# pyro-ppl/pyro

Measured on AMD Instinct MI355X. Metric: ELBO-grad steps/sec (SVI), higher is better.
Workload: dtype f32; 1 GPU; BASELINE configs[1]: Bayesian logistic regression, plate=1000000, D=32, Trace_ELBO num_particles=64 per GPU (vectorised), AutoNormal, Adam; full SVI.step of SVI(model, guide, optim, loss), one hipGraph replay per step; parallelism=particles sharded x1, flat RCCL grad all-reduce

## Files before the change

### include/pyro_amd.h

```cpp
#ifndef PYRO_AMD_H
#define PYRO_AMD_H

#include <stddef.h>
#include <stdint.h>

#ifdef __cplusplus
extern "C" {
#endif

#define PA_ABI_VERSION 9

enum { PA_OK = 0, PA_ERR_INVALID = -1, PA_ERR_UNSUPPORTED = -2, PA_ERR_LAUNCH = -3 };

enum { PA_F32 = 0, PA_F64 = 1 };

enum {
  PA_DIST_NORMAL = 0,
  PA_DIST_BERNOULLI_LOGITS = 1,
  PA_DIST_HALF_CAUCHY = 2,
  PA_DIST_LOG_NORMAL = 3,
  PA_DIST_EXPONENTIAL = 4,
  PA_DIST_HALF_NORMAL = 5,
  PA_DIST_GAMMA = 6,
  PA_DIST_BETA = 7,
// ... 312 lines not shown
#define PA_LSE_MAX_DIMS 6
typedef struct {
  const void* ptr;
  int64_t strides[PA_LSE_MAX_DIMS];
} pa_lse_term;
int pa_logsumexp_terms(int dtype, void* out, int nterms, const pa_lse_term* terms, int ndim,
                       const int64_t* sizes, int rdim, pa_stream_t stream);
int pa_logsumexp_terms_grad(int dtype, void* G, const void* g_out, const void* out, int nterms,
                            const pa_lse_term* terms, int ndim, const int64_t* sizes, int rdim,
                            pa_stream_t stream);

int pa_adam_step(int dtype, void* param, void* grad, void* exp_avg, void* exp_avg_sq, int64_t n,
                 double lr, double beta1, double beta2, double eps, double weight_decay,
                 double clip_norm, double lrd, int clipped, int64_t* step_dev, int zero_grad,
                 pa_stream_t stream);

int pa_mvn_tril_sample(int dtype, const void* loc, const void* rho, const void* A, int64_t n,
                       int64_t P, uint64_t seed, uint64_t offset, const uint64_t* offset_dev,
                       int eps_given, void* eps, void* z, void* logq, pa_stream_t stream);
int pa_mvn_tril_sample_bwd(int dtype, const void* loc, const void* rho, const void* eps,
                           const void* z, const void* d_z, const void* d_logq, int64_t n,
                           int64_t P, void* d_loc, void* d_rho, void* d_A, int accumulate,
                           pa_stream_t stream);

size_t pa_logchain_workspace(int dtype, int64_t B, int64_t T, int64_t K);
int pa_logchain_fwd_bwd(int dtype, const void* unary, const void* pairwise,
                        int64_t pair_stride_batch, int64_t pair_stride_step, int64_t B,
                        int64_t T, int64_t K, void* log_z, void* grad_unary, void* grad_pairwise,
                        void* workspace, size_t workspace_bytes, pa_stream_t stream);

int pa_chain_matvec(int dtype, const void* M, int64_t m_stride_chain, const void* x, void* y,
                    int64_t C, int64_t D, int transpose, pa_stream_t stream);

int pa_adam_step_publish(int dtype, void* param, void* grad, void* exp_avg, void* exp_avg_sq,
                         int64_t n, double lr, double beta1, double beta2, double eps,
                         double weight_decay, double clip_norm, double lrd, int clipped,
                         int64_t* step_dev, int zero_grad, int src_dtype, const void* src,
                         double* host_value, uint64_t* host_seq, uint64_t* counter, uint64_t inc,
                         pa_stream_t stream);

size_t pa_bow_workspace(int64_t B, int64_t V, int64_t H);
int pa_bow_linear_fwd(const void* image_a, const float* W, const float* bias, int64_t B, int64_t V,
                      int64_t H, float* out, void* workspace, size_t workspace_bytes,
                      pa_stream_t stream);
int pa_bow_linear_bwd(const void* image_b, const float* d_out, int64_t B, int64_t V, int64_t H,
                      float* dW, void* workspace, size_t workspace_bytes, pa_stream_t stream);
int pa_bow_linear_fwd_act(const void* image_a, const float* W, const float* bias, int64_t B, int64_t V,
                          int64_t H, int sigmoid_out, float* out, void* workspace,
                          size_t workspace_bytes, pa_stream_t stream);
int pa_bow_linear_bwd_act(const void* image_b, const float* d_out, const float* y_mul, int64_t B, int64_t V,
                          int64_t H, float* dW, float* db_partial, void* workspace, size_t workspace_bytes,
                          pa_stream_t stream);

size_t pa_tsgemm_tn_workspace(int64_t B, int64_t M, int64_t N);
int pa_tsgemm_tn(const float* A, const float* X, int64_t B, int64_t M, int64_t N, float* out,
                 void* workspace, size_t workspace_bytes, pa_stream_t stream);

int pa_tall_linear(const float* G, int64_t B, int64_t R, const float* W, int64_t w_row_stride,
                   int64_t w_col_stride, int64_t C, const float* bias, float* Y, pa_stream_t stream);
size_t pa_tall_wgrad_workspace(int64_t B, int64_t R, int64_t K);
int pa_tall_wgrad(const float* G, const float* X, int64_t B, int64_t R, int64_t K, float* dW, float* db,
                  void* workspace, size_t workspace_bytes, pa_stream_t stream);
int pa_tall_linear_act(const float* G, int64_t B, int64_t R, const float* W, int64_t w_row_stride,
                       int64_t w_col_stride, int64_t C, const float* bias, const float* y_mul,
                       int sigmoid_out, float* Y, pa_stream_t stream);
int pa_tall_wgrad_act(const float* G, const float* X, const float* y_mul, int64_t B, int64_t R, int64_t K,
                      float* dW, float* db, void* workspace, size_t workspace_bytes, pa_stream_t stream);
int pa_tall_linear_path(int64_t B, int64_t R, int64_t C, int64_t w_row_stride, int64_t w_col_stride,
                        int g_aligned16, int ymul_aligned16, int w_aligned16);
int pa_tall_wgrad_path(int64_t B, int64_t R, int64_t K);

int pa_gamma_rsample(int dtype, void* out, void* d_alpha, pa_view2d alpha, int64_t rows, int64_t cols,
                     uint64_t seed, uint64_t offset, const uint64_t* offset_dev, pa_stream_t stream);
int pa_gamma_implicit_grad(int dtype, void* d_alpha, pa_view2d alpha, pa_view2d value, int64_t rows,
                           int64_t cols, pa_stream_t stream);

#define PA_CHAIN_SYNC_BYTES 64
int pa_chain_begin(pa_stream_t stream, void* sync_words, size_t sync_bytes);
int pa_chain_flush(void);
int pa_chain_end(int* launches, int* phases);
int pa_chain_pending(void);
int pa_chain_tune(int fuse_tail);
int pa_chain_fused_launches(void);
int pa_chain_debug_stamps(void* stamps32);

#define PA_RTC_MAX_POINTERS 384
int pa_rtc_compile(const char* source, const char* kernel_name, void** function_out);
int pa_rtc_compile_cached(const char* source, const char* kernel_name, const char* cache_file,
                          void** function_out, int* compiled_out);
int pa_rtc_version(int* hiprtc_major, int* hiprtc_minor, int* runtime_version);
void* pa_rtc_blocks_begin(void);
int pa_rtc_blocks_end(void* scope, int64_t* n_blocks_out);
int pa_rtc_blocks_free(void* scope);
int pa_rtc_launch(void* function, uint32_t grid, uint32_t block, const void* const* pointers,
                  int n_pointers, pa_stream_t stream);

size_t pa_mixture_workspace(int K, int64_t B);
int pa_mixture_fwd_bwd(int dtype, int dist, const void* x, int64_t N, int K, int64_t B, const void* a,
                       int64_t a_batch_stride, const void* p0, int64_t p0_stride, int64_t p0_batch_stride,
                       const void* p1, int64_t p1_stride, int64_t p1_batch_stride, void* workspace,
                       size_t workspace_bytes, double* out, pa_stream_t stream);

int pa_mixture_diag_normal_layout(int K, int D, int* kp_out, int* dd_out);
size_t pa_mixture_diag_normal_workspace(int K, int D, int64_t B);
int pa_mixture_diag_normal_fwd_bwd(int dtype, const void* x, int64_t N, int D, int K, int64_t B, const void* a,
                                   int64_t a_batch_stride, const void* loc, int64_t loc_stride_k,
                                   int64_t loc_stride_d, int64_t loc_batch_stride, const void* scale,
                                   int64_t scale_stride_k, int64_t scale_stride_d, int64_t scale_batch_stride,
                                   void* workspace, size_t workspace_bytes, double* out_padded, pa_stream_t stream);

int64_t pa_mixture_mvn_layout(int K, int D);
size_t pa_mixture_mvn_workspace(int K, int D, int64_t B);
int pa_mixture_mvn_fwd_bwd(int dtype, const void* x, int64_t N, int D, int K, int64_t B, const void* a,
                           int64_t a_batch_stride, const void* loc, int64_t loc_stride_k, int64_t loc_batch_stride,
                           const void* w, int64_t w_stride_k, int64_t w_batch_stride, void* row_lse,
                           void* workspace, size_t workspace_bytes, double* out, pa_stream_t stream);

int64_t pa_mixture_event_layout(int dist, int K, int D);
size_t pa_mixture_event_workspace(int dist, int K, int D, int64_t B);
int pa_mixture_event_fwd_bwd(int dtype, int dist, const void* x, int64_t N, int D, int K, int64_t B, const void* a,
                             int64_t a_batch_stride, const void* p0, int64_t p0_stride_k, int64_t p0_stride_d,
                             int64_t p0_batch_stride, const void* p1, int64_t p1_stride_k, int64_t p1_stride_d,
                             int64_t p1_batch_stride, void* row_lse, void* workspace, size_t workspace_bytes,
                             double* out, pa_stream_t stream);

int pa_mixture_rows_layout(int K, int* kp_out);
size_t pa_mixture_rows_workspace(int K, int64_t B);
int pa_mixture_rows_fwd_bwd(int dtype, int dist, const void* x, int64_t N, int K, int64_t B, const void* a,
                            int64_t a_stride_k, int64_t a_stride_n, int64_t a_batch_stride, const void* p0,
                            int64_t p0_stride, int64_t p0_batch_stride, const void* p1, int64_t p1_stride,
                            int64_t p1_batch_stride, void* da, void* workspace, size_t workspace_bytes,
                            double* out_padded, pa_stream_t stream);

int pa_mixture_rows_diag_normal_layout(int K, int D, int* kp_out, int* dd_out);
size_t pa_mixture_rows_diag_normal_workspace(int K, int D, int64_t B);
int pa_mixture_rows_diag_normal_fwd_bwd(int dtype, const void* x, int64_t N, int D, int K, int64_t B, const void* a,
                                        int64_t a_stride_k, int64_t a_stride_n, int64_t a_batch_stride,
                                        const void* loc, int64_t loc_stride_k, int64_t loc_stride_d,
                                        int64_t loc_batch_stride, const void* scale, int64_t scale_stride_k,
                                        int64_t scale_stride_d, int64_t scale_batch_stride, void* da,
                                        void* workspace, size_t workspace_bytes, double* out_padded,
                                        pa_stream_t stream);

int pa_mixture_assign(int dtype, int dist, const void* x, int64_t N, int K, int64_t B, const void* a,
                      int64_t a_stride_k, int64_t a_stride_n, int64_t a_batch_stride, const void* p0,
                      int64_t p0_stride, int64_t p0_batch_stride, const void* p1, int64_t p1_stride,
                      int64_t p1_batch_stride, int mode, uint64_t seed, uint64_t offset, const uint64_t* offset_dev,
                      int64_t* z, pa_stream_t stream);

int pa_mixture_assign_diag_normal(int dtype, const void* x, int64_t N, int D, int K, int64_t B, const void* a,
                                  int64_t a_stride_k, int64_t a_stride_n, int64_t a_batch_stride, const void* loc,
                                  int64_t loc_stride_k, int64_t loc_stride_d, int64_t loc_batch_stride,
                                  const void* scale, int64_t scale_stride_k, int64_t scale_stride_d,
                                  int64_t scale_batch_stride, int mode, uint64_t seed, uint64_t offset,
                                  const uint64_t* offset_dev, int64_t* z, pa_stream_t stream);

int pa_graph_direct_plan(void* hip_graph, int max_nodes, void** plan_out, int* n_nodes_out);
int pa_graph_direct_launch(void* plan, pa_stream_t stream);
int pa_graph_direct_free(void* plan);

#ifdef __cplusplus
}
#endif
#endif
```

### pyro_amd/_lib.py

```python
import ctypes
import os
from ctypes import (POINTER, Structure, c_char_p, c_double, c_int, c_int32, c_int64, c_size_t, c_uint32,
                    c_uint64, c_void_p)

_HERE = os.path.dirname(os.path.abspath(__file__))
LIB_PATH = os.path.join(_HERE, "lib", "libpyro_amd.so")

PA_OK, PA_ERR_INVALID, PA_ERR_UNSUPPORTED, PA_ERR_LAUNCH = 0, -1, -2, -3
PA_F32, PA_F64 = 0, 1
ABI_VERSION = 9

DIST_NORMAL = 0
DIST_BERNOULLI_LOGITS = 1
DIST_HALF_CAUCHY = 2
DIST_LOG_NORMAL = 3
DIST_EXPONENTIAL = 4
DIST_HALF_NORMAL = 5
DIST_GAMMA = 6
DIST_BETA = 7
DIST_POISSON = 8
DIST_BINOMIAL_LOGITS = 9
DIST_KL_NORMAL_LOC = 10
DIST_KL_NORMAL_SCALE = 11

# ... 220 lines not shown
                                                    c_size_t, c_void_p, c_void_p]),
    "pa_mixture_assign": (c_int, [c_int, c_int, c_void_p, c_int64, c_int, c_int64, c_void_p, c_int64, c_int64, c_int64,
                                  c_void_p, c_int64, c_int64, c_void_p, c_int64, c_int64, c_int, c_uint64, c_uint64,
                                  c_void_p, c_void_p, c_void_p]),
    "pa_mixture_assign_diag_normal": (c_int, [c_int, c_void_p, c_int64, c_int, c_int, c_int64, c_void_p, c_int64,
                                              c_int64, c_int64, c_void_p, c_int64, c_int64, c_int64, c_void_p,
                                              c_int64, c_int64, c_int64, c_int, c_uint64, c_uint64, c_void_p,
                                              c_void_p, c_void_p]),
    "pa_graph_direct_plan": (c_int, [c_void_p, c_int, POINTER(c_void_p), POINTER(c_int)]),
    "pa_graph_direct_launch": (c_int, [c_void_p, c_void_p]),
    "pa_graph_direct_free": (c_int, [c_void_p]),
    "pa_rtc_launch": (c_int, [c_void_p, c_uint32, c_uint32, c_void_p, c_int, c_void_p]),
    "pa_nuts_gaussian_find_step": (c_int, [c_int, c_void_p, c_void_p, c_void_p, c_void_p, c_void_p,
                                           c_void_p, c_int64, c_int64, c_uint64, c_uint64, c_uint64,
                                           c_double, c_double, c_double, c_void_p]),
    "pa_lda_factor_workspace": (c_size_t, [c_int, c_int64, c_int64, c_int64]),
    "pa_lda_factor_fwd_bwd": (c_int, [c_int, c_void_p, c_void_p, c_void_p, c_int64, c_int64,
                                      c_int64, c_int64, c_void_p, c_void_p, c_void_p, c_void_p,
                                      c_size_t, c_void_p]),
    "pa_dirichlet_log_prob": (c_int, [c_int, c_void_p, View2D, View2D, c_int64, c_int64, c_void_p]),
    "pa_dirichlet_log_prob_grad": (c_int, [c_int, c_void_p, View2D, View2D, c_int64, c_int64,
                                           c_void_p, c_void_p, c_void_p]),
    "pa_logsumexp_terms": (c_int, [c_int, c_void_p, c_int, POINTER(LseTerm), c_int, POINTER(c_int64),
                                   c_int, c_void_p]),
    "pa_logsumexp_terms_grad": (c_int, [c_int, c_void_p, c_void_p, c_void_p, c_int, POINTER(LseTerm),
                                        c_int, POINTER(c_int64), c_int, c_void_p]),
    "pa_lda_index_bytes": (c_size_t, [c_int64, c_int64, c_int64]),
    "pa_lda_index_workspace": (c_size_t, [c_int64, c_int64, c_int64]),
    "pa_lda_build_index": (c_int, [c_void_p, c_int64, c_int64, c_int64, c_void_p, c_size_t,
                                   c_void_p, c_size_t, c_void_p]),
    "pa_lda_factor_indexed_workspace": (c_size_t, [c_int, c_int64, c_int64, c_int64, c_int64]),
    "pa_lda_factor_indexed_fwd_bwd": (c_int, [c_int, c_void_p, c_void_p, c_size_t, c_void_p,
                                              c_void_p, c_int64, c_int64, c_int64, c_int64,
                                              c_void_p, c_void_p, c_void_p, c_void_p, c_size_t,
                                              c_void_p]),
    "pa_adam_step": (c_int, [c_int, c_void_p, c_void_p, c_void_p, c_void_p, c_int64, c_double,
                             c_double, c_double, c_double, c_double, c_double, c_double, c_int,
                             c_void_p, c_int, c_void_p]),
    "pa_dist_log_prob_sum_nd_workspace": (c_size_t, []),
    "pa_dist_log_prob_sum_nd": (c_int, [c_int, c_int, c_void_p, c_int, c_void_p, c_void_p, c_void_p,
                                        c_void_p, c_void_p, c_void_p, c_void_p, c_void_p, c_void_p,
                                        c_double, c_void_p, c_size_t, c_void_p]),
    "pa_dist_log_prob_grad_nd": (c_int, [c_int, c_int, c_void_p, c_void_p, c_void_p, c_void_p, c_int,
                                         c_void_p, c_void_p, c_void_p, c_void_p, c_void_p, c_void_p,
                                         c_void_p, c_void_p, c_void_p, c_double, c_void_p]),
    "pa_sum_to_nd_workspace": (c_size_t, [c_int64, c_int64, c_int64]),
    "pa_sum_to_nd": (c_int, [c_int, c_void_p, c_void_p, c_int64, c_int64, c_int64, c_void_p,
                             c_size_t, c_void_p]),
    "pa_sum_to_nd_pair": (c_int, [c_int, c_void_p, c_void_p, c_void_p, c_void_p, c_int64, c_int64, c_int64,
                                  c_void_p, c_size_t, c_void_p]),
    "pa_mvn_tril_sample": (c_int, [c_int, c_void_p, c_void_p, c_void_p, c_int64, c_int64, c_uint64,
                                   c_uint64, c_void_p, c_int, c_void_p, c_void_p, c_void_p, c_void_p]),
    "pa_mvn_tril_sample_bwd": (c_int, [c_int, c_void_p, c_void_p, c_void_p, c_void_p, c_void_p,
                                       c_void_p, c_int64, c_int64, c_void_p, c_void_p, c_void_p,
                                       c_int, c_void_p]),
    "pa_logchain_workspace": (c_size_t, [c_int, c_int64, c_int64, c_int64]),
    "pa_logchain_fwd_bwd": (c_int, [c_int, c_void_p, c_void_p, c_int64, c_int64, c_int64, c_int64,
                                    c_int64, c_void_p, c_void_p, c_void_p, c_void_p, c_size_t,
                                    c_void_p]),
    "pa_chain_matvec": (c_int, [c_int, c_void_p, c_int64, c_void_p, c_void_p, c_int64, c_int64, c_int,
                                c_void_p]),
    "pa_bow_workspace": (c_size_t, [c_int64, c_int64, c_int64]),
    "pa_bow_linear_fwd": (c_int, [c_void_p, c_void_p, c_void_p, c_int64, c_int64, c_int64, c_void_p,
                                  c_void_p, c_size_t, c_void_p]),
    "pa_bow_linear_bwd": (c_int, [c_void_p, c_void_p, c_int64, c_int64, c_int64, c_void_p, c_void_p,
                                  c_size_t, c_void_p]),
    "pa_bow_linear_fwd_act": (c_int, [c_void_p, c_void_p, c_void_p, c_int64, c_int64, c_int64, c_int, c_void_p,
                                      c_void_p, c_size_t, c_void_p]),
    "pa_bow_linear_bwd_act": (c_int, [c_void_p, c_void_p, c_void_p, c_int64, c_int64, c_int64, c_void_p,
                                      c_void_p, c_void_p, c_size_t, c_void_p]),
    "pa_tsgemm_tn_workspace": (c_size_t, [c_int64, c_int64, c_int64]),
    "pa_tsgemm_tn": (c_int, [c_void_p, c_void_p, c_int64, c_int64, c_int64, c_void_p, c_void_p, c_size_t,
                             c_void_p]),
    "pa_gamma_rsample": (c_int, [c_int, c_void_p, c_void_p, View2D, c_int64, c_int64, c_uint64, c_uint64,
                                 c_void_p, c_void_p]),
    "pa_gamma_implicit_grad": (c_int, [c_int, c_void_p, View2D, View2D, c_int64, c_int64, c_void_p]),
    "pa_chain_begin": (c_int, [c_void_p, c_void_p, c_size_t]),
    "pa_chain_flush": (c_int, []),
    "pa_chain_end": (c_int, [POINTER(c_int), POINTER(c_int)]),
    "pa_chain_pending": (c_int, []),
    "pa_chain_debug_stamps": (c_int, [c_void_p]),
    "pa_chain_tune": (c_int, [c_int]),
    "pa_chain_fused_launches": (c_int, []),
    "pa_adam_step_publish": (c_int, [c_int, c_void_p, c_void_p, c_void_p, c_void_p, c_int64,
                                     c_double, c_double, c_double, c_double, c_double, c_double,
                                     c_double, c_int, c_void_p, c_int, c_int, c_void_p, c_void_p,
                                     c_void_p, c_void_p, c_uint64, c_void_p]),
}

_lib = None


def exported_symbols():
    return sorted(_SIGNATURES)


def load(path=None):
    global _lib
    if _lib is not None:
        return _lib
    path = path or os.environ.get("PYRO_AMD_LIB", LIB_PATH)
    if not os.path.exists(path):
        raise RuntimeError(
            "pyro_amd: HIP extension %s not found. Build it with "
            "`python -m pyro_amd.csrc.build` (hipcc --offload-arch=gfx950). There is no CPU "
            "fallback." % path)
    import torch
    lib = ctypes.CDLL(path)
    for name, (res, args) in _SIGNATURES.items():
        fn = getattr(lib, name)
        fn.restype = res
        fn.argtypes = args
    if lib.pa_abi_version() != ABI_VERSION:
        raise RuntimeError("pyro_amd: ABI version mismatch: %d" % lib.pa_abi_version())
    if os.environ.get("PYRO_AMD_GLM_FINALIZE") == "in_kernel":
        lib.pa_glm_planes_finalize_mode(1)
    _lib = lib
    return lib


def check(rc):
    if rc == PA_OK:
        return
    msg = load().pa_last_error().decode("utf-8", "replace")
    if rc == PA_ERR_INVALID:
        raise ValueError("pyro_amd: " + msg)
    if rc == PA_ERR_UNSUPPORTED:
        raise Unsupported("pyro_amd: " + msg)
    raise RuntimeError("pyro_amd: kernel launch failed: " + msg)
```

### pyro_amd/csrc/chain.hip

```cpp
#include "chain.h"
#include "glm_finalize.h"
#include "multisite_dev.h"
#include "optim_dev.h"
#include "site_tail.h"

namespace pa {

constexpr int CH_FIN = 0, CH_MULTI = 1, CH_MF = 2, CH_ADAM = 3, CH_PHASES = 4;
constexpr int CH_MF_SITES = 8;

struct MfArgs8 {
  int nsites;
  MfSiteDev s[CH_MF_SITES];
};
static_assert(offsetof(MfArgs8, s) == offsetof(MfArgs, s), "layout");

constexpr int CH_TAIL_ENTRIES = 6;
struct TailSite {
  int n_entries;
  int entries[CH_TAIL_ENTRIES];
  int extras_mask;
  int64_t off_loc, off_rho;
  int fast;
  int layout;
};

struct ChainArgs {
  MultiArgs multi;
  MfArgs8 mf;
  const float* fin_part;
  float *fin_ll, *fin_gw, *fin_gb;
  double fin_scale, fin_ll_offset;
  int fin_nblocks, fin_npass, fin_D, fin_P, fin_DT, fin_PT;
  float* multi_out;
  const float* multi_g;
  double multi_coef_all;
  int multi_accumulate, multi_n;
  int64_t mf_P;
  int mf_gy, mf_nsites;
  float *ad_p, *ad_g, *ad_m, *ad_v;
  int64_t ad_n;
  double ad_lr, ad_b1, ad_b2, ad_eps, ad_wd, ad_clip, ad_lrd;
  int64_t* ad_step;
  int ad_clipped, ad_zero;
  AdamPublish ad_pub;
  uint32_t* sync;
  int have[CH_PHASES];
  int grid[CH_PHASES];
  int last;
  uint64_t* stamps;
  const int64_t* gate;
  uint32_t jitter;
  int tail_nsites;
  uint32_t fin_dep_mask;
  TailSite tail[CH_MF_SITES];
};
static_assert(sizeof(ChainArgs) <= 6144, "kernel arguments grew unexpectedly");

__device__ __forceinline__ void chain_jitter(uint32_t seed, int p, uint32_t salt) {
  if (seed == 0u) return;
  uint32_t hsh = seed * 2654435761u ^ (blockIdx.x + 1u) * 40503u ^ (uint32_t)(p + 1) * 2246822519u ^ salt;
  hsh ^= hsh >> 15;
  hsh *= 2654435761u;
  hsh ^= hsh >> 13;
  const uint32_t n = (hsh >> 8) & 63u;
  if ((hsh & 3u) == 0u) return;
  for (uint32_t i = 0; i < n; ++i) __builtin_amdgcn_s_sleep(8);
}

__device__ __forceinline__ void chain_signal(uint32_t jitter, uint32_t* sync, int p, uint32_t expected,
                                             bool last) {
  chain_jitter(jitter, p, 0x9e3779b9u);
  __syncthreads();
  if (threadIdx.x == 0) {
    __builtin_amdgcn_fence(__ATOMIC_RELEASE, "agent");
    const uint32_t old =
        __hip_atomic_fetch_add(&sync[p], 1u, __ATOMIC_RELAXED, __HIP_MEMORY_SCOPE_AGENT);
    if (last && old == expected - 1u) {
#pragma unroll
      for (int q = 0; q < CH_PHASES; ++q)
        __hip_atomic_store(&sync[q], 0u, __ATOMIC_RELAXED, __HIP_MEMORY_SCOPE_AGENT);
    }
  }
}

__device__ __forceinline__ void chain_wait(uint32_t jitter, uint32_t* sync, int p, uint32_t expected) {
  if (threadIdx.x == 0) {
    const uint64_t t0 = wall_clock64();
    while (__hip_atomic_load(&sync[p], __ATOMIC_RELAXED, __HIP_MEMORY_SCOPE_AGENT) < expected) {
      __builtin_amdgcn_s_sleep(2);
      if (wall_clock64() - t0 > 400000000ull) __builtin_trap();
    }
    __builtin_amdgcn_fence(__ATOMIC_ACQUIRE, "agent");
  }
  __syncthreads();
  chain_jitter(jitter, p, 0x85ebca6bu);
}

template <int DT, int PT, int SUB>
__device__ __forceinline__ void chain_fin(const ChainArgs& a, int me, int nw) {
  __shared__ double sm[SUB][FIN_GROUPS][FIN_OUT];
  const int sub = SUB == 1 ? 0 : (int)(threadIdx.x >> 8), tid = (int)(threadIdx.x & 255);
  for (int64_t base = (int64_t)me * SUB; base < a.grid[CH_FIN]; base += (int64_t)nw * SUB) {
    glm_finalize_body<DT, PT>(base + sub, a.fin_part, a.fin_nblocks, a.fin_npass, a.fin_D, a.fin_P,
                              a.fin_scale, a.fin_ll, a.fin_gw, a.fin_gb, a.fin_ll_offset, tid,
                              sm[sub]);
    __syncthreads();
  }
}
template <int SUB>
__device__ __forceinline__ void chain_fin_any(const ChainArgs& a, int me, int nw) {
  if (a.fin_DT == 1 && a.fin_PT == 2) chain_fin<1, 2, SUB>(a, me, nw);
  else if (a.fin_DT == 1 && a.fin_PT == 1) chain_fin<1, 1, SUB>(a, me, nw);
  else if (a.fin_DT == 2 && a.fin_PT == 1) chain_fin<2, 1, SUB>(a, me, nw);
  else if (a.fin_DT == 2 && a.fin_PT == 2) chain_fin<2, 2, SUB>(a, me, nw);
  else if (a.fin_DT == 4 && a.fin_PT == 2) chain_fin<4, 2, SUB>(a, me, nw);
  else chain_fin<4, 1, SUB>(a, me, nw);
}

#define PA_CHAIN_STAMP(i)                                                     \
  do {                                                                        \
    if (a.stamps != nullptr && threadIdx.x == 0 && (me == 0 || total_wg))     \
      a.stamps[(total_wg ? 16 : 0) + (i)] = wall_clock64();                   \
  } while (0)

__global__ __launch_bounds__(1024) void chain_kernel(const ChainArgs a) {
  if (a.gate != nullptr && *a.gate != 0) return;
  const bool total_wg = blockIdx.x == gridDim.x - 1;
  if (!total_wg && threadIdx.x >= 256) return;
  const int nw = (int)gridDim.x - 1, me = (int)blockIdx.x;
  uint32_t* sync = a.sync;
  const int part_fin = a.grid[CH_FIN] < nw ? a.grid[CH_FIN] : nw;
  const int part_multi = (a.multi_n < nw ? a.multi_n : nw) + 1;
  const int part_mf = a.grid[CH_MF] < nw ? a.grid[CH_MF] : nw;
  int prev = -1, prev_n = 0;
  PA_CHAIN_STAMP(0);

  if (a.have[CH_FIN]) {
    if (!total_wg && me < part_fin) {
      chain_fin_any<1>(a, me, nw);
      chain_signal(a.jitter, sync, CH_FIN, (uint32_t)part_fin, a.last == CH_FIN);
    }
    prev = CH_FIN;
    prev_n = part_fin;
  }
  PA_CHAIN_STAMP(1);
  if (a.have[CH_MULTI]) {
    constexpr uint32_t KB = (uint32_t)offsetof(ChainArgs, multi);
    if (total_wg || me < part_multi - 1) {
      if (prev >= 0) chain_wait(a.jitter, sync, prev, (uint32_t)prev_n);
      PA_CHAIN_STAMP(2);
      if (total_wg) {
        multi_sum_body<float, MULTI_THREADS>(KB, a.multi_out, a.multi_coef_all, a.multi_accumulate);
      } else {
        for (int vb = me; vb < a.multi_n; vb += nw) {
          multi_grad_body<float>(KB, vb, a.multi_g, a.multi_coef_all);
          __syncthreads();
        }
      }
      chain_signal(a.jitter, sync, CH_MULTI, (uint32_t)part_multi, a.last == CH_MULTI);
    }
    prev = CH_MULTI;
    prev_n = part_multi;
  }
  PA_CHAIN_STAMP(3);
  if (total_wg) return;
  if (a.have[CH_MF]) {
    constexpr uint32_t KB = (uint32_t)offsetof(ChainArgs, mf);
    if (me < part_mf) {
      if (prev >= 0) chain_wait(a.jitter, sync, prev, (uint32_t)prev_n);
      PA_CHAIN_STAMP(4);
      for (int vb = me; vb < a.grid[CH_MF]; vb += nw) {
        meanfield_sample_bwd_body<float>(KB, (uint32_t)(vb % a.mf_nsites),
                                         (uint32_t)(vb / a.mf_nsites), (uint32_t)a.mf_gy, a.mf_P);
        __syncthreads();
      }
      chain_signal(a.jitter, sync, CH_MF, (uint32_t)part_mf, a.last == CH_MF);
    }
    prev = CH_MF;
    prev_n = part_mf;
  }
  PA_CHAIN_STAMP(5);
  if (a.have[CH_ADAM]) {
    const int part_adam = a.grid[CH_ADAM] < nw ? a.grid[CH_ADAM] : nw;
    if (me < part_adam) {
      if (prev >= 0) chain_wait(a.jitter, sync, prev, (uint32_t)prev_n);
      PA_CHAIN_STAMP(6);
      for (int64_t vb = me; vb < a.grid[CH_ADAM]; vb += nw)
        adam_body<float>(vb, (int64_t)a.grid[CH_ADAM], a.ad_p, a.ad_g, a.ad_m, a.ad_v, a.ad_n,
                         a.ad_lr, a.ad_b1, a.ad_b2, a.ad_eps, a.ad_wd, a.ad_clip, a.ad_lrd,
                         a.ad_clipped, a.ad_step, a.ad_zero, a.ad_pub);
      chain_signal(a.jitter, sync, CH_ADAM, (uint32_t)part_adam, a.last == CH_ADAM);
    }
  }
  PA_CHAIN_STAMP(7);
}

__global__ __launch_bounds__(1024) void chain_tail_kernel(const ChainArgs a) {
  if (a.gate != nullptr && *a.gate != 0) return;
  const bool total_wg = blockIdx.x == gridDim.x - 1;
  const int nw = (int)gridDim.x - 1, me = (int)blockIdx.x;
  uint32_t* sync = a.sync;
  if (me < a.tail_nsites && threadIdx.x >= 256) return;
  const int nfw = nw - a.tail_nsites;
  const int fin_vwg = (a.grid[CH_FIN] + 3) / 4;
  const int part_fin = fin_vwg < nfw ? fin_vwg : nfw;
  PA_CHAIN_STAMP(0);
  if (!total_wg && me >= a.tail_nsites) {
    const int fme = me - a.tail_nsites;
    if (a.have[CH_FIN] && fme < part_fin) {
      chain_fin_any<4>(a, fme, nfw);
      chain_signal(a.jitter, sync, CH_FIN, (uint32_t)part_fin, false);
    }
    return;
  }
  PA_CHAIN_STAMP(1);
  constexpr uint32_t KB = (uint32_t)offsetof(ChainArgs, multi);
  constexpr uint32_t KMF = (uint32_t)offsetof(ChainArgs, mf);
  const uint32_t KT = (uint32_t)offsetof(ChainArgs, tail) + (uint32_t)me * (uint32_t)sizeof(TailSite);
  auto tail_entry = [&](int q) -> int {
    return kernarg_load<int>(KT + (uint32_t)offsetof(TailSite, entries) + 4u * (uint32_t)q);
  };
  int ts_n = 0, ts_mask = 0, ts_fast = 0;
  int64_t step = 0;
  if (!total_wg) ts_fast = kernarg_load<int>(KT + (uint32_t)offsetof(TailSite, fast));
  if (!total_wg && ts_fast) {
    __shared__ double fast_red[4 * GRAD_THREADS];
    __shared__ float fast_xch[4 * 64];
    const int layout = kernarg_load<int>(KT + (uint32_t)offsetof(TailSite, layout));
    const EntryDev eh = kernarg_load<EntryDev>(KB + (uint32_t)offsetof(MultiArgs, e) +
                                               (uint32_t)tail_entry(0) * (uint32_t)sizeof(EntryDev));
    const EntryDev eg = kernarg_load<EntryDev>(KB + (uint32_t)offsetof(MultiArgs, e) +
                                               (uint32_t)tail_entry(1) * (uint32_t)sizeof(EntryDev));
    const MfSiteDev ms = kernarg_load<MfSiteDev>(KMF + (uint32_t)offsetof(MfArgs, s) +
                                                 (uint32_t)me * (uint32_t)sizeof(MfSiteDev));
    const int64_t off_loc = kernarg_load<int64_t>(KT + (uint32_t)offsetof(TailSite, off_loc));
    const int64_t off_rho = kernarg_load<int64_t>(KT + (uint32_t)offsetof(TailSite, off_rho));
    const SiteAdam ad{a.ad_p, a.ad_g, a.ad_m, a.ad_v, a.ad_step, a.ad_lr, a.ad_b1, a.ad_b2, a.ad_eps,
                      a.ad_wd, a.ad_clip, a.ad_lrd, a.ad_clipped, a.ad_zero};
    auto wait = [&]() {
      PA_CHAIN_STAMP(7);
      if (a.have[CH_FIN]) chain_wait(a.jitter, sync, CH_FIN, (uint32_t)part_fin);
      else __syncthreads();
      PA_CHAIN_STAMP(2);
    };
    site_fast<PA_DIST_NORMAL>(eh, eg, ms, layout, a.multi_coef_all, off_loc, off_rho, ad, fast_red,
                              fast_xch, wait, &step);
    PA_CHAIN_STAMP(5);
  } else {
  double total_acc = 0.0;
  if (total_wg) {
    total_acc = multi_sum_partial<float, MULTI_THREADS>(KB, a.fin_dep_mask, 0u);
  }
  if (!total_wg) {
    ts_n = kernarg_load<int>(KT + (uint32_t)offsetof(TailSite, n_entries));
    ts_mask = kernarg_load<int>(KT + (uint32_t)offsetof(TailSite, extras_mask));
    for (int q = 0; q < ts_n; ++q) {
      multi_grad_body<float>(KB, tail_entry(q), a.multi_g, a.multi_coef_all, GRAD_NO_EXTRAS);
      __syncthreads();
    }
  }
  PA_CHAIN_STAMP(7);
  if (a.have[CH_FIN]) chain_wait(a.jitter, sync, CH_FIN, (uint32_t)part_fin);
  PA_CHAIN_STAMP(2);
  if (total_wg) {
    total_acc += multi_sum_partial<float, MULTI_THREADS>(KB, 0u, a.fin_dep_mask);
    multi_sum_finish<float>(total_acc, a.multi_out, a.multi_coef_all, a.multi_accumulate);
    if (threadIdx.x == 0) step = a.ad_step[0] + 1;
  } else {
    for (int q = 0; q < ts_n; ++q)
      if (ts_mask >> q & 1)
        multi_grad_body<float>(KB, tail_entry(q), a.multi_g, a.multi_coef_all, GRAD_EXTRAS_ONLY);
    __syncthreads();
    PA_CHAIN_STAMP(3);
    meanfield_sample_bwd_body<float>(KMF, (uint32_t)me, 0u, 1u, a.mf_P);
    __syncthreads();
    PA_CHAIN_STAMP(4);
    const MfSiteDev ms = kernarg_load<MfSiteDev>(KMF + (uint32_t)offsetof(MfArgs, s) +
                                                 (uint32_t)me * (uint32_t)sizeof(MfSiteDev));
    const int64_t off_loc = kernarg_load<int64_t>(KT + (uint32_t)offsetof(TailSite, off_loc));
    const int64_t off_rho = kernarg_load<int64_t>(KT + (uint32_t)offsetof(TailSite, off_rho));
    adam_two_ranges<float>(off_loc, off_rho, ms.n, a.ad_p, a.ad_g, a.ad_m, a.ad_v, a.ad_step,
                           a.ad_lr, a.ad_b1, a.ad_b2, a.ad_eps, a.ad_wd, a.ad_clip, a.ad_lrd,
                           a.ad_clipped, a.ad_zero, &step);
    PA_CHAIN_STAMP(5);
  }
  }
  __syncthreads();
  if (threadIdx.x == 0) {
    __builtin_amdgcn_fence(__ATOMIC_RELEASE, "agent");
    const unsigned long long ticket = __hip_atomic_fetch_add(
        reinterpret_cast<unsigned long long*>(a.ad_step + 1), 1ull, __ATOMIC_RELAXED,
        __HIP_MEMORY_SCOPE_AGENT);
    if (ticket == (unsigned long long)a.tail_nsites) {
      __builtin_amdgcn_fence(__ATOMIC_ACQUIRE, "agent");
      a.ad_step[1] = 0;
      a.ad_step[0] = step;
#pragma unroll
      for (int q = 0; q < CH_PHASES; ++q)
        __hip_atomic_store(&sync[q], 0u, __ATOMIC_RELAXED, __HIP_MEMORY_SCOPE_AGENT);
      publish_to_host(a.ad_pub);
    }
  }
  PA_CHAIN_STAMP(6);
}

static int g_chain_fast_sites = 1;

static bool chain_plan_tail(ChainArgs& a) {
  if (!(a.have[CH_MULTI] && a.have[CH_MF] && a.have[CH_ADAM])) return false;
  if (a.multi_g != nullptr || a.mf_nsites < 1 || a.mf_nsites > CH_MF_SITES) return false;
  const float* g0 = a.ad_g;
  const float* g1 = a.ad_g + a.ad_n;
  int owner[PA_MULTI_MAX_ENTRIES];
  for (int e = 0; e < a.multi.n; ++e) owner[e] = -1;
  int64_t covered = 0;
  int64_t lo[2 * CH_MF_SITES], hi[2 * CH_MF_SITES];
  for (int k = 0; k < a.mf_nsites; ++k) {
    const MfSiteDev& s = a.mf.s[k];
    TailSite& t = a.tail[k];
    t.n_entries = 0;
    t.extras_mask = 0;
    if (s.n < 1 || s.n > 4096 || !s.accumulate || s.d_loc == nullptr || s.d_rho == nullptr) return false;
    const float* dl = (const float*)s.d_loc;
    const float* dr = (const float*)s.d_rho;
    if (dl < g0 || dl + s.n > g1 || dr < g0 || dr + s.n > g1) return false;
    t.off_loc = dl - g0;
    t.off_rho = dr - g0;
    lo[2 * k] = t.off_loc; hi[2 * k] = t.off_loc + s.n;
    lo[2 * k + 1] = t.off_rho; hi[2 * k + 1] = t.off_rho + s.n;
    covered += 2 * s.n;
    for (int e = 0; e < a.multi.n; ++e) {
      const EntryDev& en = a.multi.e[e];
      const bool own_v = (en.need & PA_NEED_VALUE) && en.dv && !(en.need & PA_VALUE_BY_CHAIN);
      const bool own_a = (en.need & PA_NEED_P0) && en.da, own_b = (en.need & PA_NEED_P1) && en.db;
      int hits = 0, outs = 0;
      if (own_v) { ++outs; hits += (en.dv == s.d_z); }
      if (own_a) { ++outs; hits += (en.da == s.d_loc_out || en.da == s.d_scale); }
      if (own_b) { ++outs; hits += (en.db == s.d_loc_out || en.db == s.d_scale); }
      if (hits == 0) continue;
      if (hits != outs || owner[e] >= 0) return false;
      if (t.n_entries == CH_TAIL_ENTRIES) return false;
      owner[e] = k;
      if (t.n_entries == 0) t.extras_mask = 0;
      if (own_v && en.xg != nullptr) t.extras_mask |= 1 << t.n_entries;
      t.entries[t.n_entries++] = e;
    }
  }
  for (int e = 0; e < a.multi.n; ++e) {
    const EntryDev& en = a.multi.e[e];
    const bool writes = ((en.need & PA_NEED_VALUE) && en.dv && !(en.need & PA_VALUE_BY_CHAIN)) ||
                        ((en.need & PA_NEED_P0) && en.da) || ((en.need & PA_NEED_P1) && en.db);
    if (writes && owner[e] < 0) return false;
  }
  for (int k = 0; k < a.mf_nsites; ++k) {
    const MfSiteDev& s = a.mf.s[k];
    const void* wants[3] = {s.d_z, s.d_scale, s.d_loc_out};
    for (const void* w : wants) {
      if (w == nullptr) continue;
      bool found = false;
      for (int q = 0; q < a.tail[k].n_entries && !found; ++q) {
        const EntryDev& en = a.multi.e[a.tail[k].entries[q]];
        found = en.dv == w || en.da == w || en.db == w;
      }
      if (!found) return false;
    }
  }
  if (covered != a.ad_n) return false;
  const int m = 2 * a.mf_nsites;
  for (int i = 0; i < m; ++i)
    for (int j = i + 1; j < m; ++j)
      if (lo[i] < hi[j] && lo[j] < hi[i]) return false;
  a.fin_dep_mask = 0u;
  if (a.have[CH_FIN]) {
    auto in_fin = [&](const void* p) {
      const float* f = (const float*)p;
      return p != nullptr &&
             ((f >= a.fin_ll && f < a.fin_ll + a.fin_P) || (f >= a.fin_gb && f < a.fin_gb + a.fin_P) ||
              (f >= a.fin_gw && f < a.fin_gw + (int64_t)a.fin_P * a.fin_D));
    };
    for (int e = 0; e < a.multi.n; ++e) {
      const EntryDev& en = a.multi.e[e];
      if (in_fin(en.v) || in_fin(en.a) || in_fin(en.b) || in_fin(en.m)) a.fin_dep_mask |= 1u << e;
    }
    if (a.multi.n > MULTI_THREADS / 64) a.fin_dep_mask = 0xffffffffu;
  }
  for (int k = 0; k < a.mf_nsites; ++k) {
    const MfSiteDev& s = a.mf.s[k];
    TailSite& t = a.tail[k];
    t.fast = 0;
    t.layout = SITE_LAYOUT_COLS;
    if (!g_chain_fast_sites || t.n_entries != 2) continue;
    const EntryDev& h = a.multi.e[t.entries[0]];
    const EntryDev& q = a.multi.e[t.entries[1]];
    const bool family = h.dist == PA_DIST_NORMAL;
    const bool shape =
        family && q.dist == PA_DIST_NORMAL && h.m == nullptr &&
        q.m == nullptr && h.chain_next == t.entries[1] && q.chain_next < 0 &&
        (h.need & PA_NEED_VALUE) && !(h.need & PA_VALUE_BY_CHAIN) && h.dv == s.d_z &&
        !((h.need & PA_NEED_P0) && h.da) && !((h.need & PA_NEED_P1) && h.db) &&
        (q.need & PA_VALUE_BY_CHAIN) && (q.need & PA_NEED_P0) && (q.need & PA_NEED_P1) &&
        q.da == s.d_loc_out && q.db == s.d_scale && q.da != nullptr && q.db != nullptr &&
        q.v == h.v && q.vsr == h.vsr && q.vsc == h.vsc && q.rows == h.rows && q.cols == h.cols &&
        s.d_z != nullptr && s.eps != nullptr && s.rho != nullptr;
    if (!shape) continue;
    const int64_t P = a.mf_P;
    if (s.n >= 2 && s.n <= GRAD_THREADS && h.rows == P && h.cols == s.n && h.vsr == s.n &&
        h.vsc == 1 && q.asr == 0 && q.asc == 1 && q.bsr == 0 && q.bsc == 1) {
      const int64_t ng = GRAD_THREADS / s.n > 8 ? 8 : GRAD_THREADS / s.n;
      if (P <= UN * ng) { t.fast = 1; t.layout = SITE_LAYOUT_COLS; }
    } else if (s.n == 1 && h.rows == 1 && h.cols == P && P >= 2 && P <= 64 && h.vsc == 1 &&
               q.asc == 0 && q.bsc == 0) {
      t.fast = 1;
      t.layout = SITE_LAYOUT_SCALAR;
    }
  }
  a.tail_nsites = a.mf_nsites;
  return true;
}

struct ChainState {
  bool on = false;
  hipStream_t stream = nullptr;
  int top = -1;
  int launches = 0;
  int phases = 0;
  int fused = 0;
  ChainArgs a;
};
static ChainState g_chain;
static uint64_t* g_chain_stamps = nullptr;
static int g_chain_fuse = 1;
static uint32_t g_chain_jitter = 0;

static int chain_launch() {
  ChainState& c = g_chain;
  if (c.top < 0) return PA_OK;
  ChainArgs& a = c.a;
  int maxgrid = 1, np = 0;
  for (int p = 0; p < CH_PHASES; ++p)
    if (a.have[p]) {
      a.last = p;
      ++np;
      if (a.grid[p] > maxgrid) maxgrid = a.grid[p];
    }
  a.stamps = g_chain_stamps;
  gate_emit_deferred(c.stream);
  a.gate = gate_word();
  a.jitter = g_chain_jitter;
  gate_aware_launch();
  int nw = cu_count() - 1;
  if (nw < 1) nw = 1;
  if (maxgrid < nw) nw = maxgrid;
  const hipStream_t s = c.stream;
  c.top = -1;
  a.tail_nsites = 0;
  if (g_chain_fuse && cu_count() - 1 > CH_MF_SITES && chain_plan_tail(a)) {
    nw = a.tail_nsites + (a.have[CH_FIN] ? (a.grid[CH_FIN] + 3) / 4 : 0);
    if (nw > cu_count() - 1) nw = cu_count() - 1;
    hipLaunchKernelGGL(chain_tail_kernel, dim3((unsigned)nw + 1), dim3(1024), 0, s, a);
    c.fused += 1;
  } else {
    hipLaunchKernelGGL(chain_kernel, dim3((unsigned)nw + 1), dim3(1024), 0, s, a);
  }
  c.launches += 1;
  c.phases += np;
  for (int p = 0; p < CH_PHASES; ++p) a.have[p] = 0;
  return check_launch("chain_kernel");
}

static bool chain_open(pa_stream_t stream, int k, int* rc) {
  ChainState& c = g_chain;
  *rc = PA_OK;
  if (!c.on) return false;
  if ((hipStream_t)stream != c.stream) {
    *rc = chain_launch();
    return false;
  }
  if (c.top >= k) *rc = chain_launch();
  if (*rc != PA_OK) return false;
  if (c.top < 0) {
    for (int p = 0; p < CH_PHASES; ++p) c.a.have[p] = 0, c.a.grid[p] = 0;
  }
  c.top = k;
  c.a.have[k] = 1;
  return true;
}

int chain_record_fin(pa_stream_t stream, int DT, int PT, const float* part, int nblocks, int npass,
                     int D, int P, double scale, float* ll, float* gw, float* gb, double ll_offset) {
  const bool shape_ok = (PT == 1 || PT == 2) && (DT == 1 || DT == 2 || DT == 4);
  if (!g_chain.on || !shape_ok) return 0;
  int rc;
  if (!chain_open(stream, CH_FIN, &rc)) return rc;
  ChainArgs& a = g_chain.a;
  a.fin_part = part; a.fin_ll = ll; a.fin_gw = gw; a.fin_gb = gb;
  a.fin_scale = scale; a.fin_ll_offset = ll_offset;
  a.fin_nblocks = nblocks; a.fin_npass = npass; a.fin_D = D; a.fin_P = P;
  a.fin_DT = DT; a.fin_PT = PT;
  const int64_t J = (int64_t)P * D + 2 * P;
  a.grid[CH_FIN] = (int)((J + FIN_OUT - 1) / FIN_OUT);
  return 1;
}

int chain_record_multi(pa_stream_t stream, const MultiArgs& args, float* out, const float* g,
                       double coef_all, int accumulate) {
  if (!g_chain.on) return 0;
  int rc;
  if (!chain_open(stream, CH_MULTI, &rc)) return rc;
  ChainArgs& a = g_chain.a;
  a.multi = args;
  a.multi_out = out; a.multi_g = g; a.multi_coef_all = coef_all; a.multi_accumulate = accumulate;
  a.multi_n = args.n;
  a.grid[CH_MULTI] = args.n;
  return 1;
}

int chain_record_mf_bwd(pa_stream_t stream, const MfArgs& args, int nsites, int64_t P, int gy) {
  if (!g_chain.on || nsites > CH_MF_SITES) return 0;
  int rc;
  if (!chain_open(stream, CH_MF, &rc)) return rc;
  ChainArgs& a = g_chain.a;
  a.mf.nsites = nsites;
  for (int k = 0; k < nsites; ++k) a.mf.s[k] = args.s[k];
  a.mf_P = P; a.mf_gy = gy; a.mf_nsites = nsites;
  a.grid[CH_MF] = nsites * gy;
  return 1;
}

// ... 10 lines not shown
  a.ad_lrd = lrd; a.ad_step = step_dev; a.ad_clipped = clipped; a.ad_zero = zero_grad;
  a.ad_pub = pub;
  int64_t grid = (n + 255) / 256;
  const int64_t cap = (int64_t)cu_count() * 8;
  if (grid > cap) grid = cap;
  a.grid[CH_ADAM] = (int)grid;
  return 1;
}

struct PendingDraw {
  bool have = false;
  MfArgs args;
  int nsites = 0;
  int64_t P = 0;
  uint64_t seed = 0;
  const uint64_t* offset_dev = nullptr;
};
static PendingDraw g_draw;
static int g_draw_enabled = 1;

int meanfield_sample_launch(const MfArgs& args, int nsites, int64_t P, uint64_t seed,
                            const uint64_t* offset_dev, hipStream_t s);

int chain_flush_draw() {
  if (!g_draw.have) return PA_OK;
  g_draw.have = false;
  return meanfield_sample_launch(g_draw.args, g_draw.nsites, g_draw.P, g_draw.seed, g_draw.offset_dev,
                                 g_chain.stream);
}

int chain_park_draw(pa_stream_t stream, const MfArgs& args, int nsites, int64_t P, uint64_t seed,
                    const uint64_t* offset_dev) {
  if (!g_chain.on || !g_draw_enabled || (hipStream_t)stream != g_chain.stream || g_chain.top >= 0) return 0;
  int rc = chain_flush_draw();
  if (rc != PA_OK) return rc;
  g_draw.have = true;
  g_draw.args = args;
  g_draw.nsites = nsites;
  g_draw.P = P;
  g_draw.seed = seed;
  g_draw.offset_dev = offset_dev;
  return 1;
}

bool glm_take_pending_draw(pa_stream_t stream, const float* w, const float* b, int64_t P, int64_t D,
                           GlmDraw* out) {
  if (!g_draw.have || (hipStream_t)stream != g_chain.stream || g_draw.P != P) return false;
  int kw = -1, kb = -1;
  for (int k = 0; k < g_draw.nsites; ++k) {
    const MfSiteDev& sd = g_draw.args.s[k];
    if (sd.z == (const void*)w && sd.n == D) kw = k;
    if (b != nullptr && sd.z == (const void*)b && sd.n == 1) kb = k;
  }
  if (kw < 0 || (b != nullptr && kb < 0)) return false;
  const MfSiteDev& sw = g_draw.args.s[kw];
  out->loc_w = (const float*)sw.loc; out->rho_w = (const float*)sw.rho;
  out->z_w = (float*)sw.z; out->eps_w = (float*)sw.eps; out->scale_w = (float*)sw.scale;
  out->lout_w = (float*)sw.loc_out; out->off_w = sw.offset;
  out->have_b = kb >= 0;
  if (kb >= 0) {
    const MfSiteDev& sb = g_draw.args.s[kb];
    out->loc_b = (const float*)sb.loc; out->rho_b = (const float*)sb.rho;
    out->z_b = (float*)sb.z; out->eps_b = (float*)sb.eps; out->scale_b = (float*)sb.scale;
    out->lout_b = (float*)sb.loc_out; out->off_b = sb.offset;
  } else {
    out->loc_b = out->rho_b = nullptr;
    out->z_b = out->eps_b = out->scale_b = out->lout_b = nullptr;
    out->off_b = 0;
  }
  out->seed = g_draw.seed;
  out->offset_dev = g_draw.offset_dev;
  MfArgs rest;
  rest.nsites = 0;
  for (int k = 0; k < g_draw.nsites; ++k)
    if (k != kw && k != kb) rest.s[rest.nsites++] = g_draw.args.s[k];
  g_draw.have = false;
  if (rest.nsites > 0)
    (void)meanfield_sample_launch(rest, rest.nsites, g_draw.P, g_draw.seed, g_draw.offset_dev, g_chain.stream);
  return true;
}

hipStream_t as_stream(pa_stream_t s) {
  if (g_draw.have) (void)chain_flush_draw();
  if (g_chain.on && g_chain.top >= 0) (void)chain_launch();
  return (hipStream_t)s;
}

}

extern "C" {

int pa_chain_begin(pa_stream_t stream, void* sync_words, size_t sync_bytes) {
  PA_REQUIRE(!pa::g_chain.on, "pa_chain_begin: already recording on this thread");
  PA_REQUIRE(sync_words != nullptr && sync_bytes >= PA_CHAIN_SYNC_BYTES,
             "pa_chain_begin: needs %d zeroed bytes of device memory", PA_CHAIN_SYNC_BYTES);
  pa::g_chain.on = true;
  pa::g_chain.stream = (hipStream_t)stream;
  pa::g_chain.top = -1;
  pa::g_chain.launches = pa::g_chain.phases = pa::g_chain.fused = 0;
  for (int p = 0; p < pa::CH_PHASES; ++p) pa::g_chain.a.have[p] = 0;
  pa::g_chain.a.sync = (uint32_t*)sync_words;
  return PA_OK;
}

int pa_chain_flush(void) {
  if (!pa::g_chain.on) return PA_OK;
  int rc = pa::chain_flush_draw();
  if (rc != PA_OK) return rc;
  return pa::chain_launch();
}

int pa_chain_end(int* launches, int* phases) {
  int rc = PA_OK;
  if (pa::g_chain.on) {
    rc = pa::chain_flush_draw();
    const int rc2 = pa::chain_launch();
    if (rc == PA_OK) rc = rc2;
  }
  pa::g_chain.on = false;
  if (launches) *launches = pa::g_chain.launches;
  if (phases) *phases = pa::g_chain.phases;
  return rc;
}

int pa_chain_tune(int fuse_tail) {
  pa::g_chain_fuse = (fuse_tail & 1) ? 1 : 0;
  pa::g_chain_fast_sites = (fuse_tail & 2) ? 0 : 1;
  pa::g_chain_jitter = (uint32_t)fuse_tail >> 8;
  pa::g_draw_enabled = (fuse_tail & 4) ? 0 : 1;
  return PA_OK;
}

int pa_chain_fused_launches(void) { return pa::g_chain.fused; }

int pa_chain_debug_stamps(void* stamps32) {
  pa::g_chain_stamps = (uint64_t*)stamps32;
#ifdef PA_CHAIN_LATENCY_PROBE
  uint64_t* p = (uint64_t*)stamps32;
  int zero = 0;
  (void)hipMemcpyToSymbol(HIP_SYMBOL(pa::pa_dbg_stamps), &p, sizeof(p));
  (void)hipMemcpyToSymbol(HIP_SYMBOL(pa::pa_dbg_next), &zero, sizeof(zero));
#endif
  return PA_OK;
}

int pa_chain_pending(void) {
  if (!pa::g_chain.on || pa::g_chain.top < 0) return 0;
  int n = 0;
  for (int p = 0; p < pa::CH_PHASES; ++p) n += pa::g_chain.a.have[p];
  return n;
}

}
```

### pyro_amd/csrc/common.h

```cpp
#pragma once
#include <hip/hip_runtime.h>
#include <stdarg.h>
#include <stdint.h>
#include <stdio.h>

#include "../../include/pyro_amd.h"

namespace pa {

__device__ __forceinline__ float fast_sigmoid(float h) {
  return __builtin_amdgcn_rcpf(1.0f + __builtin_amdgcn_exp2f(-1.44269504088896340736f * h));
}


constexpr int WAVE = 64;

void set_error(const char* fmt, ...);
int fail(int code, const char* fmt, ...);
int check_launch(const char* what);
int cu_count();
const int64_t* gate_word();
void gate_aware_launch();
void gate_emit_deferred(hipStream_t s);
bool take_bracket(int tag, hipEvent_t* start, hipEvent_t* stop);

#define PA_REQUIRE(cond, ...)                                  \
  do {                                                         \
    if (!(cond)) return ::pa::fail(PA_ERR_INVALID, __VA_ARGS__); \
  } while (0)

template <int CTRL>
__device__ __forceinline__ int dpp_mov(int v) {
  return __builtin_amdgcn_update_dpp(0, v, CTRL, 0xf, 0xf, false);
}
template <int CTRL>
__device__ __forceinline__ float dpp_get(float v) {
  return __int_as_float(dpp_mov<CTRL>(__float_as_int(v)));
}
template <int CTRL>
__device__ __forceinline__ double dpp_get(double v) {
  const int lo = dpp_mov<CTRL>(__double2loint(v)), hi = dpp_mov<CTRL>(__double2hiint(v));
  return __hiloint2double(hi, lo);
}
__device__ __forceinline__ float lane_get(float v, int lane) {
  return __int_as_float(__builtin_amdgcn_readlane(__float_as_int(v), lane));
}
__device__ __forceinline__ double lane_get(double v, int lane) {
  const int lo = __builtin_amdgcn_readlane(__double2loint(v), lane);
  const int hi = __builtin_amdgcn_readlane(__double2hiint(v), lane);
  return __hiloint2double(hi, lo);
}
template <typename T>
__device__ __forceinline__ T wave_sum(T v) {
  if constexpr (sizeof(T) == 4 || sizeof(T) == 8) {
    v += dpp_get<0xB1>(v);
    v += dpp_get<0x4E>(v);
    v += dpp_get<0x141>(v);
    v += dpp_get<0x140>(v);
    const T s0 = lane_get(v, 0), s1 = lane_get(v, 16), s2 = lane_get(v, 32), s3 = lane_get(v, 48);
    return (s0 + s1) + (s2 + s3);
  } else {
#pragma unroll
    for (int o = 32; o > 0; o >>= 1) v += __shfl_xor(v, o, 64);
    return v;
  }
}
template <typename T>
__device__ __forceinline__ T wave_max(T v) {
#pragma unroll
  for (int o = 32; o > 0; o >>= 1) {
    T u = __shfl_xor(v, o, 64);
    v = u > v ? u : v;
  }
  return v;
}

__device__ __forceinline__ double block_sum_f64_waves(double v, double* smem ,
                                                      int nw) {
  v = wave_sum(v);
  const int lane = threadIdx.x & 63, wid = threadIdx.x >> 6;
  __syncthreads();
  if (lane == 0) smem[wid] = v;
  __syncthreads();
  double t = 0.0;
  if (threadIdx.x == 0)
    for (int i = 0; i < nw; ++i) t += smem[i];
  return t;
}

__device__ __forceinline__ double block_sum_f64(double v, double* smem ) {
  v = wave_sum(v);
  const int lane = threadIdx.x & 63, wid = threadIdx.x >> 6, nw = (blockDim.x + 63) >> 6;
  __syncthreads();
  if (lane == 0) smem[wid] = v;
  __syncthreads();
  double t = 0.0;
  if (threadIdx.x == 0)
    for (int i = 0; i < nw; ++i) t += smem[i];
  return t;
}

struct u32x4 {
  uint32_t x, y, z, w;
};
__host__ __device__ __forceinline__ u32x4 philox4x32_10(uint64_t seed, uint64_t ctr_lo,
                                                        uint64_t ctr_hi) {
// ... 72 lines not shown
```

### pyro_amd/csrc/glm.hip

```cpp
#include "common.h"
#include "glm_bf16.h"
#include "glm_planes.h"
#include "glm_planes16.h"
#include "glm_planes16w.h"
#include "glm_planes16d.h"
#include "glm_finalize.h"
#include "chain.h"

namespace pa {

static int g_glm_variant = 0;

typedef float f32x16 __attribute__((ext_vector_type(16)));

constexpr int GLM_WAVES = 4;

template <int DT>
struct GlmCfg {
  static constexpr int DP = 32 * DT;
  static constexpr int S = DP + 3;
  static constexpr int TILE_F = 32 * S;
};


template <int DT, int PT, bool VEC4, bool GROUPED>
__global__ __launch_bounds__(64 * GLM_WAVES, 2) void glm_bernoulli_kernel(
    const float* __restrict__ X, const float* __restrict__ y, const float* __restrict__ w,
    const float* __restrict__ b, const uint8_t* __restrict__ mask, int64_t N, int D, int P,
    int64_t iters, float* __restrict__ part, const int64_t* __restrict__ seg, int G) {
  using C = GlmCfg<DT>;
  constexpr int DP = C::DP, S = C::S, TILE_F = C::TILE_F;
  extern __shared__ __attribute__((aligned(16))) float lds[];
  const int lane = threadIdx.x & 63, wave = threadIdx.x >> 6;
  const int l31 = lane & 31, h = lane >> 5;
  float* Xs = lds + wave * TILE_F;

  for (int i = threadIdx.x; i < GLM_WAVES * TILE_F; i += 64 * GLM_WAVES) lds[i] = 0.0f;

  int64_t row_begin = 0, row_end = N;
  int group = 0;
  if constexpr (GROUPED) {
    row_begin = seg[3 * (int64_t)blockIdx.x];
    row_end = seg[3 * (int64_t)blockIdx.x + 1];
    group = (int)seg[3 * (int64_t)blockIdx.x + 2];
  }

  const int pbase = blockIdx.y * 32 * PT;
  float wf[PT][DP / 2];
  float bias[PT];
#pragma unroll
  for (int pt = 0; pt < PT; ++pt) {
    const int p = pbase + pt * 32 + l31;
#pragma unroll
    for (int kk = 0; kk < DP / 2; ++kk) {
      const int d = 2 * kk + h;
      wf[pt][kk] = (p < P && d < D)
                       ? w[(GROUPED ? ((int64_t)p * G + group) : (int64_t)p) * D + d]
                       : 0.0f;
    }
    bias[pt] = (p < P && b != nullptr) ? b[p] : 0.0f;
  }

  f32x16 gwacc[PT][DT];
  float ll_acc[PT], gb_acc[PT];
#pragma unroll
  for (int pt = 0; pt < PT; ++pt) {
    ll_acc[pt] = 0.0f;
    gb_acc[pt] = 0.0f;
#pragma unroll
    for (int dt = 0; dt < DT; ++dt)
#pragma unroll
      for (int r = 0; r < 16; ++r) gwacc[pt][dt][r] = 0.0f;
  }

  constexpr int NLD = VEC4 ? 4 * DT : 16 * DT;
  constexpr int EPL = VEC4 ? 4 : 1;
  float stage[NLD * EPL];
  uint8_t stage_m[NLD];
  float st_y = 0.0f, st_m = 0.0f;
  const int step_e = 64 * EPL;
  const int q0 = step_e / D, r0 = step_e % D;
  const int e0 = lane * EPL;
  const int n_first = e0 / D, d_first = e0 % D;
  const int64_t total_e = row_end * (int64_t)D;
  int nrow[NLD];
  {
    int n = n_first, d = d_first;
#pragma unroll
    for (int j = 0; j < NLD; ++j) {
      nrow[j] = n;
// ... 390 lines not shown
  (void)hipFuncSetAttribute((const void*)k, hipFuncAttributeMaxDynamicSharedMemorySize, lds);
  hipLaunchKernelGGL(k, dim3((unsigned)pl.nblocks, (unsigned)pl.npass), dim3(256), lds, s, img, y, w,
                     b, N, D, P, pl.nst, part, cu_count(), fin, GlmGroupArgs{nullptr, nullptr, 1});
}

static void glm_planes_launch_grouped(int nseg, int npass, const unsigned char* img,
                                      const float* y_img, const float* w, const float* b, int64_t N,
                                      int D, int P, int64_t nst_total, float* part,
                                      const GlmGroupArgs& grp, hipStream_t s) {
  auto k = glm_planes_kernel<2, 3, 3, true>;
  constexpr int lds = GlmPlCfg<2, 3>::LDS_BYTES;
  (void)hipFuncSetAttribute((const void*)k, hipFuncAttributeMaxDynamicSharedMemorySize, lds);
  GlmFinArgs fin;
  fin.counters = nullptr;
  fin.part64 = nullptr;
  fin.ll = fin.gw = fin.gb = nullptr;
  fin.scale = fin.ll_offset = 0.0;
  fin.D = D; fin.P = P;
  fin.tstamps = g_planes_stamps;
  hipLaunchKernelGGL(k, dim3((unsigned)nseg, (unsigned)npass), dim3(256), lds, s, img, y_img, w, b, N,
                     D, P, nst_total, part, cu_count(), fin, grp);
}

static int64_t glmh_tile_bytes(int64_t ntiles) { return ntiles * (int64_t)GLMH_TILE; }

static bool g_planes_wide = true;
static int g_planes_wide_max = 8;
static bool g_planes_wide_force = false;

static GlmPlanesPlan glmh_plan(int64_t N, int64_t P, bool allow_wide = true) {
  GlmPlanesPlan pl;
  pl.nb = g_planes_nb;
  pl.bpc = g_planes_bpc > 0 && g_planes_bpc <= 4 ? g_planes_bpc : 2;
  pl.npass = (int)((P + 63) / 64);
  pl.nst = ((N + 31) / 32 + 1) / 2;
  int64_t cap = (int64_t)cu_count() * pl.bpc / pl.npass;
  if (cap < 1) cap = 1;
  pl.nblocks = (int)(pl.nst < cap ? (pl.nst < 1 ? 1 : pl.nst) : cap);
  pl.ypass = pl.npass;
  const bool enough_tiles = (N + 31) / 32 >= (int64_t)48 * cu_count();
  if (allow_wide && g_planes_wide && pl.nb == 3 && g_planes_bpc <= 0 && P > 64 &&
      (enough_tiles || g_planes_wide_force)) {
    const bool eight = P > 128 && g_planes_wide_max >= 8;
    pl.nrt = eight ? 1 : 2;
    pl.npt = eight ? 8 : 4;
    const int64_t wrows = 32 * pl.npt;
    pl.ypass = (int)((P + wrows - 1) / wrows);
    pl.nst = pl.nrt == 1 ? (N + 31) / 32 : ((N + 31) / 32 + 1) / 2;
    pl.bpc = 1;
    cap = (int64_t)cu_count() / pl.ypass;
    if (cap < 1) cap = 1;
    pl.nblocks = (int)(pl.nst < cap ? (pl.nst < 1 ? 1 : pl.nst) : cap);
  }
  return pl;
}

template <int NRT, int NPT, bool LIN>
static void glmh_launch_wide(const GlmPlanesPlan& pl, const unsigned char* img, const float* y, const float* w,
                             const float* b, int64_t N, int D, int P, float* part, const uint32_t* trailer,
                             hipStream_t s, const double* moments) {
  auto k = glm_planes_f16_kernel<3, 1, false, false, LIN, false, NRT, NPT>;
  constexpr int lds = GlmHCfg<3, false, NRT, NPT>::LDS_BYTES;
  (void)hipFuncSetAttribute((const void*)k, hipFuncAttributeMaxDynamicSharedMemorySize, lds);
  hipLaunchKernelGGL(k, dim3((unsigned)pl.nblocks, (unsigned)pl.ypass), dim3(64 * NRT * NPT), lds, s, img, y, w, b,
                     N, D, P, pl.nst, part, cu_count(), trailer, g_planes_stamps, GlmGroupArgs{nullptr, nullptr, 1},
                     gate_word(), moments, GlmDraw{});
  gate_aware_launch();
}

template <int NB, int OCC, bool PRIV = false, bool LIN = false, bool DRAW = false>
static void glmh_launch_one(const GlmPlanesPlan& pl, const unsigned char* img, const float* y,
                            const float* w, const float* b, int64_t N, int D, int P, float* part,
                            const uint32_t* trailer, hipStream_t s, const double* moments = nullptr,
                            const GlmDraw& draw = GlmDraw{}) {
  auto k = glm_planes_f16_kernel<NB, OCC, false, PRIV, LIN, DRAW>;
  constexpr int lds = GlmHCfg<NB, PRIV>::LDS_BYTES + (DRAW ? 256 : 0);
  (void)hipFuncSetAttribute((const void*)k, hipFuncAttributeMaxDynamicSharedMemorySize, lds);
  hipLaunchKernelGGL(k, dim3((unsigned)pl.nblocks, (unsigned)pl.npass), dim3(256), lds, s, img, y, w,
                     b, N, D, P, pl.nst, part, cu_count(), trailer, g_planes_stamps,
                     GlmGroupArgs{nullptr, nullptr, 1}, gate_word(), moments, draw);
  gate_aware_launch();
}

template <int DT, int OCC>
static int glmd_launch(const unsigned char* img, const float* y, const float* w, const float* b, int64_t N,
                       int D, int P, float* part, const uint32_t* trailer, int bpc, int* nblocks_out,
                       int64_t* nst_out, hipStream_t s) {
  auto k = glm_planes_f16d_kernel<DT, 3, OCC>;
  constexpr int lds = GlmDCfg<DT, 3>::LDS_BYTES;
  (void)hipFuncSetAttribute((const void*)k, hipFuncAttributeMaxDynamicSharedMemorySize, lds);
  const int npass = (int)((P + 63) / 64);
  const int64_t nst = ((N + 31) / 32 + 1) / 2;
  int64_t cap = (int64_t)cu_count() * bpc / npass;
  if (cap < 1) cap = 1;
  const int nblocks = (int)(nst < cap ? (nst < 1 ? 1 : nst) : cap);
  *nblocks_out = nblocks;
  *nst_out = nst;
  hipLaunchKernelGGL(k, dim3((unsigned)nblocks, (unsigned)npass), dim3(256), lds, s, img, y, w, b, N, D, P,
                     nst, part, trailer, gate_word());
  gate_aware_launch();
  return check_launch("glm_planes_f16d_kernel");
}

static int glmd_run(const void* planes, const float* y, const float* w, const float* b, double scale,
                    int64_t N, int D, int P, float* ll, float* gw, float* gb, float* part,
                    pa_stream_t stream, hipStream_t s) {
  const int DT = D <= 64 ? 2 : 4;
  const unsigned char* img = (const unsigned char*)planes;
  const uint32_t* trailer = (const uint32_t*)(img + glmh_tile_bytes(glm_planes_tiles(N)) * DT);
  hipEvent_t ev0, ev1;
  const bool br = take_bracket(PA_KERNEL_GLM, &ev0, &ev1);
  if (br) (void)hipEventRecord(ev0, s);
  int nblocks = 1;
  int64_t nst = 0;
  int rc = DT == 2 ? glmd_launch<2, 2>(img, y, w, b, N, D, P, part, trailer, 2, &nblocks, &nst, s)
                   : glmd_launch<4, 1>(img, y, w, b, N, D, P, part, trailer, 1, &nblocks, &nst, s);
  if (br) (void)hipEventRecord(ev1, s);
  if (rc != PA_OK) return rc;
  const int npass = (P + 63) / 64;
  const double ll_offset = (double)(nst * 64 - N) * 0.6931471805599453;
  rc = chain_record_fin(stream, DT, 2, part, nblocks, npass, D, P, scale, ll, gw, gb, ll_offset);
  if (rc != 0) return rc < 0 ? rc : PA_OK;
  const int64_t J = (int64_t)P * D + 2 * P;
  const dim3 fgrid((unsigned)((J + FIN_OUT - 1) / FIN_OUT)), fblock(FIN_OUT * FIN_GROUPS);
  if (DT == 2)
    hipLaunchKernelGGL((glm_finalize_kernel<2, 2>), fgrid, fblock, 0, s, part, nblocks, npass, D, P, scale, ll,
                       gw, gb, ll_offset);
  else
    hipLaunchKernelGGL((glm_finalize_kernel<4, 2>), fgrid, fblock, 0, s, part, nblocks, npass, D, P, scale, ll,
                       gw, gb, ll_offset);
  return check_launch("glm_finalize_kernel");
}

template <int NB>
static void glmw_launch(int bpc, const unsigned char* img, const float* y, const float* w, const float* b,
                        int64_t N, int D, int P, float* part, const uint32_t* trailer, int* nblocks_out,
                        hipStream_t s) {
  auto k = glm_planes_f16w_kernel<NB>;
  constexpr int lds = GlmWCfg<NB>::LDS_BYTES;
  (void)hipFuncSetAttribute((const void*)k, hipFuncAttributeMaxDynamicSharedMemorySize, lds);
  const int npass = (int)((P + 63) / 64);
  const int64_t ngrp = (N + 127) / 128;
  int64_t cap = (int64_t)cu_count() * bpc / npass;
  if (cap < 1) cap = 1;
  const int nblocks = (int)(ngrp < cap ? ngrp : cap);
  *nblocks_out = nblocks;
  hipLaunchKernelGGL(k, dim3((unsigned)nblocks, (unsigned)npass), dim3(256), lds, s, img, y, w, b, N, D, P,
                     ngrp, part, trailer, g_planes_stamps, gate_word());
  gate_aware_launch();
}

template <int OCC>
static void glmh_launch_grouped(int nseg, int npass, const unsigned char* img, const float* y_img,
                                const float* w, const float* b, int64_t N, int D, int P,
                                int64_t nst_total, float* part, const uint32_t* trailer,
                                const GlmGroupArgs& grp, hipStream_t s) {
  auto k = glm_planes_f16_kernel<3, OCC, true>;
  constexpr int lds = GlmHCfg<3>::LDS_BYTES;
  (void)hipFuncSetAttribute((const void*)k, hipFuncAttributeMaxDynamicSharedMemorySize, lds);
  hipLaunchKernelGGL(k, dim3((unsigned)nseg, (unsigned)npass), dim3(256), lds, s, img, y_img, w, b, N,
                     D, P, nst_total, part, cu_count(), trailer, g_planes_stamps, grp, gate_word(),
                     (const double*)nullptr, GlmDraw{});
  gate_aware_launch();
}

static int glmh_absmax(const float* X, int64_t N, int D, uint32_t* trailer, hipStream_t s) {
// ... 374 lines not shown
size_t pa_glm_bernoulli_planes_workspace(int64_t N, int64_t D, int64_t P) {
  if (N < 0 || D < 1 || D > 128 || P < 1) return 0;
  if (D > 32) {
    const size_t npass = (size_t)((P + 63) / 64);
    const size_t cap = (size_t)pa::cu_count() * 2;
    const size_t nst = (size_t)(((N + 31) / 32 + 1) / 2);
    const size_t nb = nst < cap ? (nst < 1 ? 1 : nst) : cap;
    return nb * npass * (2 * (size_t)glmd_dt(D) * 1024 + 2 * 2 * 32) * sizeof(float);
  }
  const pa::GlmPlanesPlan pl = pa::glm_planes_plan(N, P);
  const size_t cap = (size_t)pa::cu_count() * 4;
  const size_t ntiles = (size_t)((N + 31) / 32);
  const size_t nb = ntiles < cap ? (ntiles < 1 ? 1 : ntiles) : cap;
  const size_t rec = 2 * 1024 + 2 * 2 * 32;
  return nb * pl.npass * rec * sizeof(float) +
         (size_t)pl.npass * pa::GLMF_GROUPS * rec * sizeof(double);
}

size_t pa_glm_label_moments_workspace(int64_t N) {
  if (N < 0) return 0;
  int64_t grid = (N + 63) / 64;
  const int64_t cap = (int64_t)pa::cu_count() * 4;
  if (grid > cap) grid = cap;
  if (grid < 1) grid = 1;
  return (size_t)grid * 33 * sizeof(double);
}

int pa_glm_label_moments(const float* X, const float* y, int64_t N, int64_t D, double* moments,
                         void* workspace, size_t workspace_bytes, pa_stream_t stream) {
  PA_REQUIRE(N >= 0 && D >= 1 && D <= 32, "glm_label_moments: bad shape N=%lld D=%lld", (long long)N,
             (long long)D);
  PA_REQUIRE(moments != nullptr && (N == 0 || (X && y)), "glm_label_moments: NULL pointer");
  PA_REQUIRE(workspace && workspace_bytes >= pa_glm_label_moments_workspace(N),
             "glm_label_moments: workspace too small");
  const int nblocks = (int)(pa_glm_label_moments_workspace(N) / (33 * sizeof(double)));
  hipStream_t s = pa::as_stream(stream);
  hipLaunchKernelGGL(pa::glm_label_moments_partial_kernel, dim3((unsigned)nblocks), dim3(256), 0, s, X, y,
                     N, (int)D, (double*)workspace);
  int rc = pa::check_launch("glm_label_moments_partial_kernel");
  if (rc != PA_OK) return rc;
  hipLaunchKernelGGL(pa::glm_label_moments_final_kernel, dim3(1), dim3(64), 0, s,
                     (const double*)workspace, nblocks, moments);
  return pa::check_launch("glm_label_moments_final_kernel");
}

int pa_glm_bernoulli_planes_fwd_bwd(int format, const void* planes, const float* y, const float* w,
                                    const float* b, double scale, int64_t N, int64_t D, int64_t P,
                                    float* ll, float* gw, float* gb, void* workspace,
                                    size_t workspace_bytes, const double* moments,
                                    pa_stream_t stream) {
  PA_REQUIRE(N >= 0 && D >= 1 && P >= 1, "glm_planes: bad shape N=%lld D=%lld P=%lld", (long long)N,
             (long long)D, (long long)P);
  if (D > 128 || (D > 32 && format != PA_GLM_PLANES_F16X2))
    return pa::fail(PA_ERR_UNSUPPORTED, "glm_planes: the plane image holds D <= 32 (f16 format: D <= 128), got %lld",
                    (long long)D);
  PA_REQUIRE_FORMAT(format, "glm_planes");
  PA_REQUIRE(N < (int64_t(1) << 40) && P < (1 << 20), "glm_planes: shape too large");
  PA_REQUIRE(w && ll && gw && gb, "glm_planes: NULL parameter/output pointer");
  PA_REQUIRE(N == 0 || (planes && y), "glm_planes: NULL data pointer");
  pa::GlmDraw draw;
  bool drawn = false;
  if (format == PA_GLM_PLANES_F16X2 && N > 0 && D <= 32) {
    const pa::GlmPlanesPlan p0 = pa::glmh_plan(N, P);
    if (p0.nb == 3 && p0.bpc < 4) drawn = pa::glm_take_pending_draw(stream, w, b, P, D, &draw);
  }
  hipStream_t s = pa::as_stream(stream);
  if (N == 0) {
    hipError_t e1 = hipMemsetAsync(ll, 0, (size_t)P * 4, s);
    hipError_t e2 = hipMemsetAsync(gw, 0, (size_t)P * D * 4, s);
    hipError_t e3 = hipMemsetAsync(gb, 0, (size_t)P * 4, s);
    if (e1 != hipSuccess || e2 != hipSuccess || e3 != hipSuccess)
      return pa::fail(PA_ERR_LAUNCH, "glm_planes: memset failed");
    return PA_OK;
  }
  PA_REQUIRE((reinterpret_cast<uintptr_t>(planes) & 15) == 0, "glm_planes: unaligned image");
  PA_REQUIRE(workspace && workspace_bytes >= pa_glm_bernoulli_planes_workspace(N, D, P),
             "glm_planes: workspace too small");
  if (D > 32) return pa::glmd_run(planes, y, w, b, scale, N, (int)D, (int)P, ll, gw, gb, (float*)workspace, stream, s);
  pa::GlmPlanesPlan pl =
      format == PA_GLM_PLANES_F16X2 ? pa::glmh_plan(N, P, !drawn) : pa::glm_planes_plan(N, P);
  const bool wide = format == PA_GLM_PLANES_F16X2 && (pl.nb == 9 || pl.nb == 10) && pl.bpc <= 2;
  float* part = (float*)workspace;
  const unsigned char* img = (const unsigned char*)planes;
  hipEvent_t ev0, ev1;
  const bool br = pa::take_bracket(PA_KERNEL_GLM, &ev0, &ev1);
  if (br) (void)hipEventRecord(ev0, s);
  const double ll_offset = (double)((wide ? (N + 127) / 128 * 128 : pl.nst * 32 * pl.nrt) - N) * 0.6931471805599453;
  pa::GlmFinArgs fin;
  fin.counters = nullptr;
  if (format == PA_GLM_PLANES_BF16X3 && pa::g_planes_fin_mode == 1 && pl.npass <= pa::GLMF_MAX_PASSES) {
    hipStreamCaptureStatus cs = hipStreamCaptureStatusNone;
    const bool capturing = hipStreamIsCapturing(s, &cs) == hipSuccess && cs != hipStreamCaptureStatusNone;
    fin.counters = pa::glmf_counters(!capturing);
  }
  const size_t rec_bytes = (size_t)pl.nblocks * pl.npass * (2 * 1024 + 2 * 2 * 32) * sizeof(float);
  PA_REQUIRE(rec_bytes <= workspace_bytes, "glm_planes: %d x %d records exceed the workspace", pl.nblocks, pl.npass);
  fin.part64 = (double*)((char*)workspace + ((rec_bytes + 15) & ~(size_t)15));
  fin.ll = ll; fin.gw = gw; fin.gb = gb;
  fin.scale = scale; fin.ll_offset = ll_offset;
  fin.D = (int)D; fin.P = (int)P;
  fin.tstamps = pa::g_planes_stamps;
  if (format == PA_GLM_PLANES_F16X2) {
    const uint32_t* trailer = (const uint32_t*)(img + pa::glmh_tile_bytes(pa::glm_planes_tiles(N)));
    if (pl.npt == 4 && moments != nullptr) pa::glmh_launch_wide<2, 4, true>(pl, img, y, w, b, N, (int)D, (int)P, part, trailer, s, moments);
    else if (pl.npt == 4) pa::glmh_launch_wide<2, 4, false>(pl, img, y, w, b, N, (int)D, (int)P, part, trailer, s, nullptr);
    else if (pl.npt == 8 && moments != nullptr) pa::glmh_launch_wide<1, 8, true>(pl, img, y, w, b, N, (int)D, (int)P, part, trailer, s, moments);
    else if (pl.npt == 8) pa::glmh_launch_wide<1, 8, false>(pl, img, y, w, b, N, (int)D, (int)P, part, trailer, s, nullptr);
    else if (wide && pl.nb == 9) pa::glmw_launch<3>(pl.bpc, img, y, w, b, N, (int)D, (int)P, part, trailer, &pl.nblocks, s);
    else if (wide) pa::glmw_launch<4>(pl.bpc, img, y, w, b, N, (int)D, (int)P, part, trailer, &pl.nblocks, s);
    else if (pl.nb == 5) pa::glmh_launch_one<3, 3, true>(pl, img, y, w, b, N, (int)D, (int)P, part, trailer, s);
    else if (pl.nb == 6) pa::glmh_launch_one<4, 3, true>(pl, img, y, w, b, N, (int)D, (int)P, part, trailer, s);
    else if (pl.nb == 4) pa::glmh_launch_one<4, 3>(pl, img, y, w, b, N, (int)D, (int)P, part, trailer, s);
    else if (pl.bpc >= 4) pa::glmh_launch_one<3, 4>(pl, img, y, w, b, N, (int)D, (int)P, part, trailer, s);
    else if (moments != nullptr && drawn)
      pa::glmh_launch_one<3, 3, false, true, true>(pl, img, y, w, b, N, (int)D, (int)P, part, trailer, s, moments, draw);
    else if (moments != nullptr)
      pa::glmh_launch_one<3, 3, false, true>(pl, img, y, w, b, N, (int)D, (int)P, part, trailer, s, moments);
    else if (drawn)
      pa::glmh_launch_one<3, 3, false, false, true>(pl, img, y, w, b, N, (int)D, (int)P, part, trailer, s, nullptr, draw);
    else pa::glmh_launch_one<3, 3>(pl, img, y, w, b, N, (int)D, (int)P, part, trailer, s);
  } else if (pl.nb == 3) {
    pa::glm_planes_launch_one<3, 3>(pl, img, y, w, b, N, (int)D, (int)P, part, fin, s);
  } else {
    pa::glm_planes_launch_one<4, 2>(pl, img, y, w, b, N, (int)D, (int)P, part, fin, s);
  }
  if (br) (void)hipEventRecord(ev1, s);
  int rc = pa::check_launch("glm_planes_kernel");
  if (rc != PA_OK) return rc;
  if (fin.counters != nullptr) return PA_OK;
  const int64_t J = (int64_t)P * D + 2 * P;
  rc = pa::chain_record_fin(stream, 1, 2, part, pl.nblocks, pl.npass, (int)D, (int)P, scale, ll, gw,
                            gb, ll_offset);
  if (rc != 0) return rc < 0 ? rc : PA_OK;
  hipLaunchKernelGGL((pa::glm_finalize_kernel<1, 2>),
                     dim3((unsigned)((J + pa::FIN_OUT - 1) / pa::FIN_OUT)),
                     dim3(pa::FIN_OUT * pa::FIN_GROUPS), 0, s, part, pl.nblocks, pl.npass, (int)D,
                     (int)P, scale, ll, gw, gb, ll_offset);
  return pa::check_launch("glm_finalize_kernel");
}

}
```

### pyro_amd/csrc/glm_planes16.h

```cpp
#pragma once
#include "chain.h"
#include "glm_planes.h"
#include "multisite_dev.h"

namespace pa {

constexpr int GLMH_TILE = 2 * GLMP_PLANE;
constexpr int GLMH_TRAILER = 256;
constexpr int GLMH_KX = 32;
constexpr int GLMH_KNONE = 1 << 20;

constexpr float GLMH_GSCALE = 16384.0f;
typedef _Float16 f16x8 __attribute__((ext_vector_type(8)));
typedef _Float16 f16x2v __attribute__((ext_vector_type(2)));

__device__ __forceinline__ f16x8 as_f16x8(uint32_t a, uint32_t b, uint32_t c, uint32_t d) {
  u32x4v v = {a, b, c, d};
  return __builtin_bit_cast(f16x8, v);
}

__host__ __device__ __forceinline__ int glmh_exponent_of(uint32_t absmax_bits) {
  const int e = (int)(absmax_bits >> 23) & 0xff;
  if (absmax_bits == 0u || e == 0xff) return 0;
  return 14 - (e == 0 ? -127 : e - 127);
// ... 101 lines not shown
    const int d = 8 * s + j;
    v[j] = (row < N && d < D) ? ldexpf(X[row * D + d], glmh_exponent_of(trailer[d])) : 0.0f;
  }
  glmh_store_slot(v, img + T * GLMH_TILE + glmp_slot_ofs(r, s));
}

__global__ __launch_bounds__(256) void glm_pack_planes_f16_grouped_kernel(
    const float* __restrict__ X, const float* __restrict__ y, const int64_t* __restrict__ row_of, int D,
    const int64_t* __restrict__ seg, const int64_t* __restrict__ st_off, int nseg, int64_t ntiles,
    unsigned char* __restrict__ img, float* __restrict__ y_img, uint32_t* __restrict__ trailer) {
  const int64_t idx = (int64_t)blockIdx.x * 256 + threadIdx.x;
  if (idx < 32) trailer[GLMH_KX + idx] = (uint32_t)glmh_exponent_of(trailer[idx]);
  if (idx >= ntiles * 128) return;
  const int64_t T = idx >> 7, st = T >> 1;
  const int r = (int)(idx >> 2) & 31, sl = (int)idx & 3;
  int lo = 0, hi = nseg - 1;
  while (lo < hi) {
    const int mid = (lo + hi + 1) >> 1;
    if (st_off[mid] <= st) lo = mid;
    else hi = mid - 1;
  }
  const int64_t a = seg[3 * lo], e = seg[3 * lo + 1];
  const int64_t pos = a + (T - 2 * st_off[lo]) * 32 + r;
  const bool ok = pos < e;
  const int64_t row = (ok && row_of) ? row_of[pos] : pos;
  float v[8];
#pragma unroll
  for (int j = 0; j < 8; ++j) {
    const int d = 8 * sl + j;
    v[j] = (ok && d < D) ? ldexpf(X[row * D + d], glmh_exponent_of(trailer[d])) : 0.0f;
  }
  glmh_store_slot(v, img + T * GLMH_TILE + glmp_slot_ofs(r, sl));
  if (sl == 0) y_img[T * 32 + r] = ok ? __builtin_fmaf(y[row], GLMH_GSCALE, -0.5f * GLMH_GSCALE) : 0.0f;
}

template <int NB, bool PRIV = false, int NRT_ = 2, int NPT_ = 2>
struct GlmHCfg {
  static constexpr int NRT = NRT_, NPT = NPT_, NW = NRT_ * NPT_;
  static constexpr int ST_BYTES = NRT * GLMH_TILE;
  static constexpr int PIECES = ST_BYTES / 1024;
  static constexpr int PW = PRIV ? GLMH_TILE / 1024 : (PIECES >= NW ? PIECES / NW : 1);
  static constexpr int DMA_WAVES = PRIV ? NW : PIECES / PW;
  static constexpr int NDMA = PW + 1;
  static constexpr int RING_BYTES = PRIV ? NW * NB * GLMH_TILE : NB * ST_BYTES;
  static constexpr int WROWS = 32 * NPT;
  static constexpr int WPL = WROWS * 64;
  static constexpr int OFS_WAUX = 2 * WPL;
  static constexpr int OFS_RING = OFS_WAUX + WROWS * 16;
  static constexpr int OFS_Y = OFS_RING + RING_BYTES;
  static constexpr int LDS_BYTES = OFS_Y + NB * 4 * 256;
  static_assert(!PRIV || (NRT_ == 2 && NPT_ == 2), "private rings: the 2 x 2 geometry only");
  static_assert(PW * DMA_WAVES == PIECES || PRIV, "the image pieces must divide over the issuing waves");
};

constexpr uint32_t F16_2P15 = 0x7800u;

__device__ __forceinline__ f32x16v glmh_keep(const f16x8& a, const f16x8& b, const f32x16v& c) {
  asm volatile("" : : "v"(a), "v"(b));
  return c;
}
#ifdef PA_GLMH_ABL_NOGEMM1
#define GLMH_MFMA1(a, b, c) glmh_keep(a, b, c)
#else
#define GLMH_MFMA1(a, b, c) __builtin_amdgcn_mfma_f32_32x32x16_f16(a, b, c, 0, 0, 0)
#endif
#ifdef PA_GLMH_ABL_NOGEMM2
#define GLMH_MFMA2(a, b, c) glmh_keep(a, b, c)
#else
#define GLMH_MFMA2(a, b, c) __builtin_amdgcn_mfma_f32_32x32x16_f16(a, b, c, 0, 0, 0)
#endif

#ifndef PA_GLMH_SCHED
#define PA_GLMH_SCHED 0
#endif
#ifndef PA_GLMH_DEFER
#define PA_GLMH_DEFER 0
#endif
#if PA_GLMH_SCHED
#define GLMH_SB() __builtin_amdgcn_sched_barrier(0)
#else
#define GLMH_SB() do { } while (0)
#endif

template <int NB, int OCC, bool GROUPED = false, bool PRIV = false, bool LIN = false, bool DRAW = false,
          int NRT_ = 2, int NPT_ = 2>
__global__ __launch_bounds__(64 * NRT_ * NPT_, OCC) void glm_planes_f16_kernel(
    const unsigned char* __restrict__ img, const float* __restrict__ y,
    const float* __restrict__ w, const float* __restrict__ b, int64_t N, int D, int P,
    int64_t nst, float* __restrict__ part, int prio_cus, const uint32_t* __restrict__ trailer,
    unsigned long long* __restrict__ tstamps, const GlmGroupArgs grp,
    const int64_t* __restrict__ gate, const double* __restrict__ moments = nullptr,
    const GlmDraw draw = GlmDraw{}) {
  if (gate != nullptr && *gate != 0) return;
  using C = GlmHCfg<NB, PRIV, NRT_, NPT_>;
  constexpr int NRT = C::NRT, NPT = C::NPT, ST_BYTES = C::ST_BYTES, PW = C::PW, WROWS = C::WROWS,
                WPL = C::WPL, NT = 64 * C::NW;
  static_assert(!GROUPED || (NRT == 2 && NPT == 2), "the grouped image: 2 x 2 only");
#ifdef PA_GLMH_Y_PER_WAVE
  constexpr bool YSHARE = !PRIV && !(NRT == 2 && NPT == 2);
#else
  constexpr bool YSHARE = !PRIV;
#endif
  extern __shared__ __attribute__((aligned(16))) unsigned char smem[];
  const int lane = threadIdx.x & 63;
  const int wave = __builtin_amdgcn_readfirstlane(threadIdx.x >> 6);
  const int l31 = lane & 31, h = lane >> 5;
  const int rt = wave / NPT, pt = wave % NPT;
  const int pbase = blockIdx.y * WROWS;

  if (tstamps != nullptr && threadIdx.x == 0)
    __hip_atomic_fetch_min(&tstamps[0], (unsigned long long)wall_clock64(), __ATOMIC_RELAXED,
                           __HIP_MEMORY_SCOPE_AGENT);
  const uint32_t lds_base = __builtin_amdgcn_readfirstlane((uint32_t)(uintptr_t)smem);
  int64_t grid = gridDim.x, first = blockIdx.x, st_end = nst, row_st0 = 0, n_rows = N;
  int64_t my_count = first < nst ? (nst - first + grid - 1) / grid : 0;
  int64_t w_stride = D;
  if constexpr (GROUPED) {
    const int64_t sg = blockIdx.x;
    first = grp.st_off[sg];
    st_end = grp.st_off[sg + 1];
    my_count = st_end - first;
    grid = 1;
    row_st0 = first;
    n_rows = grp.seg[3 * sg + 1] - grp.seg[3 * sg];
    w += grp.seg[3 * sg + 2] * D;
    w_stride = (int64_t)grp.G * D;
  }

  auto issue = [&](int64_t st, int bi) {
#ifdef PA_GLMH_ABL_NODMA
    return;
#endif
    const int64_t stc = st < st_end ? st : st_end - 1;
    const unsigned char* src = img + stc * ST_BYTES + (PRIV ? rt * GLMH_TILE : (wave * PW) * 1024) + lane * 16;
    const uint32_t dst = lds_base + C::OFS_RING +
                         (PRIV ? (wave * NB + bi) * GLMH_TILE : bi * ST_BYTES + (wave * PW) * 1024);
    if (PRIV || wave < C::DMA_WAVES) {
#pragma unroll
      for (int k = 0; k < PW; ++k) dma16(src + k * 1024, dst + k * 1024);
    }
    if constexpr (!YSHARE) {
      int64_t row = (stc * NRT + rt) * 32 + l31;
      if constexpr (!GROUPED) row = row < N ? row : N - 1;
      dma4(y + row, lds_base + C::OFS_Y + (bi * 4 + wave) * 256);
    } else if (wave == 0) {
      int64_t row = stc * (NRT * 32) + lane;
      if constexpr (!GROUPED) row = row < N ? row : N - 1;
      dma4(y + row, lds_base + C::OFS_Y + bi * 1024);
    }
  };
  const int my_ndma = !YSHARE ? C::NDMA : (wave < C::DMA_WAVES ? PW : 0) + (wave == 0 ? 1 : 0);
  auto wait_tiles_in_flight = [&](auto kconst) {
    constexpr int K = decltype(kconst)::value;
    if (my_ndma == PW + 1) wait_vmcnt<K * (PW + 1)>();
    else if (my_ndma == PW) wait_vmcnt<K * PW>();
    else wait_vmcnt<0>();
  };

#pragma unroll
  for (int k = 0; k < NB - 1; ++k) issue(first + k * grid, k);

  const int kx_l = (int)trailer[GLMH_KX + l31];
  float* sp_s = reinterpret_cast<float*>(smem + C::LDS_BYTES);
  if constexpr (DRAW) {
    if (threadIdx.x < 32) sp_s[threadIdx.x] = (int)threadIdx.x < D ? softplus_t<float>(draw.rho_w[threadIdx.x]) : 0.0f;
    else if (threadIdx.x == 32) sp_s[32] = draw.have_b ? softplus_t<float>(draw.rho_b[0]) : 0.0f;
    __syncthreads();
  }
#pragma unroll 1
  for (int pl0 = 0; pl0 < WROWS; pl0 += NT / 4) {
    const int pl = pl0 + (int)(threadIdx.x >> 2), s = threadIdx.x & 3;
    const int p = pbase + pl;
    float v[8];
    float mw = 0.0f;
    float wraw[8], braw = 0.0f;
    if constexpr (DRAW) {
      const uint64_t obase = draw.offset_dev ? *draw.offset_dev : 0;
      const bool store = blockIdx.x == 0 && p < P;
      float nrm[8];
      const int64_t i0 = (int64_t)p * D + 8 * s;
      if ((D & 3) == 0 && p < P) {
#pragma unroll
        for (int q = 0; q < 2; ++q) {
          const u32x4 blk = philox4x32_10(draw.seed, draw.off_w + obase + (uint64_t)(i0 >> 2) + q, 0);
          box_muller_f32(u32_to_unit_f32(blk.x), u32_to_unit_f32(blk.y), nrm[4 * q], nrm[4 * q + 1]);
          box_muller_f32(u32_to_unit_f32(blk.z), u32_to_unit_f32(blk.w), nrm[4 * q + 2], nrm[4 * q + 3]);
        }
      } else {
#pragma unroll
        for (int j = 0; j < 8; ++j)
          nrm[j] = (p < P && 8 * s + j < D)
                       ? philox_normal_f32(draw.seed, draw.off_w + obase, (uint64_t)(i0 + j)) : 0.0f;
      }
#pragma unroll
      for (int j = 0; j < 8; ++j) {
        const int d = 8 * s + j;
        wraw[j] = 0.0f;
        if (p < P && d < D) {
          const float sp = sp_s[d];
          wraw[j] = __builtin_fmaf(sp, nrm[j], draw.loc_w[d]);
          if (store) {
            draw.eps_w[i0 + j] = nrm[j];
            draw.z_w[i0 + j] = wraw[j];
            if (p == 0) {
              draw.scale_w[d] = sp;
              draw.lout_w[d] = draw.loc_w[d];
            }
          }
        }
      }
      if (draw.have_b && p < P) {
        const float eb_ = philox_normal_f32(draw.seed, draw.off_b + obase, (uint64_t)p);
        const float spb = sp_s[32];
        braw = __builtin_fmaf(spb, eb_, draw.loc_b[0]);
        if (store && s == 0) {
          draw.eps_b[p] = eb_;
          draw.z_b[p] = braw;
          if (p == 0) {
            draw.scale_b[0] = spb;
            draw.lout_b[0] = draw.loc_b[0];
          }
        }
      }
    } else {
#pragma unroll
      for (int j = 0; j < 8; ++j) {
        const int d = 8 * s + j;
        wraw[j] = (p < P && d < D) ? w[(int64_t)p * w_stride + d] : 0.0f;
      }
      braw = (p < P && b != nullptr) ? b[p] : 0.0f;
    }
#pragma unroll
    for (int j = 0; j < 8; ++j) {
      const int d = 8 * s + j;
      v[j] = (p < P && d < D) ? ldexpf(wraw[j] * GLMP_LOG2E, -(int)trailer[GLMH_KX + d]) : 0.0f;
      mw = __builtin_fmaxf(mw, __builtin_fabsf(v[j]));
    }
    mw = __builtin_fmaxf(mw, __shfl_xor(mw, 1));
    mw = __builtin_fmaxf(mw, __shfl_xor(mw, 2));
    const float b2 = braw * GLMP_LOG2E;
    const uint32_t mwb = __builtin_bit_cast(uint32_t, mw), bb = __builtin_bit_cast(uint32_t, b2) & 0x7fffffffu;
    const int ew = (int)(mwb >> 23), eb = (int)(bb >> 23);
    int kw = (mwb != 0u && ew != 0xff) ? 14 - (ew == 0 ? -127 : ew - 127) : GLMH_KNONE;
    const int kb = (bb != 0u && eb != 0xff) ? 29 - (eb == 0 ? -127 : eb - 127) : GLMH_KNONE;
    kw = kw < kb ? kw : kb;
    if (kw == GLMH_KNONE) kw = 0;
#pragma unroll
    for (int j = 0; j < 8; ++j) v[j] = ldexpf(v[j], kw);
    uint32_t p1[4], p2[4];
#pragma unroll
    for (int j = 0; j < 4; ++j) split_pair_f16(v[2 * j], v[2 * j + 1], p1[j], p2[j]);
    unsigned char* q = smem + (pl >> 5) * GLMP_PLANE + glmp_slot_ofs(pl & 31, s);
    *reinterpret_cast<uint4*>(q) = make_uint4(p1[0], p1[1], p1[2], p1[3]);
    *reinterpret_cast<uint4*>(q + WPL) = make_uint4(p2[0], p2[1], p2[2], p2[3]);
    if (s == 0) {
      const float bs = ldexpf(b2, kw - 15);
      uint32_t q1, q2, q3, dummy;
      split_pair_f16(bs, 0.0f, q1, q2);
      const float r2 = (bs - f16_lo(q1)) - f16_lo(q2);
      split_pair_f16(r2, 0.0f, q3, dummy);
      uint32_t* wx = reinterpret_cast<uint32_t*>(smem + C::OFS_WAUX) + 4 * pl;
      wx[0] = (q1 & 0xffffu) | (q2 << 16);
      wx[1] = q3 & 0xffffu;
      int kd = -kw;
      kd = kd > 126 ? 126 : (kd < -126 ? -126 : kd);
      wx[2] = __builtin_bit_cast(uint32_t, ldexpf(1.0f, kd));
      wx[3] = 0u;
    }
  }
  __syncthreads();

  const uint32_t* wx_l = reinterpret_cast<const uint32_t*>(smem + C::OFS_WAUX) + 4 * (pt * 32 + l31);
  const f16x8 b_aux = as_f16x8(h == 0 ? wx_l[0] : 0u, h == 0 ? wx_l[1] : 0u, 0u, 0u);
  const float dsc = __builtin_bit_cast(float, wx_l[2]);
  f32x16v gwacc;
#pragma unroll
  for (int r = 0; r < 16; ++r) gwacc[r] = 0.0f;
  float s_yl[2] = {0.0f, 0.0f}, s_abs[2] = {0.0f, 0.0f}, s_g[2] = {0.0f, 0.0f};
  float p_t[2] = {1.0f, 1.0f};
  int e_t[2] = {0, 0};

  const int a_ofs0 = glmp_slot_ofs(l31, h), a_ofs1 = glmp_slot_ofs(l31, 2 + h);
  const unsigned char* w_row = smem + pt * GLMP_PLANE;
  const int q = lane & 15, gi1 = (lane >> 4) & 1;
  const int tr_row = 4 * h + (q >> 2);
  const int tr_slot = 2 * gi1 + ((q & 3) >> 1), tr_in = (q & 1) * 8;
  const int tr_ofs_a = tr_row * 64 + ((tr_slot ^ h) << 4) + tr_in;
  const int tr_ofs_b = (tr_row + 8) * 64 + ((tr_slot ^ ((h + 2) & 3)) << 4) + tr_in;

  constexpr int TA[3] = {1, 0, 0};
  constexpr int TB[3] = {0, 1, 0};

  f16x8 wa0[2], wa1[2];
#pragma unroll
  for (int pl = 0; pl < 2; ++pl) {
    wa0[pl] = *reinterpret_cast<const f16x8*>(w_row + pl * WPL + a_ofs0);
    wa1[pl] = *reinterpret_cast<const f16x8*>(w_row + pl * WPL + a_ofs1);
  }

  auto prep_rows = [&](int b_, int64_t st_) -> bool {
    const int64_t rows_left = n_rows - ((st_ - row_st0) * NRT + rt) * 32;
    const bool okr = (int64_t)l31 < rows_left;
    if constexpr (!GROUPED) {
      if constexpr (!YSHARE) {
        float* ys_ = reinterpret_cast<float*>(smem + C::OFS_Y + (b_ * 4 + wave) * 256);
        if (lane < 32) ys_[lane] = okr ? __builtin_fmaf(ys_[lane], GLMH_GSCALE, -0.5f * GLMH_GSCALE) : 0.0f;
      } else if (wave == 0) {
        float* ys_ = reinterpret_cast<float*>(smem + C::OFS_Y + b_ * 1024);
        const int64_t left64 = n_rows - (st_ - row_st0) * (NRT * 32);
        ys_[lane] = (int64_t)lane < left64 ? __builtin_fmaf(ys_[lane], GLMH_GSCALE, -0.5f * GLMH_GSCALE) : 0.0f;
      }
    }
    return okr;
  };
  auto gemm1_aux = [&](bool okr) -> f32x16v {
    const uint32_t a0 = (h == 0 && okr) ? (F16_2P15 | (F16_2P15 << 16)) : 0u;
    const uint32_t a1 = (h == 0 && okr) ? F16_2P15 : 0u;
    const f32x16v zero = {};
    return GLMH_MFMA1(as_f16x8(a0, a1, 0u, 0u), b_aux, zero);
  };
  auto load_a = [&](const unsigned char* Xt, int c, f16x8 (&xa)[2]) {
    const int ao = c == 0 ? a_ofs0 : a_ofs1;
#pragma unroll
    for (int pl = 0; pl < 2; ++pl) xa[pl] = *reinterpret_cast<const f16x8*>(Xt + pl * GLMP_PLANE + ao);
  };
  auto elem1 = [&](float acc, float yh, int par) -> float {
#ifdef PA_GLMH_ABL_NOELEM
    return acc + yh;
#endif
    const float l2 = acc * dsc;
#ifdef PA_GLMH_ABL_NOTRANS
    const float e = __builtin_fabsf(l2) * -0.001f;
    const float t = e + 1.0f;
    const float inv = t * 0.5f;
#else
    const float e = __builtin_amdgcn_exp2f(-__builtin_fabsf(l2));
    const float t = e + 1.0f;
    const float inv = __builtin_amdgcn_rcpf(t);
#endif
    if constexpr (!LIN) s_yl[par] = __builtin_fmaf(yh, l2, s_yl[par]);
    asm("v_add_f32 %0, |%1|, %0" : "+v"(s_abs[par]) : "v"(l2));
    p_t[par] *= t;
    const float g = yh - __builtin_copysignf(__builtin_fmaf(inv, GLMH_GSCALE, -0.5f * GLMH_GSCALE), l2);
    s_g[par] += g;
    return g;
  };
  auto elem2 = [&](float acc0, float acc1, float yh0, float yh1, int chain, float& g0, float& g1) {
#if defined(PA_GLMH_ABL_NOELEM) || defined(PA_GLMH_ABL_NOTRANS)
    g0 = elem1(acc0, yh0, 0);
    g1 = elem1(acc1, yh1, 1);
    return;
#endif
    const float l0 = acc0 * dsc, l1 = acc1 * dsc;
#ifdef PA_GLMH_OLD_PAIR
    const float t0 = __builtin_amdgcn_exp2f(-__builtin_fabsf(l0)) + 1.0f;
    const float t1 = __builtin_amdgcn_exp2f(-__builtin_fabsf(l1)) + 1.0f;
    const float tt = t0 * t1;
    const float r = __builtin_amdgcn_rcpf(tt);
    const float inv0 = r * t1, inv1 = r * t0;
#else
    const float e0 = __builtin_amdgcn_exp2f(-__builtin_fabsf(l0));
    const float t1 = __builtin_amdgcn_exp2f(-__builtin_fabsf(l1)) + 1.0f;
    const float tt = __builtin_fmaf(e0, t1, t1);
    const float r = __builtin_amdgcn_rcpf(tt);
    const float inv0 = r * t1, inv1 = __builtin_fmaf(r, e0, r);
#endif
    if constexpr (!LIN) {
      s_yl[0] = __builtin_fmaf(yh0, l0, s_yl[0]);
      s_yl[1] = __builtin_fmaf(yh1, l1, s_yl[1]);
    }
    asm("v_add_f32 %0, |%1|, %0" : "+v"(s_abs[0]) : "v"(l0));
    asm("v_add_f32 %0, |%1|, %0" : "+v"(s_abs[1]) : "v"(l1));
    p_t[chain] *= tt;
    g0 = yh0 - __builtin_copysignf(__builtin_fmaf(inv0, GLMH_GSCALE, -0.5f * GLMH_GSCALE), l0);
    g1 = yh1 - __builtin_copysignf(__builtin_fmaf(inv1, GLMH_GSCALE, -0.5f * GLMH_GSCALE), l1);
    s_g[0] += g0;
    s_g[1] += g1;
  };
  auto renorm = [&]() {
#pragma unroll
    for (int c2 = 0; c2 < 2; ++c2) {
      e_t[c2] += __builtin_amdgcn_frexp_expf(p_t[c2]);
      p_t[c2] = __builtin_amdgcn_frexp_mantf(p_t[c2]);
    }
  };
  auto tr_wait = [&](v2u32 (&xlo)[2], v2u32 (&xhi)[2], f16x8 (&xb)[2]) {
    asm volatile("s_waitcnt lgkmcnt(0)"
                 : "+v"(xlo[0]), "+v"(xhi[0]), "+v"(xlo[1]), "+v"(xhi[1])
                 :
                 : "memory");
#pragma unroll
    for (int pl = 0; pl < 2; ++pl) {
      const u32x4v cc = {xlo[pl][0], xlo[pl][1], xhi[pl][0], xhi[pl][1]};
      xb[pl] = __builtin_bit_cast(f16x8, cc);
    }
  };
  auto tr_issue = [&](uint32_t tr_a, uint32_t tr_b, int kh, v2u32 (&xlo)[2], v2u32 (&xhi)[2]) {
#ifdef PA_GLMH_ABL_NOTR
    xlo[0] = xhi[0] = xlo[1] = xhi[1] = v2u32{tr_a, tr_b};
    return;
#endif
    const uint32_t a = tr_a + (kh ? 1024u : 0u), b2 = tr_b + (kh ? 1024u : 0u);
    asm volatile("ds_read_b64_tr_b16 %0, %1 offset:0" : "=v"(xlo[0]) : "v"(a));
    asm volatile("ds_read_b64_tr_b16 %0, %1 offset:0" : "=v"(xhi[0]) : "v"(b2));
    asm volatile("ds_read_b64_tr_b16 %0, %1 offset:2048" : "=v"(xlo[1]) : "v"(a));
    asm volatile("ds_read_b64_tr_b16 %0, %1 offset:2048" : "=v"(xhi[1]) : "v"(b2));
  };
  auto load_y = [&](const float* ys_, int kh, float (&yv)[8]) {
    const float4 y0 = *reinterpret_cast<const float4*>(ys_ + 16 * kh + 4 * h);
    const float4 y1 = *reinterpret_cast<const float4*>(ys_ + 16 * kh + 8 + 4 * h);
    yv[0] = y0.x; yv[1] = y0.y; yv[2] = y0.z; yv[3] = y0.w;
    yv[4] = y1.x; yv[5] = y1.y; yv[6] = y1.z; yv[7] = y1.w;
  };

  int64_t st = first;
  int bi = 0;
  const uint32_t prio_slot = (uint32_t)(blockIdx.x / prio_cus);
  uint64_t prio_clock = wall_clock64();

  f32x16v acc_cur = {};
  if (my_count > 0) {
    wait_tiles_in_flight(std::integral_constant<int, NB - 2>{});
    if constexpr (!PRIV) __builtin_amdgcn_s_barrier();
    const bool ok0 = prep_rows(0, st);
    acc_cur = gemm1_aux(ok0);
    const unsigned char* X0 = smem + C::OFS_RING + (PRIV ? wave * NB * GLMH_TILE : rt * GLMH_TILE);
    f16x8 xa[2];
    load_a(X0, 0, xa);
#pragma unroll
    for (int t = 0; t < 3; ++t)
      acc_cur = GLMH_MFMA1(xa[TA[t]], wa0[TB[t]], acc_cur);
    load_a(X0, 1, xa);
#pragma unroll
    for (int t = 0; t < 3; ++t)
      acc_cur = GLMH_MFMA1(xa[TA[t]], wa1[TB[t]], acc_cur);
  }
  int64_t it = 0;
#if PA_GLMH_DEFER
  f16x8 pend_ga[2] = {}, pend_xb[2] = {};
#endif
  auto tile = [&](const f32x16v& acc_cur, f32x16v& acc_nxt) {
#if defined(PA_GLMH_ABL_NOPRIO)
    if constexpr (false) {
      const uint32_t ph = 0;
#elif defined(PA_GLMH_PRIO_BY_TILE)
    if constexpr (OCC > 1) {
      const uint32_t ph = ((uint32_t)(it >> 2) + prio_slot) % (uint32_t)OCC;
#else
    if constexpr (OCC > 1) {
      const uint32_t ph = ((uint32_t)(prio_clock >> 8) + prio_slot) % (uint32_t)OCC;
#endif
      if (ph == 0) __builtin_amdgcn_s_setprio(0);
      else if (ph == 1) __builtin_amdgcn_s_setprio(1);
      else if (ph == 2) __builtin_amdgcn_s_setprio(2);
      else __builtin_amdgcn_s_setprio(3);
#if !defined(PA_GLMH_PRIO_BY_TILE)
      prio_clock = wall_clock64();
#endif
    }
    if ((it & 7) == 7) renorm();
    int bn = bi + 1 == NB ? 0 : bi + 1;
    wait_tiles_in_flight(std::integral_constant<int, NB - 3>{});
    if constexpr (!PRIV) __builtin_amdgcn_s_barrier();
    {
      int bf = bi + (NB - 1);
      bf = bf >= NB ? bf - NB : bf;
      issue(st + (NB - 1) * grid, bf);
    }
    const unsigned char* Xc = smem + C::OFS_RING + (PRIV ? (wave * NB + bi) * GLMH_TILE : bi * ST_BYTES + rt * GLMH_TILE);
    const unsigned char* Xn = smem + C::OFS_RING + (PRIV ? (wave * NB + bn) * GLMH_TILE : bn * ST_BYTES + rt * GLMH_TILE);
    const float* ysc = reinterpret_cast<const float*>(smem + C::OFS_Y +
                                                      (!YSHARE ? (bi * 4 + wave) * 256 : bi * 1024 + rt * 128));
    const uint32_t tr_a = (uint32_t)(uintptr_t)Xc + (uint32_t)tr_ofs_a;
    const uint32_t tr_b = (uint32_t)(uintptr_t)Xc + (uint32_t)tr_ofs_b;

    const bool okn = prep_rows(bn, st + grid);
    acc_nxt = gemm1_aux(okn);
    v2u32 xlo[2], xhi[2];
    f16x8 xa[2], xb[2];
    float yv[8], g[8];
    uint32_t g1[4], g2[4];

    tr_issue(tr_a, tr_b, 0, xlo, xhi);
    load_y(ysc, 0, yv);
    load_a(Xn, 0, xa);
#pragma unroll
    for (int t = 0; t < 3; ++t) {
      acc_nxt = GLMH_MFMA1(xa[TA[t]], wa0[TB[t]], acc_nxt);
#if PA_GLMH_DEFER
      gwacc = GLMH_MFMA2(pend_ga[TA[t]], pend_xb[TB[t]], gwacc);
#endif
      elem2(acc_cur[2 * t], acc_cur[2 * t + 1], yv[2 * t], yv[2 * t + 1], t & 1, g[2 * t], g[2 * t + 1]);
      GLMH_SB();
    }
    load_a(Xn, 1, xa);
#pragma unroll
    for (int t = 0; t < 3; ++t) {
      acc_nxt = GLMH_MFMA1(xa[TA[t]], wa1[TB[t]], acc_nxt);
      if (t == 0) {
        elem2(acc_cur[6], acc_cur[7], yv[6], yv[7], 1, g[6], g[7]);
// ... 4 lines not shown
      GLMH_SB();
    }
    tr_wait(xlo, xhi, xb);
    {
      const f16x8 ga[2] = {as_f16x8(g1[0], g1[1], g1[2], g1[3]), as_f16x8(g2[0], g2[1], g2[2], g2[3])};
      tr_issue(tr_a, tr_b, 1, xlo, xhi);
      load_y(ysc, 1, yv);
#pragma unroll
      for (int t = 0; t < 3; ++t) {
        if (GLMH_G_PIECE(t)) gwacc = GLMH_MFMA2(ga[TA[t]], xb[TB[t]], gwacc);
        const int q0 = t == 0 ? 0 : t + 1, q1 = t == 0 ? 2 : t + 2;
#pragma unroll
        for (int qp = q0; qp < q1; ++qp)
          elem2(acc_cur[8 + 2 * qp], acc_cur[9 + 2 * qp], yv[2 * qp], yv[2 * qp + 1], qp & 1, g[2 * qp],
                g[2 * qp + 1]);
        GLMH_SB();
      }
    }
    uint32_t h1[4], h2[4];
#pragma unroll
    for (int j = 0; j < 4; ++j) split_pair_g(g[2 * j], g[2 * j + 1], h1[j], h2[j]);
    tr_wait(xlo, xhi, xb);
    {
      const f16x8 ga[2] = {as_f16x8(h1[0], h1[1], h1[2], h1[3]), as_f16x8(h2[0], h2[1], h2[2], h2[3])};
#if PA_GLMH_DEFER
      pend_ga[0] = ga[0]; pend_ga[1] = ga[1];
      pend_xb[0] = xb[0]; pend_xb[1] = xb[1];
#else
#pragma unroll
      for (int t = 0; t < 3; ++t)
        if (GLMH_G_PIECE(t)) gwacc = GLMH_MFMA2(ga[TA[t]], xb[TB[t]], gwacc);
#endif
    }
    st += grid;
    bi = bn;
    ++it;
  };
  f32x16v acc_alt = {};
  if constexpr (OCC >= 4) {
    while (it < my_count) {
      tile(acc_cur, acc_alt);
      acc_cur = acc_alt;
    }
  } else {
    while (it + 1 < my_count) {
      tile(acc_cur, acc_alt);
      tile(acc_alt, acc_cur);
    }
    if (it < my_count) tile(acc_cur, acc_alt);
  }
#if PA_GLMH_DEFER
#pragma unroll
  for (int t = 0; t < 3; ++t) gwacc = GLMH_MFMA2(pend_ga[TA[t]], pend_xb[TB[t]], gwacc);
#endif
  wait_vmcnt<0>();
  __builtin_amdgcn_s_setprio(0);
  renorm();
  __syncthreads();

  constexpr int NPG = NPT / 2, REC2 = 2 * 1024 + 2 * 2 * 32;
  constexpr int RED_OFS = NPT > 2 ? 0 : C::OFS_RING;
  static_assert((NPT * 1024 + 2 * NPT * 64) * 4 <= C::LDS_BYTES - RED_OFS, "LDS too small");
  float* red = reinterpret_cast<float*>(smem + RED_OFS);
  float* red2 = red + NPT * 1024;
  const float g_dsc = 1.0f / GLMH_GSCALE;
  const float s_lg = (float)(e_t[0] + e_t[1]) + (__builtin_amdgcn_logf(p_t[0]) + __builtin_amdgcn_logf(p_t[1]));
  const float ll_acc = 0.69314718055994530942f *
                       ((s_yl[0] + s_yl[1]) * g_dsc - 0.5f * (s_abs[0] + s_abs[1]) - s_lg);
  const float gb_acc = (s_g[0] + s_g[1]) * g_dsc;
  for (int rr = 0; rr < NRT; ++rr) {
    if (rt == rr) {
#pragma unroll
      for (int r = 0; r < 16; ++r) {
        const int idx = (pt * 16 + r) * 64 + lane;
        red[idx] = (rr == 0 ? 0.0f : red[idx]) + ldexpf(gwacc[r], -(14 + kx_l));
      }
      const int i0 = (2 * pt) * 64 + lane, i1 = (2 * pt + 1) * 64 + lane;
      red2[i0] = (rr == 0 ? 0.0f : red2[i0]) + ll_acc;
      red2[i1] = (rr == 0 ? 0.0f : red2[i1]) + gb_acc;
    }
    __syncthreads();
  }
  for (int gi = 0; gi < NPG; ++gi) {
    const int pass = (int)blockIdx.y * NPG + gi;
    if ((int64_t)pass * 64 >= P) continue;
    float* rec = part + ((int64_t)pass * gridDim.x + blockIdx.x) * REC2;
    for (int i = threadIdx.x; i < 2 * 1024; i += NT) rec[i] = red[gi * 2048 + i];
    for (int i = threadIdx.x; i < 2 * 2 * 32; i += NT) {
      const int qq = i >> 5, j = i & 31, ptl = qq >> 1, which = qq & 1;
      const int src = (2 * (2 * gi + ptl) + which) * 64;
      float v = red2[src + j] + red2[src + 32 + j];
      if constexpr (LIN) {
        const int p = pass * 64 + ptl * 32 + j;
        if (blockIdx.x == 0 && which == 0 && p < P) {
          const float* wq = DRAW ? draw.z_w : w;
          const float* bq = DRAW ? (draw.have_b ? draw.z_b : nullptr) : b;
          double lin = bq != nullptr ? moments[32] * (double)bq[p] : 0.0;
          for (int d = 0; d < D; ++d) lin = __builtin_fma(moments[d], (double)wq[(int64_t)p * w_stride + d], lin);
          v += (float)lin;
        }
      }
      rec[2 * 1024 + i] = v;
    }
  }
  if (tstamps != nullptr && threadIdx.x == 0)
    __hip_atomic_fetch_max(&tstamps[1], (unsigned long long)wall_clock64(), __ATOMIC_RELAXED,
                           __HIP_MEMORY_SCOPE_AGENT);
}

}
```

### pyro_amd/csrc/multisite_dev.h

```cpp
#pragma once
#include "common.h"
#include "dist_fam.h"

namespace pa {

struct EntryDev {
  int dist, need;
  int64_t rows, cols;
  const void *v, *a, *b;
  const uint8_t* m;
  int64_t vsr, vsc, asr, asc, bsr, bsc, msr, msc;
  double coef;
  void *dv, *da, *db;
  int chain_next;
  const void* xg;
  double xcoef;
};
struct MultiArgs {
  int n;
  EntryDev e[PA_MULTI_MAX_ENTRIES];
};

template <typename S>
__device__ __forceinline__ S kernarg_load(uint32_t byte_offset) {
// ... 15 lines not shown
    if (pa_dbg_stamps != nullptr && blockIdx.x == 0 && threadIdx.x == 0 && pa_dbg_next < 30) \
      pa_dbg_stamps[32 + pa_dbg_next++] = wall_clock64();                               \
  } while (0)
#else
#define PA_DBG_STAMP() do { } while (0)
#endif

constexpr int MULTI_THREADS = 1024;
constexpr int UN = 8;
template <> struct NParams<PA_SITE_IDENTITY> { static constexpr int n = 1; };

template <typename T>
struct Elem {
  T v, a, b;
  bool keep;
};
template <int DIST, typename T>
__device__ __forceinline__ Elem<T> load_elem(const EntryDev& e, uint32_t r, uint32_t c, bool ok) {
  r = ok ? r : 0u;
  c = ok ? c : 0u;
  Elem<T> x;
  x.v = ((const T*)e.v)[r * (int32_t)e.vsr + c * (int32_t)e.vsc];
  x.a = T(0);
  x.b = T(0);
  if constexpr (DIST < PA_DIST_COUNT) {
    x.a = ((const T*)e.a)[r * (int32_t)e.asr + c * (int32_t)e.asc];
    if (NParams<DIST>::n > 1) x.b = ((const T*)e.b)[r * (int32_t)e.bsr + c * (int32_t)e.bsc];
  }
  x.keep = ok && (e.m == nullptr || e.m[r * (int32_t)e.msr + c * (int32_t)e.msc] != 0);
  return x;
}
template <int DIST, typename T>
__device__ __forceinline__ T elem_lp(const Elem<T>& x) {
  if constexpr (DIST == PA_SITE_IDENTITY) return x.v;
  else if constexpr (DIST == PA_SITE_NONE) return T(0);
  else return Fam<DIST, T>::lp(x.v, x.a, x.b);
}
template <int DIST, typename T>
__device__ __forceinline__ void elem_grad(const Elem<T>& x, T& gv, T& ga, T& gb) {
  if constexpr (DIST == PA_SITE_IDENTITY) { gv = T(1); ga = T(0); gb = T(0); }
  else if constexpr (DIST == PA_SITE_NONE) { gv = T(0); ga = T(0); gb = T(0); }
  else Fam<DIST, T>::grad(x.v, x.a, x.b, gv, ga, gb);
}

#define PA_DISPATCH_ENTRY(DIST_ID, CALL)                                                         \
  switch (DIST_ID) {                                                                             \
    case PA_DIST_NORMAL: { constexpr int D_ = PA_DIST_NORMAL; CALL; } break;                     \
    case PA_DIST_BERNOULLI_LOGITS: { constexpr int D_ = PA_DIST_BERNOULLI_LOGITS; CALL; } break; \
    case PA_DIST_HALF_CAUCHY: { constexpr int D_ = PA_DIST_HALF_CAUCHY; CALL; } break;           \
    case PA_DIST_LOG_NORMAL: { constexpr int D_ = PA_DIST_LOG_NORMAL; CALL; } break;             \
    case PA_DIST_EXPONENTIAL: { constexpr int D_ = PA_DIST_EXPONENTIAL; CALL; } break;           \
    case PA_DIST_HALF_NORMAL: { constexpr int D_ = PA_DIST_HALF_NORMAL; CALL; } break;           \
    case PA_DIST_GAMMA: { constexpr int D_ = PA_DIST_GAMMA; CALL; } break;                       \
    case PA_DIST_BETA: { constexpr int D_ = PA_DIST_BETA; CALL; } break;                         \
    case PA_DIST_POISSON: { constexpr int D_ = PA_DIST_POISSON; CALL; } break;                   \
    case PA_DIST_BINOMIAL_LOGITS: { constexpr int D_ = PA_DIST_BINOMIAL_LOGITS; CALL; } break;   \
    case PA_DIST_KL_NORMAL_LOC: { constexpr int D_ = PA_DIST_KL_NORMAL_LOC; CALL; } break;       \
    case PA_DIST_KL_NORMAL_SCALE: { constexpr int D_ = PA_DIST_KL_NORMAL_SCALE; CALL; } break;   \
    case PA_SITE_IDENTITY: { constexpr int D_ = PA_SITE_IDENTITY; CALL; } break;                 \
    default: { constexpr int D_ = PA_SITE_NONE; CALL; } break;                                   \
  }

constexpr int UNS = 4;
template <int DIST, typename T>
__device__ __forceinline__ double entry_sum(const EntryDev& e, uint32_t tid, uint32_t nth) {
  const uint32_t R = (uint32_t)e.rows, C = (uint32_t)e.cols;
  T acc = T(0);
  if constexpr (DIST == PA_SITE_NONE) return 0.0;
  const uint32_t tk = C < nth ? C : nth, ng = nth / tk;
  const uint32_t c0 = tid % tk, g = tid / tk;
  if (g >= ng) return 0.0;
  for (uint32_t c = c0; c < C; c += tk)
    for (uint32_t rb = g; rb < R; rb += UNS * ng) {
      Elem<T> x[UNS];
#pragma unroll
      for (int u = 0; u < UNS; ++u) x[u] = load_elem<DIST, T>(e, rb + u * ng, c, rb + u * ng < R);
#pragma unroll
      for (int u = 0; u < UNS; ++u) acc += x[u].keep ? elem_lp<DIST, T>(x[u]) : T(0);
    }
  return (double)acc;
}

template <typename T, int NTHREADS>
__device__ __forceinline__ double multi_sum_partial(uint32_t kbase, uint32_t skip_mask,
                                                    uint32_t only_mask) {
  const int n_entries = kernarg_load<int>(kbase + offsetof(MultiArgs, n));
  const int wave = __builtin_amdgcn_readfirstlane(threadIdx.x >> 6), lane = threadIdx.x & 63;
  constexpr int NW = NTHREADS / 64;
  const int wpe = n_entries >= NW ? 1 : NW / (n_entries > 0 ? n_entries : 1);
  const int epr = NW / wpe;
  double acc = 0.0;
  for (int k0 = 0; k0 < n_entries; k0 += epr) {
    const int k = k0 + wave / wpe;
    if (k < n_entries && wave / wpe < epr) {
      if ((skip_mask >> k & 1u) || (only_mask != 0u && !(only_mask >> k & 1u))) continue;
      const EntryDev e = kernarg_load<EntryDev>(kbase + offsetof(MultiArgs, e) + k * sizeof(EntryDev));
      const uint32_t tid = (uint32_t)((wave % wpe) * 64 + lane), nth = (uint32_t)(wpe * 64);
      double s = 0.0;
      PA_DISPATCH_ENTRY(e.dist, s = (entry_sum<D_, T>(e, tid, nth)));
      acc += e.coef * s;
    }
  }
  return acc;
}
template <typename T>
__device__ __forceinline__ void multi_sum_finish(double acc, T* __restrict__ out, double coef_all,
                                                 int accumulate) {
  __shared__ double smem[16];
  const double t = block_sum_f64(acc, smem);
  if (threadIdx.x == 0) {
    const double base = accumulate ? (double)*out : 0.0;
    *out = (T)(base + coef_all * t);
  }
}
template <typename T, int NTHREADS>
__device__ __forceinline__ void multi_sum_body(uint32_t kbase, T* __restrict__ out, double coef_all,
                                               int accumulate) {
  multi_sum_finish<T>(multi_sum_partial<T, NTHREADS>(kbase, 0u, 0u), out, coef_all, accumulate);
}

template <typename T>
__global__ __launch_bounds__(MULTI_THREADS) void multi_sum_kernel(const MultiArgs args_by_value,
                                                                  T* __restrict__ out,
                                                                  double coef_all, int accumulate) {
  multi_sum_body<T, MULTI_THREADS>(0u, out, coef_all, accumulate);
}

constexpr int GRAD_THREADS = 256;
__device__ __forceinline__ uint32_t row_groups(uint32_t tk) {
  const uint32_t ng = GRAD_THREADS / tk;
  return ng > 8u ? 8u : ng;
}
enum { PAT_SKIP = 0, PAT_FULL = 1, PAT_ROWRED = 2, PAT_SCALAR = 3, PAT_COLRED = 4 };
__device__ __forceinline__ int pattern_of(bool wanted, int64_t sr, int64_t sc, int64_t R, int64_t C) {
  if (!wanted) return PAT_SKIP;
  const bool red_r = (sr == 0 && R > 1), red_c = (sc == 0 && C > 1);
  return red_r ? (red_c ? PAT_SCALAR : PAT_ROWRED) : (red_c ? PAT_COLRED : PAT_FULL);
}

template <int DIST, typename T>
__device__ __forceinline__ void combined_pass(const EntryDev& e, double w, int pv, bool accumulate,
                                              const T* xg, T xw, int pa_, int pb_, double* red) {
#pragma clang fp contract(off)
  const uint32_t R = (uint32_t)e.rows, C = (uint32_t)e.cols, t = threadIdx.x;
  const uint32_t tk = C < GRAD_THREADS ? C : GRAD_THREADS, ng = row_groups(tk);
  const uint32_t c0 = t % tk, g = t / tk;
  T* dv = (T*)e.dv;
  T* da = (T*)e.da;
  T* db = (T*)e.db;
  const T wT = (T)w;
  T tot_a = T(0), tot_b = T(0);
  for (uint32_t cb = 0; cb < C; cb += tk) {
    const uint32_t c = cb + c0;
    const bool okc = g < ng && c < C;
    T col_a = T(0), col_b = T(0);
    for (uint32_t rb = g; rb < R; rb += UN * ng) {
      Elem<T> x[UN];
      T old[UN], ex[UN];
#pragma unroll
      for (int u = 0; u < UN; ++u) {
        const uint32_t r = rb + u * ng;
        const bool ok = okc && r < R;
        x[u] = load_elem<DIST, T>(e, r, c, ok);
        const uint32_t o = ok ? r * C + c : 0u;
        old[u] = (pv == PAT_FULL && accumulate) ? dv[o] : T(0);
        ex[u] = (pv == PAT_FULL && xg != nullptr) ? xg[o] : T(0);
      }
#pragma unroll
      for (int u = 0; u < UN; ++u) {
        const uint32_t r = rb + u * ng;
        const bool ok = okc && r < R;
        T gv, ga, gb;
        elem_grad<DIST, T>(x[u], gv, ga, gb);
        gv = x[u].keep ? gv : T(0);
        ga = x[u].keep ? ga : T(0);
        gb = x[u].keep ? gb : T(0);
        if (ok) {
          const uint32_t o = r * C + c;
          if (pv == PAT_FULL) dv[o] = old[u] + wT * gv + xw * ex[u];
          if (pa_ == PAT_FULL) da[o] = wT * ga;
          if (pb_ == PAT_FULL) db[o] = wT * gb;
        }
        col_a += ga;
        col_b += gb;
      }
    }
    tot_a += col_a;
    tot_b += col_b;
    if (pa_ == PAT_ROWRED || pb_ == PAT_ROWRED) {
      __syncthreads();
      red[t] = (double)col_a;
      red[GRAD_THREADS + t] = (double)col_b;
      __syncthreads();
// ... 457 lines not shown
```

### pyro_amd/csrc/runtime.hip

```cpp
#include "common.h"

#include <stdlib.h>
#include <string.h>

namespace pa {

static thread_local char g_err[512] = "";

void set_error(const char* fmt, ...) {
  va_list ap;
  va_start(ap, fmt);
  vsnprintf(g_err, sizeof(g_err), fmt, ap);
  va_end(ap);
}

int fail(int code, const char* fmt, ...) {
  va_list ap;
  va_start(ap, fmt);
  vsnprintf(g_err, sizeof(g_err), fmt, ap);
  va_end(ap);
  return code;
}

static int64_t* g_gate = nullptr;
static int64_t g_gate_launches = 0, g_gate_aware = 0;
struct GateDeferred {
  bool pending = false, emitted = false;
  const int64_t* go = nullptr;
  int64_t* gate = nullptr;
  int64_t* ack = nullptr;
  unsigned long long ticks = 0;
  int64_t pre = 0, pre_other = 0;
};
static GateDeferred g_gate_late;
const int64_t* gate_word() { return g_gate == nullptr ? nullptr : g_gate + 1; }
void gate_aware_launch() {
  if (!g_gate_late.pending) g_gate_aware += 1;
}

int check_launch(const char* what) {
  static const bool trace = getenv("PYRO_AMD_TRACE_LAUNCHES") != nullptr;
  if (trace) fprintf(stderr, "pyro_amd launch: %s%s\n", what, g_gate_late.pending ? "  (in front of a late gate)" : "");
  if (g_gate_late.pending) {
    g_gate_late.pre += 1;
    if (strncmp(what, "glm_planes_kernel", 17) != 0 || strchr(what, '<') != nullptr) g_gate_late.pre_other += 1;
  } else {
    g_gate_launches += 1;
  }
  hipError_t e = hipGetLastError();
  if (e != hipSuccess) return fail(PA_ERR_LAUNCH, "%s: %s", what, hipGetErrorString(e));
  return PA_OK;
}

int cu_count() {
  static int cached = 0;
  if (cached > 0) return cached;
  int dev = 0;
  if (hipGetDevice(&dev) != hipSuccess) return 256;
  int n = 0;
  if (hipDeviceGetAttribute(&n, hipDeviceAttributeMultiprocessorCount, dev) != hipSuccess || n <= 0)
    return 256;
  cached = n;
  return n;
}

static thread_local int g_br_tag = 0;
static thread_local hipEvent_t g_br_start = nullptr, g_br_stop = nullptr;

bool take_bracket(int tag, hipEvent_t* start, hipEvent_t* stop) {
  if (g_br_tag != tag || g_br_start == nullptr) return false;
  *start = g_br_start;
  *stop = g_br_stop;
  g_br_tag = 0;
  g_br_start = g_br_stop = nullptr;
  return true;
}

__global__ void gate_kernel(const int64_t* go, int64_t* gate, int64_t* ack, unsigned long long ticks) {
  const int64_t n = gate[0] + 1;
  const unsigned long long t0 = wall_clock64();
  int aborted = 0;
  for (unsigned iter = 0;; ++iter) {
    const int64_t v = __hip_atomic_load(go, __ATOMIC_RELAXED, __HIP_MEMORY_SCOPE_SYSTEM);
    if (v >= n) break;
    if (v == -n || wall_clock64() - t0 > ticks || iter > (1u << 22)) {
      aborted = 1;
      break;
    }
    __builtin_amdgcn_s_sleep(2);
  }
  __atomic_thread_fence(__ATOMIC_ACQUIRE);
  gate[1] = aborted;
  if (!aborted) {
    gate[0] = n;
  } else {
    __hip_atomic_store(ack, n, __ATOMIC_RELEASE, __HIP_MEMORY_SCOPE_SYSTEM);
  }
}

void gate_emit_deferred(hipStream_t s) {
  GateDeferred& d = g_gate_late;
  if (!d.pending) return;
  d.pending = false;
  d.emitted = true;
  g_gate = d.gate;
  hipLaunchKernelGGL(gate_kernel, dim3(1), dim3(1), 0, s, d.go, d.gate, d.ack, d.ticks);
  g_gate_aware += 1;
  (void)check_launch("gate_kernel");
}

}

extern "C" {

int pa_gate_defer(const int64_t* go, int64_t* gate, int64_t* ack, int64_t timeout_us) {
  PA_REQUIRE(go && gate && ack, "pa_gate_defer: NULL pointer");
  PA_REQUIRE(timeout_us > 0 && timeout_us <= 100000, "pa_gate_defer: timeout_us=%lld outside (0, 1e5]",
             (long long)timeout_us);
// ... 57 lines not shown
```

### pyro_amd/infer/svi.py

```python
import os as _os
import warnings

import torch
import torch.utils._python_dispatch

from .. import kernels, poutine
from ..params import _PARAM_STORE
from ..util import capture_scope, torch_isnan, zero_grads
from .elbo import ELBO


def _arg_key(x):
    if isinstance(x, torch.Tensor):
        return ("t", x.data_ptr(), tuple(x.shape), tuple(x.stride()), x.dtype, x.device)
    if isinstance(x, (list, tuple)):
        return tuple(_arg_key(v) for v in x)
    try:
        hash(x)
        return ("p", x)
    except TypeError:
        return ("id", id(x))


def _fast_geometry(args):
# ... 528 lines not shown
            entry.arm_penalty = 1
        return loss

    def _capture(self, key, args, kwargs):
        from .constants import HoistedConstantWritten
        rec = self._const_rec.pop(key, None)
        multi = hasattr(self.optim, "reduce_gradients") and getattr(self.optim, "multi_rank", False)
        forms = [False, True] if multi and not getattr(self, "_force_split", False) \
            and _os.environ.get("PYRO_AMD_GRAPH_COLLECTIVE", "1") != "0" else [None]
        for form in forms:
            gated = ("late" if self.speculate else True) if (self.prearm and not multi
                                                             and not self._eager_update) else False
            try:
                entry = self._capture_once(key, args, kwargs, rec, force_split=form,
                                           quiet=form is False, with_gate=gated)
            except HoistedConstantWritten:
                rec = None
                entry = self._capture_once(key, args, kwargs, None, force_split=form,
                                           quiet=form is False, with_gate=gated)
            while getattr(entry, "gate", None) is not None and not entry.gate.armable:
                if _os.environ.get("PYRO_AMD_DEBUG_GATE"):
                    g = entry.gate
                    print("pyro_amd: gate form %r not armable: launches %s gate-aware %s torch operators %s "
                          "emitted %s in front of a late gate %s (not the GLM kernel: %s)"
                          % (gated, g.total, g.aware, g.torch_ops, getattr(g, "emitted", None),
                             getattr(g, "pre", None), getattr(g, "pre_other", None)), flush=True)
                gated = True if gated == "late" else False
                self._drop(key)
                entry = self._capture_once(key, args, kwargs, rec, force_split=form,
                                           quiet=form is False, with_gate=gated)
            if entry is not None:
                return entry
            if form is False:
                warnings.warn("pyro_amd: capturing the gradient all-reduce inside the step's graph "
                              "failed; capturing the step in two graphs around an eager collective")
                self.hip_graph = True
        return None

    def _capture_once(self, key, args, kwargs, const_rec, force_split=None, quiet=False,
                      with_gate=False, _retried=False):
        from .. import rng
        from ..ops import fuser
        from ..primitives import validation_enabled

        compiled_before = fuser.STATS["loaded"]

        device = None
        for a in list(args) + list(kwargs.values()):
            if isinstance(a, torch.Tensor) and a.is_cuda:
                device = a.device
                break
        if device is None:
            device = torch.device("cuda", torch.cuda.current_device())
        cap = rng.GraphCapture(device)
        mailbox = (torch.zeros(1, dtype=torch.float64).pin_memory(),
                   torch.zeros(1, dtype=torch.int64).pin_memory())
        graph = kernels.new_graph()
        graph2 = between = None
        split = hasattr(self.optim, "reduce_gradients") and \
            (getattr(self.optim, "multi_rank", False) or getattr(self, "_force_split", False))
        if force_split is not None:
            split = bool(force_split)
        import contextlib
        chained = _os.environ.get("PYRO_AMD_CHAIN", "1") != "0"
        if chained:
            kernels.chain_sync_buffer(device)
        chain = lambda: kernels.chain_recording(device) if chained else contextlib.nullcontext()
        self.chain_stats = []
        if const_rec is not None and const_rec.calls:
            from .constants import ConstantReplayer
            consts = ConstantReplayer(const_rec)
        else:
            consts = None
        hoist = (lambda: consts) if consts is not None else contextlib.nullcontext
        gate = kernels.StepGate(device, late=(with_gate == "late")) \
            if (with_gate and chained and not split) else None
        gated = (lambda: gate) if gate is not None else contextlib.nullcontext
        try:
            with validation_enabled(False):
                multi = getattr(self.optim, "multi_rank", False)
                mode = {"capture_error_mode": "thread_local"} if (split or multi) else {}
                reads = _ReadSet()
                blocks = fuser.RtcBlocks()
                with capture_scope(), blocks, torch.cuda.graph(graph, **mode):
                    with fuser.scope(), gated(), cap, chain() as rec, hoist(), reads:
                        if gate is not None:
                            gate.launch()
                        with poutine.trace(param_only=True) as param_capture:
                            loss = self._loss_device(self.model, self.guide, *args, **kwargs)
                        params = self._params_of(param_capture)
                        loss = loss.detach() if isinstance(loss, torch.Tensor) else \
                            torch.full((), float(loss), device=device)
                        if not split and getattr(self.optim, "fused_publish", False):
                            self.optim(params, publish=cap.finish_args((loss,) + mailbox))
                        else:
                            if not split and not self._eager_update:
                                self.optim(params)
                                if not getattr(self.optim, "zeroes_grads", False):
                                    zero_grads(params)
                            cap.finish(publish=(loss,) + mailbox)
                    self.chain_stats.append(getattr(rec, "stats", None))
                    self.chain_fused = getattr(rec, "fused", 0)
                if split:
                    optim = self.optim
                    optim.reduce_gradients(params)
                    graph2 = torch.cuda.CUDAGraph()
                    blocks2 = fuser.RtcBlocks()
                    with capture_scope(), blocks2, torch.cuda.graph(graph2, pool=graph.pool(), **mode):
                        with chain():
                            optim.apply(params)
                            if not getattr(optim, "zeroes_grads", False):
                                zero_grads(params)
                    between = lambda: optim.reduce_gradients(params)
        except Exception as e:
            import os
            from .constants import HoistedConstantWritten
            for b_ in (locals().get("blocks"), locals().get("blocks2")):
                if b_ is not None:
                    b_.free()
            if isinstance(e, HoistedConstantWritten):
                raise
            if not _retried and fuser.STATS["loaded"] != compiled_before:
                return self._capture_once(key, args, kwargs, const_rec, force_split=force_split, quiet=quiet,
                                          with_gate=with_gate, _retried=True)
            if os.environ.get("PYRO_AMD_DEBUG_GRAPH"):
                raise
            if quiet or self._auto_graph:
                self.hip_graph = False
                return None
            warnings.warn("pyro_amd: hipGraph capture of SVI.step failed ({}: {}); continuing "
                          "with eager steps".format(type(e).__name__, e))
            self.hip_graph = False
            return None
        entry = _CapturedStep(graph, cap, loss, graph2, between, mailbox)
        if not split:
            entry.direct = kernels.graph_direct_plan(graph)
        if entry.direct is None and hasattr(graph, "instantiate"):
            for g_ in (graph, graph2):
                if g_ is not None:
                    try:
                        g_.instantiate()
                    except RuntimeError:
                        pass
        if self._eager_update and not split:
            entry.eager_params = list(params)
        entry.rtc_blocks = (blocks, blocks2 if split else None)
        entry.gate = gate
        entry.reads = tuple(reads.external.values())
        entry.constants = consts.tensors if consts is not None else []
        entry.constants_served = consts.served if consts is not None else 0
        self._graphs[key] = entry
        return entry
```

### pyro_amd/kernels.py

```python
import ctypes
import os

import torch
import torch.utils._python_dispatch

from . import _lib
from ._lib import NULL_VIEW, Unsupported, View2D, check

_DTYPES = {torch.float32: _lib.PA_F32, torch.float64: _lib.PA_F64}


def on_device(t):
    return t.is_cuda


def _require_gpu(*tensors):
    for t in tensors:
        if t is not None and not t.is_cuda:
            raise RuntimeError(
                "pyro_amd: kernel called with a tensor on %s; the HIP backend only runs on an "
                "MI355X device and has no CPU fallback" % t.device)


def _dtype(t):
# ... 64 lines not shown
        return None
    for hook in _PTR_HOOKS:
        hook(t)
    if _CHAIN["keep"] is not None:
        _CHAIN["keep"].append(t)
    return ctypes.c_void_p(t.data_ptr())


def _view(t, rows, cols):
    if t is None:
        return NULL_VIEW
    for hook in _PTR_HOOKS:
        hook(t)
    if _CHAIN["keep"] is not None:
        _CHAIN["keep"].append(t)
    assert t.dim() == 2
    sr = 0 if t.shape[0] == 1 and rows != 1 else t.stride(0)
    sc = 0 if t.shape[1] == 1 and cols != 1 else t.stride(1)
    if t.shape[0] == 1:
        sr = 0
    if t.shape[1] == 1:
        sc = 0
    return View2D(t.data_ptr(), sr, sc)


_CHAIN = {"keep": None, "sync": {}, "stats": None}

_FREE_OPS = None


def _free_ops():
    global _FREE_OPS
    if _FREE_OPS is None:
        a = torch.ops.aten
        names = ["empty.memory_format", "empty_strided.default", "empty_like.default",
                 "new_empty.default", "new_empty_strided.default", "detach.default", "alias.default",
                 "lift_fresh.default", "_unsafe_view.default", "_reshape_alias.default",
                 "is_same_size.default", "sym_size.int", "sym_stride.int", "sym_numel.default",
                 "sym_storage_offset.default", "is_pinned.default"]
        ops = set()
        for n in names:
            pkt, ov = n.split(".")
            try:
                ops.add(getattr(getattr(a, pkt), ov))
            except AttributeError:
                pass
        _FREE_OPS = ops
    return _FREE_OPS


def _launches_nothing(func):
    if func in _free_ops():
        return True
    try:
        return bool(func.is_view)
    except AttributeError:
        return False


class _ChainGuard(torch.utils._python_dispatch.TorchDispatchMode):
    def __torch_dispatch__(self, func, types, args=(), kwargs=None):
        if not _launches_nothing(func):
            if "torch_ops" in _CHAIN:
                _CHAIN["torch_ops"] += 1
            chain_flush()
        return func(*args, **(kwargs or {}))


def chain_sync_buffer(device):
    device = torch.device(device)
    key = (device.type, device.index if device.index is not None else torch.cuda.current_device())
    buf = _CHAIN["sync"].get(key)
    if buf is None:
        buf = torch.zeros((_lib.CHAIN_SYNC_BYTES // 4,), dtype=torch.int32, device=device)
        _CHAIN["sync"][key] = buf
    return buf


def chain_debug_stamps(buf):
    check(_lib.load().pa_chain_debug_stamps(None if buf is None else ctypes.c_void_p(buf.data_ptr())))
    _CHAIN["stamps"] = buf


def chain_tune(fuse_tail=True, fast_sites=True, jitter_seed=0, fuse_draw=True):
    check(_lib.load().pa_chain_tune((1 if fuse_tail else 0) | (0 if fast_sites else 2)
                                    | (0 if fuse_draw else 4) | ((int(jitter_seed) & 0x7fffff) << 8)))


def chain_flush():
    if _CHAIN["keep"] is not None:
        check(_lib.load().pa_chain_flush())


class chain_recording:

    def __init__(self, device):
        self.sync = chain_sync_buffer(device)
        self.stats = (0, 0)
        self.fused = 0
        self._guard = None

    def __enter__(self):
        assert _CHAIN["keep"] is None, "nested chain recordings"
        check(_lib.load().pa_chain_begin(_stream(), ctypes.c_void_p(self.sync.data_ptr()),
                                         self.sync.numel() * 4))
        _CHAIN["keep"] = []
        self._guard = _ChainGuard()
        self._guard.__enter__()
        return self

    def __exit__(self, *exc):
        try:
            self._guard.__exit__(*exc)
        finally:
            a, b = ctypes.c_int(0), ctypes.c_int(0)
            rc = _lib.load().pa_chain_end(ctypes.byref(a), ctypes.byref(b))
            _CHAIN["keep"] = None
            self.stats = (a.value, b.value)
            self.fused = _lib.load().pa_chain_fused_launches()
        if exc[0] is None:
            check(rc)
        return False



class KernelTimer:

    def __init__(self, kernel_tag):
        self.tag = kernel_tag
        self.pairs = []

    def arm(self):
        s = torch.cuda.Event(enable_timing=True)
        e = torch.cuda.Event(enable_timing=True)
        s.record()
        e.record()
        check(_lib.load().pa_profile_bracket_next(self.tag, ctypes.c_void_p(s.cuda_event),
                                                  ctypes.c_void_p(e.cuda_event)))
        self.pairs.append((s, e))

    def read_last(self):
        s, e = self.pairs[-1]
        return s.elapsed_time(e)

    def times_ms(self):
        return [s.elapsed_time(e) for s, e in self.pairs]

    def mean_ms(self):
        t = self.times_ms()
        return sum(t) / len(t) if t else float("nan")



def philox_normal(shape, dtype, device, seed, offset, offset_dev=None):
    out = torch.empty(shape, dtype=dtype, device=device)
    _require_gpu(out, offset_dev)
    check(_lib.load().pa_philox_normal(_ptr(out), out.numel(), _dtype(out), seed, offset,
                                       _ptr(offset_dev), _stream()))
    return out


def philox_uniform(shape, dtype, device, seed, offset, offset_dev=None):
    out = torch.empty(shape, dtype=dtype, device=device)
    _require_gpu(out, offset_dev)
    check(_lib.load().pa_philox_uniform(_ptr(out), out.numel(), _dtype(out), seed, offset,
                                        _ptr(offset_dev), _stream()))
    return out


def gamma_rsample(alpha, rows, cols, seed, offset, offset_dev=None, want_grad=True):
    _require_gpu(alpha, offset_dev)
    out = torch.empty((rows, cols), dtype=alpha.dtype, device=alpha.device)
    dal = torch.empty_like(out) if want_grad else None
    check(_lib.load().pa_gamma_rsample(_dtype(alpha), _ptr(out), _ptr(dal), _view(alpha, rows, cols),
                                       rows, cols, seed, offset, _ptr(offset_dev), _stream()))
    return out, dal


def gamma_implicit_grad(alpha, value):
    _require_gpu(alpha, value)
    a2, v2 = alpha.reshape(1, -1), value.reshape(1, -1)
    out = torch.empty_like(v2)
    check(_lib.load().pa_gamma_implicit_grad(_dtype(alpha), _ptr(out), _view(a2, 1, a2.shape[1]),
                                             _view(v2, 1, v2.shape[1]), 1, v2.shape[1], _stream()))
    return out.reshape(value.shape)


def publish_scalar(src, host_value, host_seq, counter=None, inc=0):
    _require_gpu(src, counter)
    assert host_value.is_pinned() and host_seq.is_pinned()
    assert host_value.dtype == torch.float64 and host_seq.dtype == torch.int64
    assert counter is None or (counter.dtype == torch.int64 and counter.numel() >= 2)
    check(_lib.load().pa_publish_scalar(_dtype(src), _ptr(src), _ptr(host_value), _ptr(host_seq),
                                        _ptr(counter), int(inc), _stream()))


def exp_site_fwd(u, cols, lower=0.0, want_ld=True):
    _require_gpu(u)
    assert u.is_contiguous() and u.dtype in (torch.float32, torch.float64) and cols >= 1
    rows = u.numel() // cols
    value = torch.empty_like(u)
    ld = torch.empty((rows,), dtype=u.dtype, device=u.device) if want_ld else None
# ... 1838 lines not shown
```

Measured before the change: 12500 ELBO-grad steps/s (64 particles x 1e6-row plate per step).

## Merge GLM planes kernel and chain tail into one persistent step kernel

Parks the GLM planes launch while a chain is recording and, when conditions allow, emits one merged kernel. In it the GLM workgroups signal arrival through a sync word and the tail roles (finalize, per-site grad, meanfield backward, Adam) wait on that word instead of a kernel boundary. The goal is to cut a launch and the inter-kernel drain and fill gap in each step's graph. It adds spin-wait dependencies inside one grid, which can stall if not all workgroups are resident, and the merge is turned off under direct replay.

```diff
diff --git a/include/pyro_amd.h b/include/pyro_amd.h
--- a/include/pyro_amd.h
+++ b/include/pyro_amd.h
@@ -418,6 +418,7 @@
 int pa_chain_pending(void);
 int pa_chain_tune(int fuse_tail);
 int pa_chain_fused_launches(void);
+int pa_chain_merged_launches(void);
 int pa_chain_debug_stamps(void* stamps32);
 
 #define PA_RTC_MAX_POINTERS 384
diff --git a/pyro_amd/_lib.py b/pyro_amd/_lib.py
--- a/pyro_amd/_lib.py
+++ b/pyro_amd/_lib.py
@@ -326,6 +326,7 @@
     "pa_chain_debug_stamps": (c_int, [c_void_p]),
     "pa_chain_tune": (c_int, [c_int]),
     "pa_chain_fused_launches": (c_int, []),
+    "pa_chain_merged_launches": (c_int, []),
     "pa_adam_step_publish": (c_int, [c_int, c_void_p, c_void_p, c_void_p, c_void_p, c_int64,
                                      c_double, c_double, c_double, c_double, c_double, c_double,
                                      c_double, c_int, c_void_p, c_int, c_int, c_void_p, c_void_p,
diff --git a/pyro_amd/csrc/chain.hip b/pyro_amd/csrc/chain.hip
--- a/pyro_amd/csrc/chain.hip
+++ b/pyro_amd/csrc/chain.hip
@@ -1,128 +1,7 @@
 #include "chain.h"
-#include "glm_finalize.h"
-#include "multisite_dev.h"
-#include "optim_dev.h"
-#include "site_tail.h"
+#include "chain_dev.h"
 
 namespace pa {
-
-constexpr int CH_FIN = 0, CH_MULTI = 1, CH_MF = 2, CH_ADAM = 3, CH_PHASES = 4;
-constexpr int CH_MF_SITES = 8;
-
-struct MfArgs8 {
-  int nsites;
-  MfSiteDev s[CH_MF_SITES];
-};
-static_assert(offsetof(MfArgs8, s) == offsetof(MfArgs, s), "layout");
-
-constexpr int CH_TAIL_ENTRIES = 6;
-struct TailSite {
-  int n_entries;
-  int entries[CH_TAIL_ENTRIES];
-  int extras_mask;
-  int64_t off_loc, off_rho;
-  int fast;
-  int layout;
-};
-
-struct ChainArgs {
-  MultiArgs multi;
-  MfArgs8 mf;
-  const float* fin_part;
-  float *fin_ll, *fin_gw, *fin_gb;
-  double fin_scale, fin_ll_offset;
-  int fin_nblocks, fin_npass, fin_D, fin_P, fin_DT, fin_PT;
-  float* multi_out;
-  const float* multi_g;
-  double multi_coef_all;
-  int multi_accumulate, multi_n;
-  int64_t mf_P;
-  int mf_gy, mf_nsites;
-  float *ad_p, *ad_g, *ad_m, *ad_v;
-  int64_t ad_n;
-  double ad_lr, ad_b1, ad_b2, ad_eps, ad_wd, ad_clip, ad_lrd;
-  int64_t* ad_step;
-  int ad_clipped, ad_zero;
-  AdamPublish ad_pub;
-  uint32_t* sync;
-  int have[CH_PHASES];
-  int grid[CH_PHASES];
-  int last;
-  uint64_t* stamps;
-  const int64_t* gate;
-  uint32_t jitter;
-  int tail_nsites;
-  uint32_t fin_dep_mask;
-  TailSite tail[CH_MF_SITES];
-};
-static_assert(sizeof(ChainArgs) <= 6144, "kernel arguments grew unexpectedly");
-
-__device__ __forceinline__ void chain_jitter(uint32_t seed, int p, uint32_t salt) {
-  if (seed == 0u) return;
-  uint32_t hsh = seed * 2654435761u ^ (blockIdx.x + 1u) * 40503u ^ (uint32_t)(p + 1) * 2246822519u ^ salt;
-  hsh ^= hsh >> 15;
-  hsh *= 2654435761u;
-  hsh ^= hsh >> 13;
-  const uint32_t n = (hsh >> 8) & 63u;
-  if ((hsh & 3u) == 0u) return;
-  for (uint32_t i = 0; i < n; ++i) __builtin_amdgcn_s_sleep(8);
-}
-
-__device__ __forceinline__ void chain_signal(uint32_t jitter, uint32_t* sync, int p, uint32_t expected,
-                                             bool last) {
-  chain_jitter(jitter, p, 0x9e3779b9u);
-  __syncthreads();
-  if (threadIdx.x == 0) {
-    __builtin_amdgcn_fence(__ATOMIC_RELEASE, "agent");
-    const uint32_t old =
-        __hip_atomic_fetch_add(&sync[p], 1u, __ATOMIC_RELAXED, __HIP_MEMORY_SCOPE_AGENT);
-    if (last && old == expected - 1u) {
-#pragma unroll
-      for (int q = 0; q < CH_PHASES; ++q)
-        __hip_atomic_store(&sync[q], 0u, __ATOMIC_RELAXED, __HIP_MEMORY_SCOPE_AGENT);
-    }
-  }
-}
-
-__device__ __forceinline__ void chain_wait(uint32_t jitter, uint32_t* sync, int p, uint32_t expected) {
-  if (threadIdx.x == 0) {
-    const uint64_t t0 = wall_clock64();
-    while (__hip_atomic_load(&sync[p], __ATOMIC_RELAXED, __HIP_MEMORY_SCOPE_AGENT) < expected) {
-      __builtin_amdgcn_s_sleep(2);
-      if (wall_clock64() - t0 > 400000000ull) __builtin_trap();
-    }
-    __builtin_amdgcn_fence(__ATOMIC_ACQUIRE, "agent");
-  }
-  __syncthreads();
-  chain_jitter(jitter, p, 0x85ebca6bu);
-}
-
-template <int DT, int PT, int SUB>
-__device__ __forceinline__ void chain_fin(const ChainArgs& a, int me, int nw) {
-  __shared__ double sm[SUB][FIN_GROUPS][FIN_OUT];
-  const int sub = SUB == 1 ? 0 : (int)(threadIdx.x >> 8), tid = (int)(threadIdx.x & 255);
-  for (int64_t base = (int64_t)me * SUB; base < a.grid[CH_FIN]; base += (int64_t)nw * SUB) {
-    glm_finalize_body<DT, PT>(base + sub, a.fin_part, a.fin_nblocks, a.fin_npass, a.fin_D, a.fin_P,
-                              a.fin_scale, a.fin_ll, a.fin_gw, a.fin_gb, a.fin_ll_offset, tid,
-                              sm[sub]);
-    __syncthreads();
-  }
-}
-template <int SUB>
-__device__ __forceinline__ void chain_fin_any(const ChainArgs& a, int me, int nw) {
-  if (a.fin_DT == 1 && a.fin_PT == 2) chain_fin<1, 2, SUB>(a, me, nw);
-  else if (a.fin_DT == 1 && a.fin_PT == 1) chain_fin<1, 1, SUB>(a, me, nw);
-  else if (a.fin_DT == 2 && a.fin_PT == 1) chain_fin<2, 1, SUB>(a, me, nw);
-  else if (a.fin_DT == 2 && a.fin_PT == 2) chain_fin<2, 2, SUB>(a, me, nw);
-  else if (a.fin_DT == 4 && a.fin_PT == 2) chain_fin<4, 2, SUB>(a, me, nw);
-  else chain_fin<4, 1, SUB>(a, me, nw);
-}
-
-#define PA_CHAIN_STAMP(i)                                                     \
-  do {                                                                        \
-    if (a.stamps != nullptr && threadIdx.x == 0 && (me == 0 || total_wg))     \
-      a.stamps[(total_wg ? 16 : 0) + (i)] = wall_clock64();                   \
-  } while (0)
 
 __global__ __launch_bounds__(1024) void chain_kernel(const ChainArgs a) {
   if (a.gate != nullptr && *a.gate != 0) return;
@@ -198,111 +77,7 @@
 
 __global__ __launch_bounds__(1024) void chain_tail_kernel(const ChainArgs a) {
   if (a.gate != nullptr && *a.gate != 0) return;
-  const bool total_wg = blockIdx.x == gridDim.x - 1;
-  const int nw = (int)gridDim.x - 1, me = (int)blockIdx.x;
-  uint32_t* sync = a.sync;
-  if (me < a.tail_nsites && threadIdx.x >= 256) return;
-  const int nfw = nw - a.tail_nsites;
-  const int fin_vwg = (a.grid[CH_FIN] + 3) / 4;
-  const int part_fin = fin_vwg < nfw ? fin_vwg : nfw;
-  PA_CHAIN_STAMP(0);
-  if (!total_wg && me >= a.tail_nsites) {
-    const int fme = me - a.tail_nsites;
-    if (a.have[CH_FIN] && fme < part_fin) {
-      chain_fin_any<4>(a, fme, nfw);
-      chain_signal(a.jitter, sync, CH_FIN, (uint32_t)part_fin, false);
-    }
-    return;
-  }
-  PA_CHAIN_STAMP(1);
-  constexpr uint32_t KB = (uint32_t)offsetof(ChainArgs, multi);
-  constexpr uint32_t KMF = (uint32_t)offsetof(ChainArgs, mf);
-  const uint32_t KT = (uint32_t)offsetof(ChainArgs, tail) + (uint32_t)me * (uint32_t)sizeof(TailSite);
-  auto tail_entry = [&](int q) -> int {
-    return kernarg_load<int>(KT + (uint32_t)offsetof(TailSite, entries) + 4u * (uint32_t)q);
-  };
-  int ts_n = 0, ts_mask = 0, ts_fast = 0;
-  int64_t step = 0;
-  if (!total_wg) ts_fast = kernarg_load<int>(KT + (uint32_t)offsetof(TailSite, fast));
-  if (!total_wg && ts_fast) {
-    __shared__ double fast_red[4 * GRAD_THREADS];
-    __shared__ float fast_xch[4 * 64];
-    const int layout = kernarg_load<int>(KT + (uint32_t)offsetof(TailSite, layout));
-    const EntryDev eh = kernarg_load<EntryDev>(KB + (uint32_t)offsetof(MultiArgs, e) +
-                                               (uint32_t)tail_entry(0) * (uint32_t)sizeof(EntryDev));
-    const EntryDev eg = kernarg_load<EntryDev>(KB + (uint32_t)offsetof(MultiArgs, e) +
-                                               (uint32_t)tail_entry(1) * (uint32_t)sizeof(EntryDev));
-    const MfSiteDev ms = kernarg_load<MfSiteDev>(KMF + (uint32_t)offsetof(MfArgs, s) +
-                                                 (uint32_t)me * (uint32_t)sizeof(MfSiteDev));
-    const int64_t off_loc = kernarg_load<int64_t>(KT + (uint32_t)offsetof(TailSite, off_loc));
-    const int64_t off_rho = kernarg_load<int64_t>(KT + (uint32_t)offsetof(TailSite, off_rho));
-    const SiteAdam ad{a.ad_p, a.ad_g, a.ad_m, a.ad_v, a.ad_step, a.ad_lr, a.ad_b1, a.ad_b2, a.ad_eps,
-                      a.ad_wd, a.ad_clip, a.ad_lrd, a.ad_clipped, a.ad_zero};
-    auto wait = [&]() {
-      PA_CHAIN_STAMP(7);
-      if (a.have[CH_FIN]) chain_wait(a.jitter, sync, CH_FIN, (uint32_t)part_fin);
-      else __syncthreads();
-      PA_CHAIN_STAMP(2);
-    };
-    site_fast<PA_DIST_NORMAL>(eh, eg, ms, layout, a.multi_coef_all, off_loc, off_rho, ad, fast_red,
-                              fast_xch, wait, &step);
-    PA_CHAIN_STAMP(5);
-  } else {
-  double total_acc = 0.0;
-  if (total_wg) {
-    total_acc = multi_sum_partial<float, MULTI_THREADS>(KB, a.fin_dep_mask, 0u);
-  }
-  if (!total_wg) {
-    ts_n = kernarg_load<int>(KT + (uint32_t)offsetof(TailSite, n_entries));
-    ts_mask = kernarg_load<int>(KT + (uint32_t)offsetof(TailSite, extras_mask));
-    for (int q = 0; q < ts_n; ++q) {
-      multi_grad_body<float>(KB, tail_entry(q), a.multi_g, a.multi_coef_all, GRAD_NO_EXTRAS);
-      __syncthreads();
-    }
-  }
-  PA_CHAIN_STAMP(7);
-  if (a.have[CH_FIN]) chain_wait(a.jitter, sync, CH_FIN, (uint32_t)part_fin);
-  PA_CHAIN_STAMP(2);
-  if (total_wg) {
-    total_acc += multi_sum_partial<float, MULTI_THREADS>(KB, 0u, a.fin_dep_mask);
-    multi_sum_finish<float>(total_acc, a.multi_out, a.multi_coef_all, a.multi_accumulate);
-    if (threadIdx.x == 0) step = a.ad_step[0] + 1;
-  } else {
-    for (int q = 0; q < ts_n; ++q)
-      if (ts_mask >> q & 1)
-        multi_grad_body<float>(KB, tail_entry(q), a.multi_g, a.multi_coef_all, GRAD_EXTRAS_ONLY);
-    __syncthreads();
-    PA_CHAIN_STAMP(3);
-    meanfield_sample_bwd_body<float>(KMF, (uint32_t)me, 0u, 1u, a.mf_P);
-    __syncthreads();
-    PA_CHAIN_STAMP(4);
-    const MfSiteDev ms = kernarg_load<MfSiteDev>(KMF + (uint32_t)offsetof(MfArgs, s) +
-                                                 (uint32_t)me * (uint32_t)sizeof(MfSiteDev));
-    const int64_t off_loc = kernarg_load<int64_t>(KT + (uint32_t)offsetof(TailSite, off_loc));
-    const int64_t off_rho = kernarg_load<int64_t>(KT + (uint32_t)offsetof(TailSite, off_rho));
-    adam_two_ranges<float>(off_loc, off_rho, ms.n, a.ad_p, a.ad_g, a.ad_m, a.ad_v, a.ad_step,
-                           a.ad_lr, a.ad_b1, a.ad_b2, a.ad_eps, a.ad_wd, a.ad_clip, a.ad_lrd,
-                           a.ad_clipped, a.ad_zero, &step);
-    PA_CHAIN_STAMP(5);
-  }
-  }
-  __syncthreads();
-  if (threadIdx.x == 0) {
-    __builtin_amdgcn_fence(__ATOMIC_RELEASE, "agent");
-    const unsigned long long ticket = __hip_atomic_fetch_add(
-        reinterpret_cast<unsigned long long*>(a.ad_step + 1), 1ull, __ATOMIC_RELAXED,
-        __HIP_MEMORY_SCOPE_AGENT);
-    if (ticket == (unsigned long long)a.tail_nsites) {
-      __builtin_amdgcn_fence(__ATOMIC_ACQUIRE, "agent");
-      a.ad_step[1] = 0;
-      a.ad_step[0] = step;
-#pragma unroll
-      for (int q = 0; q < CH_PHASES; ++q)
-        __hip_atomic_store(&sync[q], 0u, __ATOMIC_RELAXED, __HIP_MEMORY_SCOPE_AGENT);
-      publish_to_host(a.ad_pub);
-    }
-  }
-  PA_CHAIN_STAMP(6);
+  chain_tail_roles<false>(a, (int)blockIdx.x, (int)gridDim.x - 1, blockIdx.x == gridDim.x - 1);
 }
 
 static int g_chain_fast_sites = 1;
@@ -426,6 +201,7 @@
   int launches = 0;
   int phases = 0;
   int fused = 0;
+  int merged = 0;
   ChainArgs a;
 };
 static ChainState g_chain;
@@ -433,9 +209,16 @@
 static int g_chain_fuse = 1;
 static uint32_t g_chain_jitter = 0;
 
+static int g_step_merge = 1;
+
+bool chain_may_park(pa_stream_t stream) {
+  return g_chain.on && g_step_merge && g_chain_fuse && (hipStream_t)stream == g_chain.stream &&
+         gate_word() == nullptr && !gate_deferred_pending();
+}
+
 static int chain_launch() {
   ChainState& c = g_chain;
-  if (c.top < 0) return PA_OK;
+  if (c.top < 0) return glm_emit_parked();
   ChainArgs& a = c.a;
   int maxgrid = 1, np = 0;
   for (int p = 0; p < CH_PHASES; ++p)
@@ -445,6 +228,27 @@
       if (a.grid[p] > maxgrid) maxgrid = a.grid[p];
     }
   a.stamps = g_chain_stamps;
+  a.glm_wgs = a.glm_draws = 0;
+  const bool merge = glm_parked() && g_step_merge && g_chain_fuse && a.have[CH_FIN] && gate_word() == nullptr &&
+                     !gate_deferred_pending() && cu_count() - 1 > CH_MF_SITES;
+  a.tail_nsites = 0;
+  if (merge && chain_plan_tail(a)) {
+    a.gate = nullptr;
+    a.jitter = g_chain_jitter;
+    const int tail_wgs = a.tail_nsites + a.grid[CH_FIN] + 1;
+    c.top = -1;
+    const int rc = glm_emit_merged(a, tail_wgs);
+    c.fused += 1;
+    c.merged += 1;
+    c.launches += 1;
+    c.phases += np;
+    for (int p = 0; p < CH_PHASES; ++p) a.have[p] = 0;
+    return rc;
+  }
+  if (glm_parked()) {
+    const int rc = glm_emit_parked();
+    if (rc != PA_OK) return rc;
+  }
   gate_emit_deferred(c.stream);
   a.gate = gate_word();
   a.jitter = g_chain_jitter;
@@ -621,7 +425,7 @@
 
 hipStream_t as_stream(pa_stream_t s) {
   if (g_draw.have) (void)chain_flush_draw();
-  if (g_chain.on && g_chain.top >= 0) (void)chain_launch();
+  if ((g_chain.on && g_chain.top >= 0) || glm_parked()) (void)chain_launch();
   return (hipStream_t)s;
 }
 
@@ -636,7 +440,7 @@
   pa::g_chain.on = true;
   pa::g_chain.stream = (hipStream_t)stream;
   pa::g_chain.top = -1;
-  pa::g_chain.launches = pa::g_chain.phases = pa::g_chain.fused = 0;
+  pa::g_chain.launches = pa::g_chain.phases = pa::g_chain.fused = pa::g_chain.merged = 0;
   for (int p = 0; p < pa::CH_PHASES; ++p) pa::g_chain.a.have[p] = 0;
   pa::g_chain.a.sync = (uint32_t*)sync_words;
   return PA_OK;
@@ -667,10 +471,13 @@
   pa::g_chain_fast_sites = (fuse_tail & 2) ? 0 : 1;
   pa::g_chain_jitter = (uint32_t)fuse_tail >> 8;
   pa::g_draw_enabled = (fuse_tail & 4) ? 0 : 1;
+  pa::g_step_merge = (fuse_tail & 8) ? 0 : 1;
   return PA_OK;
 }
 
 int pa_chain_fused_launches(void) { return pa::g_chain.fused; }
+
+int pa_chain_merged_launches(void) { return pa::g_chain.merged; }
 
 int pa_chain_debug_stamps(void* stamps32) {
   pa::g_chain_stamps = (uint64_t*)stamps32;
diff --git a/pyro_amd/csrc/chain_dev.h b/pyro_amd/csrc/chain_dev.h
--- /dev/null
+++ b/pyro_amd/csrc/chain_dev.h
@@ -0,0 +1,283 @@
+#pragma once
+#include "chain.h"
+#include "glm_finalize.h"
+#include "multisite_dev.h"
+#include "optim_dev.h"
+#include "site_tail.h"
+
+namespace pa {
+
+constexpr int CH_FIN = 0, CH_MULTI = 1, CH_MF = 2, CH_ADAM = 3, CH_PHASES = 4;
+constexpr int CH_SYNC_GLM = 4, CH_SYNC_DRAW = 5, CH_SYNC_WORDS = 6;
+static_assert(CH_SYNC_WORDS * 4 <= PA_CHAIN_SYNC_BYTES, "sync block too small");
+constexpr int CH_MF_SITES = 8;
+
+struct MfArgs8 {
+  int nsites;
+  MfSiteDev s[CH_MF_SITES];
+};
+static_assert(offsetof(MfArgs8, s) == offsetof(MfArgs, s), "layout");
+
+constexpr int CH_TAIL_ENTRIES = 6;
+struct TailSite {
+  int n_entries;
+  int entries[CH_TAIL_ENTRIES];
+  int extras_mask;
+  int64_t off_loc, off_rho;
+  int fast;
+  int layout;
+};
+
+struct ChainArgs {
+  MultiArgs multi;
+  MfArgs8 mf;
+  const float* fin_part;
+  float *fin_ll, *fin_gw, *fin_gb;
+  double fin_scale, fin_ll_offset;
+  int fin_nblocks, fin_npass, fin_D, fin_P, fin_DT, fin_PT;
+  float* multi_out;
+  const float* multi_g;
+  double multi_coef_all;
+  int multi_accumulate, multi_n;
+  int64_t mf_P;
+  int mf_gy, mf_nsites;
+  float *ad_p, *ad_g, *ad_m, *ad_v;
+  int64_t ad_n;
+  double ad_lr, ad_b1, ad_b2, ad_eps, ad_wd, ad_clip, ad_lrd;
+  int64_t* ad_step;
+  int ad_clipped, ad_zero;
+  AdamPublish ad_pub;
+  uint32_t* sync;
+  int have[CH_PHASES];
+  int grid[CH_PHASES];
+  int last;
+  uint64_t* stamps;
+  const int64_t* gate;
+  uint32_t jitter;
+  int tail_nsites;
+  uint32_t fin_dep_mask;
+  TailSite tail[CH_MF_SITES];
+  int glm_wgs, glm_draws;
+};
+static_assert(sizeof(ChainArgs) <= 6144, "kernel arguments grew unexpectedly");
+
+__device__ __forceinline__ void chain_jitter(uint32_t seed, int p, uint32_t salt) {
+  if (seed == 0u) return;
+  uint32_t hsh = seed * 2654435761u ^ (blockIdx.x + 1u) * 40503u ^ (uint32_t)(p + 1) * 2246822519u ^ salt;
+  hsh ^= hsh >> 15;
+  hsh *= 2654435761u;
+  hsh ^= hsh >> 13;
+  const uint32_t n = (hsh >> 8) & 63u;
+  if ((hsh & 3u) == 0u) return;
+  for (uint32_t i = 0; i < n; ++i) __builtin_amdgcn_s_sleep(8);
+}
+
+__device__ __forceinline__ void chain_signal(uint32_t jitter, uint32_t* sync, int p, uint32_t expected,
+                                             bool last) {
+  chain_jitter(jitter, p, 0x9e3779b9u);
+  __syncthreads();
+  if (threadIdx.x == 0) {
+    __builtin_amdgcn_fence(__ATOMIC_RELEASE, "agent");
+    const uint32_t old =
+        __hip_atomic_fetch_add(&sync[p], 1u, __ATOMIC_RELAXED, __HIP_MEMORY_SCOPE_AGENT);
+    if (last && old == expected - 1u) {
+#pragma unroll
+      for (int q = 0; q < CH_PHASES; ++q)
+        __hip_atomic_store(&sync[q], 0u, __ATOMIC_RELAXED, __HIP_MEMORY_SCOPE_AGENT);
+    }
+  }
+}
+
+__device__ __forceinline__ void chain_wait(uint32_t jitter, uint32_t* sync, int p, uint32_t expected) {
+  if (threadIdx.x == 0) {
+    const uint64_t t0 = wall_clock64();
+    while (__hip_atomic_load(&sync[p], __ATOMIC_RELAXED, __HIP_MEMORY_SCOPE_AGENT) < expected) {
+      __builtin_amdgcn_s_sleep(2);
+      if (wall_clock64() - t0 > 400000000ull) __builtin_trap();
+    }
+    __builtin_amdgcn_fence(__ATOMIC_ACQUIRE, "agent");
+  }
+  __syncthreads();
+  chain_jitter(jitter, p, 0x85ebca6bu);
+}
+
+template <int DT, int PT, int SUB>
+__device__ __forceinline__ void chain_fin(const ChainArgs& a, int me, int nw) {
+  __shared__ double sm[SUB][FIN_GROUPS][FIN_OUT];
+  const int sub = SUB == 1 ? 0 : (int)(threadIdx.x >> 8), tid = (int)(threadIdx.x & 255);
+  for (int64_t base = (int64_t)me * SUB; base < a.grid[CH_FIN]; base += (int64_t)nw * SUB) {
+    glm_finalize_body<DT, PT>(base + sub, a.fin_part, a.fin_nblocks, a.fin_npass, a.fin_D, a.fin_P,
+                              a.fin_scale, a.fin_ll, a.fin_gw, a.fin_gb, a.fin_ll_offset, tid,
+                              sm[sub]);
+    __syncthreads();
+  }
+}
+template <int SUB>
+__device__ __forceinline__ void chain_fin_any(const ChainArgs& a, int me, int nw) {
+  if (a.fin_DT == 1 && a.fin_PT == 2) chain_fin<1, 2, SUB>(a, me, nw);
+  else if (a.fin_DT == 1 && a.fin_PT == 1) chain_fin<1, 1, SUB>(a, me, nw);
+  else if (a.fin_DT == 2 && a.fin_PT == 1) chain_fin<2, 1, SUB>(a, me, nw);
+  else if (a.fin_DT == 2 && a.fin_PT == 2) chain_fin<2, 2, SUB>(a, me, nw);
+  else if (a.fin_DT == 4 && a.fin_PT == 2) chain_fin<4, 2, SUB>(a, me, nw);
+  else chain_fin<4, 1, SUB>(a, me, nw);
+}
+
+#define PA_CHAIN_STAMP(i)                                                     \
+  do {                                                                        \
+    if (a.stamps != nullptr && threadIdx.x == 0 && (me == 0 || total_wg))     \
+      a.stamps[(total_wg ? 16 : 0) + (i)] = wall_clock64();                   \
+  } while (0)
+
+template <bool MERGED>
+__device__ __forceinline__ void chain_tail_roles(const ChainArgs& a, const int me, const int nw,
+                                                 const bool total_wg) {
+  uint32_t* sync = a.sync;
+  if (me < a.tail_nsites && threadIdx.x >= 256) return;
+  const int nfw = nw - a.tail_nsites;
+  const int fin_vwg = MERGED ? a.grid[CH_FIN] : (a.grid[CH_FIN] + 3) / 4;
+  const int part_fin = fin_vwg < nfw ? fin_vwg : nfw;
+  PA_CHAIN_STAMP(0);
+  if (!total_wg && me >= a.tail_nsites) {
+    const int fme = me - a.tail_nsites;
+    if (a.have[CH_FIN] && fme < part_fin) {
+      if constexpr (MERGED) {
+        chain_wait(a.jitter, sync, CH_SYNC_GLM, (uint32_t)a.glm_wgs);
+        chain_fin_any<1>(a, fme, nfw);
+      } else {
+        chain_fin_any<4>(a, fme, nfw);
+      }
+      chain_signal(a.jitter, sync, CH_FIN, (uint32_t)part_fin, false);
+    }
+    return;
+  }
+  PA_CHAIN_STAMP(1);
+  if constexpr (MERGED) {
+    if (a.glm_draws > 0) chain_wait(a.jitter, sync, CH_SYNC_DRAW, (uint32_t)a.glm_draws);
+  }
+  constexpr uint32_t KB = (uint32_t)offsetof(ChainArgs, multi);
+  constexpr uint32_t KMF = (uint32_t)offsetof(ChainArgs, mf);
+  const uint32_t KT = (uint32_t)offsetof(ChainArgs, tail) + (uint32_t)me * (uint32_t)sizeof(TailSite);
+  auto tail_entry = [&](int q) -> int {
+    return kernarg_load<int>(KT + (uint32_t)offsetof(TailSite, entries) + 4u * (uint32_t)q);
+  };
+  int ts_n = 0, ts_mask = 0, ts_fast = 0;
+  int64_t step = 0;
+  if (!total_wg) ts_fast = kernarg_load<int>(KT + (uint32_t)offsetof(TailSite, fast));
+  if (!total_wg && ts_fast) {
+    __shared__ double fast_red[4 * GRAD_THREADS];
+    __shared__ float fast_xch[4 * 64];
+    const int layout = kernarg_load<int>(KT + (uint32_t)offsetof(TailSite, layout));
+    const EntryDev eh = kernarg_load<EntryDev>(KB + (uint32_t)offsetof(MultiArgs, e) +
+                                               (uint32_t)tail_entry(0) * (uint32_t)sizeof(EntryDev));
+    const EntryDev eg = kernarg_load<EntryDev>(KB + (uint32_t)offsetof(MultiArgs, e) +
+                                               (uint32_t)tail_entry(1) * (uint32_t)sizeof(EntryDev));
+    const MfSiteDev ms = kernarg_load<MfSiteDev>(KMF + (uint32_t)offsetof(MfArgs, s) +
+                                                 (uint32_t)me * (uint32_t)sizeof(MfSiteDev));
+    const int64_t off_loc = kernarg_load<int64_t>(KT + (uint32_t)offsetof(TailSite, off_loc));
+    const int64_t off_rho = kernarg_load<int64_t>(KT + (uint32_t)offsetof(TailSite, off_rho));
+    const SiteAdam ad{a.ad_p, a.ad_g, a.ad_m, a.ad_v, a.ad_step, a.ad_lr, a.ad_b1, a.ad_b2, a.ad_eps,
+                      a.ad_wd, a.ad_clip, a.ad_lrd, a.ad_clipped, a.ad_zero};
+    auto wait = [&]() {
+      PA_CHAIN_STAMP(7);
+      if (a.have[CH_FIN]) chain_wait(a.jitter, sync, CH_FIN, (uint32_t)part_fin);
+      else __syncthreads();
+      PA_CHAIN_STAMP(2);
+    };
+    site_fast<PA_DIST_NORMAL>(eh, eg, ms, layout, a.multi_coef_all, off_loc, off_rho, ad, fast_red,
+                              fast_xch, wait, &step);
+    PA_CHAIN_STAMP(5);
+  } else {
+  double total_acc = 0.0;
+  bool total_done = false;
+  if (total_wg) {
+    if constexpr (MERGED) {
+      double tv0 = 0.0, tv1 = 0.0, tv2 = 0.0, tv3 = 0.0;
+      const int pwave = __builtin_amdgcn_readfirstlane(threadIdx.x >> 6);
+#pragma unroll 1
+      for (int pass = 0; pass < 2; ++pass) {
+        if (pass == 1) {
+          PA_CHAIN_STAMP(7);
+          if (a.have[CH_FIN]) chain_wait(a.jitter, sync, CH_FIN, (uint32_t)part_fin);
+          PA_CHAIN_STAMP(2);
+        }
+        const uint32_t skip = pass == 0 ? a.fin_dep_mask : 0u, only = pass == 0 ? 0u : a.fin_dep_mask;
+#pragma unroll 1
+        for (int j = 0; j < 4; ++j) {
+          const double sj = multi_sum_partial_as<float, MULTI_THREADS>(
+              KB, skip, only, __builtin_amdgcn_readfirstlane(pwave + 4 * j), (int)(threadIdx.x & 63));
+          if (j == 0) tv0 += sj;
+          else if (j == 1) tv1 += sj;
+          else if (j == 2) tv2 += sj;
+          else tv3 += sj;
+        }
+      }
+      multi_sum_finish_v4<float>(tv0, tv1, tv2, tv3, pwave, a.multi_out, a.multi_coef_all, a.multi_accumulate);
+      if (threadIdx.x == 0) step = a.ad_step[0] + 1;
+      total_done = true;
+    } else {
+      total_acc = multi_sum_partial<float, MULTI_THREADS>(KB, a.fin_dep_mask, 0u);
+    }
+  }
+  if (!total_wg) {
+    ts_n = kernarg_load<int>(KT + (uint32_t)offsetof(TailSite, n_entries));
+    ts_mask = kernarg_load<int>(KT + (uint32_t)offsetof(TailSite, extras_mask));
+    for (int q = 0; q < ts_n; ++q) {
+      multi_grad_body<float>(KB, tail_entry(q), a.multi_g, a.multi_coef_all, GRAD_NO_EXTRAS);
+      __syncthreads();
+    }
+  }
+  if (!total_done) {
+    PA_CHAIN_STAMP(7);
+    if (a.have[CH_FIN]) chain_wait(a.jitter, sync, CH_FIN, (uint32_t)part_fin);
+    PA_CHAIN_STAMP(2);
+  }
+  if (total_wg) {
+    if (!total_done) {
+      total_acc += multi_sum_partial<float, MULTI_THREADS>(KB, 0u, a.fin_dep_mask);
+      multi_sum_finish<float>(total_acc, a.multi_out, a.multi_coef_all, a.multi_accumulate);
+      if (threadIdx.x == 0) step = a.ad_step[0] + 1;
+    }
+  } else {
+    for (int q = 0; q < ts_n; ++q)
+      if (ts_mask >> q & 1)
+        multi_grad_body<float>(KB, tail_entry(q), a.multi_g, a.multi_coef_all, GRAD_EXTRAS_ONLY);
+    __syncthreads();
+    PA_CHAIN_STAMP(3);
+    meanfield_sample_bwd_body<float>(KMF, (uint32_t)me, 0u, 1u, a.mf_P);
+    __syncthreads();
+    PA_CHAIN_STAMP(4);
+    const MfSiteDev ms = kernarg_load<MfSiteDev>(KMF + (uint32_t)offsetof(MfArgs, s) +
+                                                 (uint32_t)me * (uint32_t)sizeof(MfSiteDev));
+    const int64_t off_loc = kernarg_load<int64_t>(KT + (uint32_t)offsetof(TailSite, off_loc));
+    const int64_t off_rho = kernarg_load<int64_t>(KT + (uint32_t)offsetof(TailSite, off_rho));
+    adam_two_ranges<float>(off_loc, off_rho, ms.n, a.ad_p, a.ad_g, a.ad_m, a.ad_v, a.ad_step,
+                           a.ad_lr, a.ad_b1, a.ad_b2, a.ad_eps, a.ad_wd, a.ad_clip, a.ad_lrd,
+                           a.ad_clipped, a.ad_zero, &step);
+    PA_CHAIN_STAMP(5);
+  }
+  }
+  __syncthreads();
+  if (threadIdx.x == 0) {
+    __builtin_amdgcn_fence(__ATOMIC_RELEASE, "agent");
+    const unsigned long long ticket = __hip_atomic_fetch_add(
+        reinterpret_cast<unsigned long long*>(a.ad_step + 1), 1ull, __ATOMIC_RELAXED,
+        __HIP_MEMORY_SCOPE_AGENT);
+    if (ticket == (unsigned long long)a.tail_nsites) {
+      __builtin_amdgcn_fence(__ATOMIC_ACQUIRE, "agent");
+      a.ad_step[1] = 0;
+      a.ad_step[0] = step;
+#pragma unroll
+      for (int q = 0; q < (MERGED ? CH_SYNC_WORDS : CH_PHASES); ++q)
+        __hip_atomic_store(&sync[q], 0u, __ATOMIC_RELAXED, __HIP_MEMORY_SCOPE_AGENT);
+      publish_to_host(a.ad_pub);
+    }
+  }
+  PA_CHAIN_STAMP(6);
+}
+
+bool glm_parked();
+int glm_emit_parked();
+int glm_emit_merged(ChainArgs& a, int tail_wgs);
+bool chain_may_park(pa_stream_t stream);
+
+}
diff --git a/pyro_amd/csrc/common.h b/pyro_amd/csrc/common.h
--- a/pyro_amd/csrc/common.h
+++ b/pyro_amd/csrc/common.h
@@ -22,6 +22,7 @@
 const int64_t* gate_word();
 void gate_aware_launch();
 void gate_emit_deferred(hipStream_t s);
+bool gate_deferred_pending();
 bool take_bracket(int tag, hipEvent_t* start, hipEvent_t* stop);
 
 #define PA_REQUIRE(cond, ...)                                  \
diff --git a/pyro_amd/csrc/glm.hip b/pyro_amd/csrc/glm.hip
--- a/pyro_amd/csrc/glm.hip
+++ b/pyro_amd/csrc/glm.hip
@@ -6,6 +6,7 @@
 #include "glm_planes16d.h"
 #include "glm_finalize.h"
 #include "chain.h"
+#include "chain_dev.h"
 
 namespace pa {
 
@@ -562,6 +563,90 @@
   gate_aware_launch();
 }
 
+struct GlmStepArgs {
+  const unsigned char* img;
+  const float *y, *w, *b;
+  int64_t N, nst;
+  int D, P, prio_cus, nblocks, npass;
+  float* part;
+  const uint32_t* trailer;
+  unsigned long long* tstamps;
+  const double* moments;
+  GlmDraw draw;
+};
+
+template <bool LIN, bool DRAW>
+__global__ __launch_bounds__(256, 2) void step_kernel(const ChainArgs a, const GlmStepArgs g) {
+  extern __shared__ __attribute__((aligned(16))) unsigned char smem_raw[];
+  const int nglm = g.nblocks * g.npass;
+  if ((int)blockIdx.x < nglm) {
+    typedef __attribute__((address_space(3))) unsigned char lds_byte;
+    lds_byte* const dyn = (lds_byte*)smem_raw;
+    unsigned char* const smem0 = (unsigned char*)(dyn - (uint32_t)(uintptr_t)dyn);
+    const int by = (int)blockIdx.x / g.nblocks, bx = (int)blockIdx.x - by * g.nblocks;
+    glm_planes_f16_body<3, 3, false, false, LIN, DRAW, 2, 2>(
+        smem0, bx, by, g.nblocks, g.img, g.y, g.w, g.b, g.N, g.D, g.P, g.nst, g.part, g.prio_cus,
+        g.trailer, g.tstamps, GlmGroupArgs{nullptr, nullptr, 1}, g.moments, g.draw, a.sync + CH_SYNC_GLM,
+        a.jitter);
+    return;
+  }
+  const int me = (int)blockIdx.x - nglm, nw = (int)gridDim.x - nglm - 1;
+  chain_tail_roles<true>(a, me, nw, blockIdx.x == gridDim.x - 1);
+}
+
+struct ParkedGlm {
+  bool have = false, lin = false, draw = false, br = false;
+  GlmPlanesPlan pl;
+  GlmStepArgs g;
+  hipStream_t s = nullptr;
+  hipEvent_t ev0 = nullptr, ev1 = nullptr;
+};
+static ParkedGlm g_parked;
+
+bool glm_parked() { return g_parked.have; }
+
+int glm_emit_parked() {
+  ParkedGlm& k = g_parked;
+  if (!k.have) return PA_OK;
+  k.have = false;
+  const GlmStepArgs& g = k.g;
+  if (k.br) (void)hipEventRecord(k.ev0, k.s);
+  if (k.lin && k.draw)
+    glmh_launch_one<3, 3, false, true, true>(k.pl, g.img, g.y, g.w, g.b, g.N, g.D, g.P, g.part, g.trailer, k.s, g.moments, g.draw);
+  else if (k.lin)
+    glmh_launch_one<3, 3, false, true>(k.pl, g.img, g.y, g.w, g.b, g.N, g.D, g.P, g.part, g.trailer, k.s, g.moments);
+  else if (k.draw)
+    glmh_launch_one<3, 3, false, false, true>(k.pl, g.img, g.y, g.w, g.b, g.N, g.D, g.P, g.part, g.trailer, k.s, nullptr, g.draw);
+  else glmh_launch_one<3, 3>(k.pl, g.img, g.y, g.w, g.b, g.N, g.D, g.P, g.part, g.trailer, k.s);
+  if (k.br) (void)hipEventRecord(k.ev1, k.s);
+  return check_launch("glm_planes_kernel");
+}
+
+template <bool LIN, bool DRAW>
+static void glms_launch(const ChainArgs& a, const GlmStepArgs& g, int grid, hipStream_t s) {
+  auto k = step_kernel<LIN, DRAW>;
+  constexpr int lds = GlmHCfg<3, false>::LDS_BYTES + (DRAW ? 256 : 0);
+  (void)hipFuncSetAttribute((const void*)k, hipFuncAttributeMaxDynamicSharedMemorySize, lds);
+  hipLaunchKernelGGL(k, dim3((unsigned)grid), dim3(256), lds, s, a, g);
+}
+
+int glm_emit_merged(ChainArgs& a, int tail_wgs) {
+  ParkedGlm& k = g_parked;
+  if (!k.have) return fail(PA_ERR_INVALID, "glm_emit_merged: no parked launch");
+  k.have = false;
+  a.glm_wgs = k.pl.nblocks * k.pl.npass;
+  a.glm_draws = k.draw ? k.pl.npass : 0;
+  const int grid = a.glm_wgs + tail_wgs;
+  if (k.br) (void)hipEventRecord(k.ev0, k.s);
+  if (k.lin && k.draw) glms_launch<true, true>(a, k.g, grid, k.s);
+  else if (k.lin) glms_launch<true, false>(a, k.g, grid, k.s);
+  else if (k.draw) glms_launch<false, true>(a, k.g, grid, k.s);
+  else glms_launch<false, false>(a, k.g, grid, k.s);
+  if (k.br) (void)hipEventRecord(k.ev1, k.s);
+  gate_aware_launch();
+  return check_launch("step_kernel");
+}
+
 template <int DT, int OCC>
 static int glmd_launch(const unsigned char* img, const float* y, const float* w, const float* b, int64_t N,
                        int D, int P, float* part, const uint32_t* trailer, int bpc, int* nblocks_out,
@@ -1102,9 +1187,11 @@
   const bool wide = format == PA_GLM_PLANES_F16X2 && (pl.nb == 9 || pl.nb == 10) && pl.bpc <= 2;
   float* part = (float*)workspace;
   const unsigned char* img = (const unsigned char*)planes;
+  const bool park = format == PA_GLM_PLANES_F16X2 && pl.npt == 2 && !wide && pl.nb == 3 && pl.bpc < 4 &&
+                    pa::chain_may_park(stream);
   hipEvent_t ev0, ev1;
   const bool br = pa::take_bracket(PA_KERNEL_GLM, &ev0, &ev1);
-  if (br) (void)hipEventRecord(ev0, s);
+  if (br && !park) (void)hipEventRecord(ev0, s);
   const double ll_offset = (double)((wide ? (N + 127) / 128 * 128 : pl.nst * 32 * pl.nrt) - N) * 0.6931471805599453;
   pa::GlmFinArgs fin;
   fin.counters = nullptr;
@@ -1122,7 +1209,19 @@
   fin.tstamps = pa::g_planes_stamps;
   if (format == PA_GLM_PLANES_F16X2) {
     const uint32_t* trailer = (const uint32_t*)(img + pa::glmh_tile_bytes(pa::glm_planes_tiles(N)));
-    if (pl.npt == 4 && moments != nullptr) pa::glmh_launch_wide<2, 4, true>(pl, img, y, w, b, N, (int)D, (int)P, part, trailer, s, moments);
+    if (park) {
+      pa::ParkedGlm& k = pa::g_parked;
+      k.have = true;
+      k.lin = moments != nullptr;
+      k.draw = drawn;
+      k.pl = pl;
+      k.g = pa::GlmStepArgs{img, y, w, b, N, pl.nst, (int)D, (int)P, pa::cu_count(), pl.nblocks, pl.npass, part,
+                            trailer, pa::g_planes_stamps, moments, drawn ? draw : pa::GlmDraw{}};
+      k.s = s;
+      k.br = br;
+      k.ev0 = br ? ev0 : nullptr;
+      k.ev1 = br ? ev1 : nullptr;
+    } else if (pl.npt == 4 && moments != nullptr) pa::glmh_launch_wide<2, 4, true>(pl, img, y, w, b, N, (int)D, (int)P, part, trailer, s, moments);
     else if (pl.npt == 4) pa::glmh_launch_wide<2, 4, false>(pl, img, y, w, b, N, (int)D, (int)P, part, trailer, s, nullptr);
     else if (pl.npt == 8 && moments != nullptr) pa::glmh_launch_wide<1, 8, true>(pl, img, y, w, b, N, (int)D, (int)P, part, trailer, s, moments);
     else if (pl.npt == 8) pa::glmh_launch_wide<1, 8, false>(pl, img, y, w, b, N, (int)D, (int)P, part, trailer, s, nullptr);
@@ -1144,14 +1243,18 @@
   } else {
     pa::glm_planes_launch_one<4, 2>(pl, img, y, w, b, N, (int)D, (int)P, part, fin, s);
   }
-  if (br) (void)hipEventRecord(ev1, s);
-  int rc = pa::check_launch("glm_planes_kernel");
+  if (br && !park) (void)hipEventRecord(ev1, s);
+  int rc = park ? PA_OK : pa::check_launch("glm_planes_kernel");
   if (rc != PA_OK) return rc;
   if (fin.counters != nullptr) return PA_OK;
   const int64_t J = (int64_t)P * D + 2 * P;
   rc = pa::chain_record_fin(stream, 1, 2, part, pl.nblocks, pl.npass, (int)D, (int)P, scale, ll, gw,
                             gb, ll_offset);
-  if (rc != 0) return rc < 0 ? rc : PA_OK;
+  if (rc != 0) {
+    if (rc < 0 && pa::glm_parked()) (void)pa::glm_emit_parked();
+    return rc < 0 ? rc : PA_OK;
+  }
+  if (pa::glm_parked() && (rc = pa::glm_emit_parked()) != PA_OK) return rc;
   hipLaunchKernelGGL((pa::glm_finalize_kernel<1, 2>),
                      dim3((unsigned)((J + pa::FIN_OUT - 1) / pa::FIN_OUT)),
                      dim3(pa::FIN_OUT * pa::FIN_GROUPS), 0, s, part, pl.nblocks, pl.npass, (int)D,
diff --git a/pyro_amd/csrc/glm_planes16.h b/pyro_amd/csrc/glm_planes16.h
--- a/pyro_amd/csrc/glm_planes16.h
+++ b/pyro_amd/csrc/glm_planes16.h
@@ -207,16 +207,26 @@
 #define GLMH_SB() do { } while (0)
 #endif
 
-template <int NB, int OCC, bool GROUPED = false, bool PRIV = false, bool LIN = false, bool DRAW = false,
-          int NRT_ = 2, int NPT_ = 2>
-__global__ __launch_bounds__(64 * NRT_ * NPT_, OCC) void glm_planes_f16_kernel(
+__device__ __forceinline__ void glm_arrival_jitter(uint32_t seed, uint32_t salt) {
+  if (seed == 0u) return;
+  uint32_t hsh = seed * 2654435761u ^ (blockIdx.x + 1u) * 40503u ^ (salt + 7u) * 2246822519u;
+  hsh ^= hsh >> 15;
+  hsh *= 2654435761u;
+  hsh ^= hsh >> 13;
+  if ((hsh & 3u) == 0u) return;
+  const uint32_t n = (hsh >> 8) & 63u;
+  for (uint32_t i = 0; i < n; ++i) __builtin_amdgcn_s_sleep(8);
+}
+
+template <int NB, int OCC, bool GROUPED, bool PRIV, bool LIN, bool DRAW, int NRT_, int NPT_>
+__device__ __forceinline__ void glm_planes_f16_body(
+    unsigned char* __restrict__ smem, const int bx, const int by, const int gx,
     const unsigned char* __restrict__ img, const float* __restrict__ y,
     const float* __restrict__ w, const float* __restrict__ b, int64_t N, int D, int P,
     int64_t nst, float* __restrict__ part, int prio_cus, const uint32_t* __restrict__ trailer,
-    unsigned long long* __restrict__ tstamps, const GlmGroupArgs grp,
-    const int64_t* __restrict__ gate, const double* __restrict__ moments = nullptr,
-    const GlmDraw draw = GlmDraw{}) {
-  if (gate != nullptr && *gate != 0) return;
+    unsigned long long* __restrict__ tstamps, const GlmGroupArgs& grp,
+    const double* __restrict__ moments, const GlmDraw& draw, uint32_t* __restrict__ arrive,
+    uint32_t jitter) {
   using C = GlmHCfg<NB, PRIV, NRT_, NPT_>;
   constexpr int NRT = C::NRT, NPT = C::NPT, ST_BYTES = C::ST_BYTES, PW = C::PW, WROWS = C::WROWS,
                 WPL = C::WPL, NT = 64 * C::NW;
@@ -226,22 +236,21 @@
 #else
   constexpr bool YSHARE = !PRIV;
 #endif
-  extern __shared__ __attribute__((aligned(16))) unsigned char smem[];
   const int lane = threadIdx.x & 63;
   const int wave = __builtin_amdgcn_readfirstlane(threadIdx.x >> 6);
   const int l31 = lane & 31, h = lane >> 5;
   const int rt = wave / NPT, pt = wave % NPT;
-  const int pbase = blockIdx.y * WROWS;
+  const int pbase = by * WROWS;
 
   if (tstamps != nullptr && threadIdx.x == 0)
     __hip_atomic_fetch_min(&tstamps[0], (unsigned long long)wall_clock64(), __ATOMIC_RELAXED,
                            __HIP_MEMORY_SCOPE_AGENT);
   const uint32_t lds_base = __builtin_amdgcn_readfirstlane((uint32_t)(uintptr_t)smem);
-  int64_t grid = gridDim.x, first = blockIdx.x, st_end = nst, row_st0 = 0, n_rows = N;
+  int64_t grid = gx, first = bx, st_end = nst, row_st0 = 0, n_rows = N;
   int64_t my_count = first < nst ? (nst - first + grid - 1) / grid : 0;
   int64_t w_stride = D;
   if constexpr (GROUPED) {
-    const int64_t sg = blockIdx.x;
+    const int64_t sg = bx;
     first = grp.st_off[sg];
     st_end = grp.st_off[sg + 1];
     my_count = st_end - first;
@@ -301,7 +310,7 @@
     float wraw[8], braw = 0.0f;
     if constexpr (DRAW) {
       const uint64_t obase = draw.offset_dev ? *draw.offset_dev : 0;
-      const bool store = blockIdx.x == 0 && p < P;
+      const bool store = bx == 0 && p < P;
       float nrm[8];
       const int64_t i0 = (int64_t)p * D + 8 * s;
       if ((D & 3) == 0 && p < P) {
@@ -394,6 +403,15 @@
     }
   }
   __syncthreads();
+  if constexpr (DRAW) {
+    if (arrive != nullptr && bx == 0) {
+      glm_arrival_jitter(jitter, 1u);
+      if (threadIdx.x == 0) {
+        __builtin_amdgcn_fence(__ATOMIC_RELEASE, "agent");
+        (void)__hip_atomic_fetch_add(&arrive[1], 1u, __ATOMIC_RELAXED, __HIP_MEMORY_SCOPE_AGENT);
+      }
+    }
+  }
 
   const uint32_t* wx_l = reinterpret_cast<const uint32_t*>(smem + C::OFS_WAUX) + 4 * (pt * 32 + l31);
   const f16x8 b_aux = as_f16x8(h == 0 ? wx_l[0] : 0u, h == 0 ? wx_l[1] : 0u, 0u, 0u);
@@ -540,7 +558,7 @@
 
   int64_t st = first;
   int bi = 0;
-  const uint32_t prio_slot = (uint32_t)(blockIdx.x / prio_cus);
+  const uint32_t prio_slot = (uint32_t)(bx / prio_cus);
   uint64_t prio_clock = wall_clock64();
 
   f32x16v acc_cur = {};
@@ -711,9 +729,9 @@
     __syncthreads();
   }
   for (int gi = 0; gi < NPG; ++gi) {
-    const int pass = (int)blockIdx.y * NPG + gi;
+    const int pass = by * NPG + gi;
     if ((int64_t)pass * 64 >= P) continue;
-    float* rec = part + ((int64_t)pass * gridDim.x + blockIdx.x) * REC2;
+    float* rec = part + ((int64_t)pass * gx + bx) * REC2;
     for (int i = threadIdx.x; i < 2 * 1024; i += NT) rec[i] = red[gi * 2048 + i];
     for (int i = threadIdx.x; i < 2 * 2 * 32; i += NT) {
       const int qq = i >> 5, j = i & 31, ptl = qq >> 1, which = qq & 1;
@@ -721,7 +739,7 @@
       float v = red2[src + j] + red2[src + 32 + j];
       if constexpr (LIN) {
         const int p = pass * 64 + ptl * 32 + j;
-        if (blockIdx.x == 0 && which == 0 && p < P) {
+        if (bx == 0 && which == 0 && p < P) {
           const float* wq = DRAW ? draw.z_w : w;
           const float* bq = DRAW ? (draw.have_b ? draw.z_b : nullptr) : b;
           double lin = bq != nullptr ? moments[32] * (double)bq[p] : 0.0;
@@ -732,9 +750,33 @@
       rec[2 * 1024 + i] = v;
     }
   }
+  if (arrive != nullptr) {
+    glm_arrival_jitter(jitter, 0u);
+    __syncthreads();
+    if (threadIdx.x == 0) {
+      __builtin_amdgcn_fence(__ATOMIC_RELEASE, "agent");
+      (void)__hip_atomic_fetch_add(&arrive[0], 1u, __ATOMIC_RELAXED, __HIP_MEMORY_SCOPE_AGENT);
+    }
+  }
   if (tstamps != nullptr && threadIdx.x == 0)
     __hip_atomic_fetch_max(&tstamps[1], (unsigned long long)wall_clock64(), __ATOMIC_RELAXED,
                            __HIP_MEMORY_SCOPE_AGENT);
 }
 
-}
+template <int NB, int OCC, bool GROUPED = false, bool PRIV = false, bool LIN = false, bool DRAW = false,
+          int NRT_ = 2, int NPT_ = 2>
+__global__ __launch_bounds__(64 * NRT_ * NPT_, OCC) void glm_planes_f16_kernel(
+    const unsigned char* __restrict__ img, const float* __restrict__ y,
+    const float* __restrict__ w, const float* __restrict__ b, int64_t N, int D, int P,
+    int64_t nst, float* __restrict__ part, int prio_cus, const uint32_t* __restrict__ trailer,
+    unsigned long long* __restrict__ tstamps, const GlmGroupArgs grp,
+    const int64_t* __restrict__ gate, const double* __restrict__ moments = nullptr,
+    const GlmDraw draw = GlmDraw{}) {
+  if (gate != nullptr && *gate != 0) return;
+  extern __shared__ __attribute__((aligned(16))) unsigned char smem[];
+  glm_planes_f16_body<NB, OCC, GROUPED, PRIV, LIN, DRAW, NRT_, NPT_>(
+      smem, (int)blockIdx.x, (int)blockIdx.y, (int)gridDim.x, img, y, w, b, N, D, P, nst, part, prio_cus,
+      trailer, tstamps, grp, moments, draw, nullptr, 0u);
+}
+
+}
diff --git a/pyro_amd/csrc/multisite_dev.h b/pyro_amd/csrc/multisite_dev.h
--- a/pyro_amd/csrc/multisite_dev.h
+++ b/pyro_amd/csrc/multisite_dev.h
@@ -121,10 +121,10 @@
 }
 
 template <typename T, int NTHREADS>
-__device__ __forceinline__ double multi_sum_partial(uint32_t kbase, uint32_t skip_mask,
-                                                    uint32_t only_mask) {
+__device__ __forceinline__ double multi_sum_partial_as(uint32_t kbase, uint32_t skip_mask,
+                                                       uint32_t only_mask, const int wave,
+                                                       const int lane) {
   const int n_entries = kernarg_load<int>(kbase + offsetof(MultiArgs, n));
-  const int wave = __builtin_amdgcn_readfirstlane(threadIdx.x >> 6), lane = threadIdx.x & 63;
   constexpr int NW = NTHREADS / 64;
   const int wpe = n_entries >= NW ? 1 : NW / (n_entries > 0 ? n_entries : 1);
   const int epr = NW / wpe;
@@ -142,12 +142,43 @@
   }
   return acc;
 }
+template <typename T, int NTHREADS>
+__device__ __forceinline__ double multi_sum_partial(uint32_t kbase, uint32_t skip_mask,
+                                                    uint32_t only_mask) {
+  return multi_sum_partial_as<T, NTHREADS>(kbase, skip_mask, only_mask,
+                                           __builtin_amdgcn_readfirstlane(threadIdx.x >> 6),
+                                           (int)(threadIdx.x & 63));
+}
 template <typename T>
 __device__ __forceinline__ void multi_sum_finish(double acc, T* __restrict__ out, double coef_all,
                                                  int accumulate) {
   __shared__ double smem[16];
   const double t = block_sum_f64(acc, smem);
   if (threadIdx.x == 0) {
+    const double base = accumulate ? (double)*out : 0.0;
+    *out = (T)(base + coef_all * t);
+  }
+}
+template <typename T>
+__device__ __forceinline__ void multi_sum_finish_v4(double a0, double a1, double a2, double a3,
+                                                    int pwave, T* __restrict__ out, double coef_all,
+                                                    int accumulate) {
+  __shared__ double smem[16];
+  a0 = wave_sum(a0);
+  a1 = wave_sum(a1);
+  a2 = wave_sum(a2);
+  a3 = wave_sum(a3);
+  __syncthreads();
+  if ((threadIdx.x & 63) == 0) {
+    smem[pwave] = a0;
+    smem[pwave + 4] = a1;
+    smem[pwave + 8] = a2;
+    smem[pwave + 12] = a3;
+  }
+  __syncthreads();
+  if (threadIdx.x == 0) {
+    double t = 0.0;
+    for (int i = 0; i < 16; ++i) t += smem[i];
     const double base = accumulate ? (double)*out : 0.0;
     *out = (T)(base + coef_all * t);
   }
diff --git a/pyro_amd/csrc/runtime.hip b/pyro_amd/csrc/runtime.hip
--- a/pyro_amd/csrc/runtime.hip
+++ b/pyro_amd/csrc/runtime.hip
@@ -34,6 +34,7 @@
 };
 static GateDeferred g_gate_late;
 const int64_t* gate_word() { return g_gate == nullptr ? nullptr : g_gate + 1; }
+bool gate_deferred_pending() { return g_gate_late.pending; }
 void gate_aware_launch() {
   if (!g_gate_late.pending) g_gate_aware += 1;
 }
diff --git a/pyro_amd/infer/svi.py b/pyro_amd/infer/svi.py
--- a/pyro_amd/infer/svi.py
+++ b/pyro_amd/infer/svi.py
@@ -634,7 +634,8 @@
                 mode = {"capture_error_mode": "thread_local"} if (split or multi) else {}
                 reads = _ReadSet()
                 blocks = fuser.RtcBlocks()
-                with capture_scope(), blocks, torch.cuda.graph(graph, **mode):
+                two = kernels.two_kernel_step() if kernels.DIRECT_REPLAY["on"] else contextlib.nullcontext()
+                with two, capture_scope(), blocks, torch.cuda.graph(graph, **mode):
                     with fuser.scope(), gated(), cap, chain() as rec, hoist(), reads:
                         if gate is not None:
                             gate.launch()
@@ -653,6 +654,7 @@
                             cap.finish(publish=(loss,) + mailbox)
                     self.chain_stats.append(getattr(rec, "stats", None))
                     self.chain_fused = getattr(rec, "fused", 0)
+                    self.chain_merged = getattr(rec, "merged", 0)
                 if split:
                     optim = self.optim
                     optim.reduce_gradients(params)
diff --git a/pyro_amd/kernels.py b/pyro_amd/kernels.py
--- a/pyro_amd/kernels.py
+++ b/pyro_amd/kernels.py
@@ -170,9 +170,24 @@
     _CHAIN["stamps"] = buf
 
 
-def chain_tune(fuse_tail=True, fast_sites=True, jitter_seed=0, fuse_draw=True):
+def chain_tune(fuse_tail=True, fast_sites=True, jitter_seed=0, fuse_draw=True, merge_step=True):
     check(_lib.load().pa_chain_tune((1 if fuse_tail else 0) | (0 if fast_sites else 2)
-                                    | (0 if fuse_draw else 4) | ((int(jitter_seed) & 0x7fffff) << 8)))
+                                    | (0 if fuse_draw else 4) | (0 if merge_step else 8)
+                                    | ((int(jitter_seed) & 0x7fffff) << 8)))
+    _CHAIN["tune"] = dict(fuse_tail=fuse_tail, fast_sites=fast_sites, jitter_seed=jitter_seed,
+                          fuse_draw=fuse_draw, merge_step=merge_step)
+
+
+class two_kernel_step:
+
+    def __enter__(self):
+        self._prev = dict(_CHAIN.get("tune") or {})
+        chain_tune(**dict(self._prev, merge_step=False))
+        return self
+
+    def __exit__(self, *exc):
+        chain_tune(**self._prev)
+        return False
 
 
 def chain_flush():
@@ -186,6 +201,7 @@
         self.sync = chain_sync_buffer(device)
         self.stats = (0, 0)
         self.fused = 0
+        self.merged = 0
         self._guard = None
 
     def __enter__(self):
@@ -206,6 +222,7 @@
             _CHAIN["keep"] = None
             self.stats = (a.value, b.value)
             self.fused = _lib.load().pa_chain_fused_launches()
+            self.merged = _lib.load().pa_chain_merged_launches()
         if exc[0] is None:
             check(rc)
         return False
```

Result: slower. 9438 ELBO-grad steps/s (64 particles x 1e6-row plate per step) (-24.5%).
